# kdexd/probnmn-clevr

Hardware: AMD Instinct MI355X
Metric: CLEVR questions/sec (joint_training step) (higher is better)
Workload: dtype f32; 1 GPU; joint_training_ours.yml (NMN + seq2seq + REINFORCE), global batch 1024 = 1024 questions per GPU x 1 (BASELINE configs[3]), 14x14x1024 features, half of the batch with program supervision, fwd+bwd+[all-reduce]+clamp+Adam; global_batch=1024, per_gpu_batch=1024, parallelism=dp1

## Files before the change

include/probnmn_hip.h:

```cpp
#ifndef PROBNMN_HIP_H
#define PROBNMN_HIP_H

#include <stdint.h>

#ifdef __cplusplus
extern "C" {
#endif

#define PNMN_EINVAL (-1)
#define PNMN_ESHAPE (-2)

#define PNMN_CHANNELS 128

typedef struct pnmn_conv_item {
    const float* in;
    const float* in2;
    const float* mask;
    const float* gate;
    const float* weight;
    const float* bias;
    float*       out;
    int32_t      dilation;
    int32_t      flags;
    const float* mb_feats;
    const float* mb_attn;
    float*       mb_dfeats;
    float*       mb_dattn;
} pnmn_conv_item;
#define PNMN_CONV_ACCUMULATE 1
#define PNMN_CONV_ATOMIC     2
#define PNMN_CONV_MASKBWD    4
#define PNMN_CONV_DATTN     16
#define PNMN_CONV_MB_SOLE     8

int pnmn_conv_nhwc(const pnmn_conv_item* items, int n_items, int H, int W, int cin_chunks,
                   int ntaps , int in_stride, int out_stride,
                   int cout_blocks , int relu, void* stream);
int pnmn_conv_nhwc_cus(const pnmn_conv_item* items, int n_items, int H, int W, int cin_chunks, int ntaps, int in_stride,
                       int out_stride, int cout_blocks, int relu, int cus, void* stream);
int pnmn_conv_nhwc_launches(int n_items, int H, int W, int cin_chunks, int ntaps, int cout_blocks);
int pnmn_conv_force_split(int split);

typedef struct pnmn_wgrad_item {
    const float* x;
    const float* x2;
    const float* xmask;
    const float* dy;
    const float* gate;
    int32_t      dilation;
    int32_t      reserved;
} pnmn_wgrad_item;

typedef struct pnmn_wgrad_job {
    float*  dw;
    float*  dbias;
    int32_t item_begin;
    int32_t item_end;
} pnmn_wgrad_job;

int pnmn_conv_wgrad(const pnmn_wgrad_item* items, const pnmn_wgrad_job* jobs, int n_jobs, int H,
                    int W, int ntaps, int cin_blocks, int cout_blocks, int x_stride,
                    int dy_stride, void* stream);
int pnmn_conv_wgrad_cus(const pnmn_wgrad_item* items, const pnmn_wgrad_job* jobs, int n_jobs, int H, int W, int ntaps,
                        int cin_blocks, int cout_blocks, int x_stride, int dy_stride, int cus, void* stream);

typedef struct pnmn_wtrans_item {
    const float* src;
    float*       dst;
    int32_t      cout, cin, ntaps, reserved;
} pnmn_wtrans_item;
int pnmn_transpose_weights(const pnmn_wtrans_item* items, int n_items, void* stream);

typedef struct pnmn_dot1_item {
    const float* in;
    const float* w;
    const float* b;
    float*       out;
    const float* dout;
    float*       din;
    float*       dw;
    float*       db;
} pnmn_dot1_item;
int pnmn_dot1_sigmoid_fwd(const pnmn_dot1_item* items, int n_items, int HW, void* stream);
int pnmn_dot1_sigmoid_bwd(const pnmn_dot1_item* items, int n_items, int HW, void* stream);

typedef struct pnmn_same_item {
    const float* feats;
    const float* attn;
    const float* w;
    const float* b;
    float*       out;
    const float* dout;
    float*       dfeats;
    float*       dattn;
    float*       dw;
    float*       db;
} pnmn_same_item;
int pnmn_same_fwd(const pnmn_same_item* items, int n_items, int HW, void* stream);
int pnmn_same_bwd(const pnmn_same_item* items, int n_items, int HW, void* stream);

typedef struct pnmn_minmax_item {
    const float* a;
    const float* b;
    float*       out;
    const float* dout;
    float*       da;
    float*       db;
    int32_t      a_channels, b_channels;
    int32_t      is_max, reserved;
} pnmn_minmax_item;
int pnmn_minmax_fwd(const pnmn_minmax_item* items, int n_items, int HW, int C, void* stream);
int pnmn_minmax_bwd(const pnmn_minmax_item* items, int n_items, int HW, int C, void* stream);

typedef struct pnmn_maskbwd_item {
    const float* dx;
    const float* feats;
    const float* attn;
    float*       dfeats;
    float*       dattn;
} pnmn_maskbwd_item;
int pnmn_mask_bwd(const pnmn_maskbwd_item* items, int n_items, int HW, void* stream);
int pnmn_feat_grad_gather(const pnmn_maskbwd_item* items, float* gfeat, int n_items, int n_examples, int HW, void* stream);

typedef struct pnmn_axpy_item {
    const float* src;
    float*       dst;
    int64_t      n;
} pnmn_axpy_item;
int pnmn_accumulate(const pnmn_axpy_item* items, int n_items, void* stream);
int pnmn_set_rows(const pnmn_axpy_item* items, int n_items, void* stream);

int pnmn_nchw_to_nhwc(const float* src, float* dst, int n, int C, int HW, void* stream);
int pnmn_nchw_to_nhwc_rows(const float* src, float* dst, const int64_t* rows, int n, int C, int HW, void* stream);
int pnmn_nhwc_to_nchw(const float* src, float* dst, int n, int C, int HW, void* stream);

int pnmn_gather_features(const float* store, const int64_t* indices, float* dst, int n, int64_t n_store,
                         int C, int HW, void* stream);
int pnmn_copy_rows_h2d(const void* store, const int64_t* indices, void* dst, int n, int64_t n_store,
                       int64_t row_bytes, void* stream);

int pnmn_maxpool2_flatten_fwd(const float* in, float* out, int n, int H, int W, int C, void* stream);
int pnmn_maxpool2_flatten_bwd(const float* in, const float* dout, float* din, int n, int H, int W,
                              int C, void* stream);

int pnmn_answer_loss(const float* logits, const int64_t* answers, const int32_t* valid,
                     int64_t* predictions, float* loss, float* dlogits, int n, int num_answers,
                     int unknown_index, float scale, void* stream);

typedef struct {
    const float* src;
    const float* src2;
    float* dst;
    int32_t n, k, ld, kind;
} pnmn_derive_job;

int pnmn_token_prep(const int64_t* tokens, int64_t token_row_stride, int B, int T, int pad, int bos, int eos,
                    int drop_first, int64_t* out, float* fmask, int* last, void* stream);
int pnmn_length_order(const int32_t* last, int B, int T, int32_t* order, int32_t* tile_steps, void* stream);
int pnmn_trim_predictions(const int64_t* raw, int B, int T, int end, int64_t* out, void* stream);
int pnmn_mask_last_fwd(const float* hs, const float* fmask, const int* last, int B, int T, int H, float* enc,
                       float* hlast, void* stream);
int pnmn_mask_last_bwd(const float* denc, const float* dhlast, const float* fmask, const int* last, int B, int T,
                       int H, float* dhs, void* stream);
int64_t pnmn_embedding_grad_workspace_bytes(int B, int T, int V);
int pnmn_embedding_grad(const float* dy, const int64_t* tokens, int64_t token_row_stride, int B, int T, int C,
                        int V, int shift, int start, int skip, int accumulate, float* dw, void* workspace, void* stream);
int pnmn_derive_params(const pnmn_derive_job* jobs, int n_jobs, int max_quads, void* stream);

int pnmn_token_table_fwd(const float* emb, const float* weight, int64_t weight_row_stride,
                         const float* bias, int V, int K, int N, float* table, void* stream);
int pnmn_token_table_bwd(const float* dtable, const float* emb, const float* weight,
                         int64_t weight_row_stride, int V, int K, int N, int padding_idx, float* demb,
                         float* dweight, int64_t dweight_row_stride , float* dbias,
                         float* dbias2 , void* stream);

#define PNMN_TOKEN_SEGS 4
typedef struct pnmn_token_seg {
    const int64_t* src;
    const int64_t* index;
    int64_t        row_stride;
    int32_t        rows;
    int32_t        width;
} pnmn_token_seg;
int pnmn_token_rows(const pnmn_token_seg* segs , int n_segs, int64_t* dst, int W, int64_t pad, void* stream);

int pnmn_seq_nll_fwd(const float* logits, int64_t logits_bstride, const int64_t* tokens, int64_t tok_bstride,
                     const int64_t* mask_tokens, int64_t mask_bstride, int pad, float* loss, float* lse,
                     int B, int T, int V, float eps, void* stream);
int pnmn_seq_nll_bwd(const float* logits, int64_t logits_bstride, const int64_t* tokens, int64_t tok_bstride,
                     const int64_t* mask_tokens, int64_t mask_bstride, int pad, const float* lse,
                     const float* dloss, float* dlogits, int64_t dlogits_bstride, int B, int T, int V,
                     float eps, void* stream);

int pnmn_elbo_rows(const float* pg_loss, const float* qr_loss, const float* prior_loss, const float* nmn_loss,
                   const float* baseline, float beta, float gamma, int n, float* sums, float* dpg, void* stream);

int pnmn_joint_objective(const float* pg, const float* qr, const float* prior, const float* nmn, const float* pg_sup,
                         float* baseline, const float* w_unsup, const float* w_sup, float alpha, float beta, float gamma,
                         float decay, int update_baseline, int n, int m, float* stats, float* objective, float* d_pg,
                         float* d_qr, float* d_nmn, float* d_pg_sup, void* stream);

typedef struct pnmn_adam_item {
    float*       param;
    const float* grad;
    float*       exp_avg;
    float*       exp_avg_sq;
    int64_t      n;
    float        bc1;
    float        bc2_sqrt;
} pnmn_adam_item;
int pnmn_clamp_adam(const pnmn_adam_item* items, int n_items, double lr, double beta1, double beta2,
                    double eps, double weight_decay, double clamp, void* stream);
int pnmn_clamp_adam_blocks(const pnmn_adam_item* items, int n_items, double lr, double beta1, double beta2, double eps,
                           double weight_decay, double clamp, int blocks_per_item, void* stream);

int pnmn_lstm_cell_fwd(const float* gates, const float* c_prev, float* h, float* c, float* act,
                       int B, int hidden, void* stream);
int pnmn_lstm_cell_bwd(const float* act, const float* c_prev, const float* c, const float* dh,
                       const float* dc_in, float* dgates, float* dc_prev, int B, int hidden,
                       void* stream);

int pnmn_lstm_seq_fwd(const float* xp, const int64_t* tokens, int64_t token_stride, const float* w_hh,
                      float* hs, float* cs, float* act, int B, int T, int hidden, void* workspace,
                      void* stream);
int pnmn_lstm_seq_bwd(const float* dhs, const float* act, const float* cs, const float* w_hh_t,
                      float* dgates, int B, int T, int hidden, void* workspace, void* stream);
int64_t pnmn_lstm_seq_workspace_bytes(int B, int backward);
int pnmn_lstm_seq_fwd_ordered(const float* xp, const int64_t* tokens, int64_t token_stride, const float* w_hh,
                              float* hs, float* cs, float* act, int B, int T, int hidden, const int32_t* order,
                              const int32_t* tile_steps, void* workspace, void* stream);
int pnmn_lstm_seq_bwd_ordered(const float* dhs, const float* act, const float* cs, const float* w_hh_t,
                              float* dgates, int B, int T, int hidden, const int32_t* order,
                              const int32_t* tile_steps, void* workspace, void* stream);
int pnmn_cluster_reserve_cus(int cus);

int pnmn_attn_lstm_fwd(const float* xe, const float* etable, const float* enc, const float* mask,
                       const float* h0, const float* w_c, const float* w_hh, const float* w_p,
                       const float* b_p, float* hs, float* cs, float* act, float* ctx, float* probs,
                       int64_t* tokens, int B, int T, int S, int V, int hidden, int sample,
                       int pad_index, int unk_index, int start_index, uint64_t seed,
                       uint64_t row_offset, const int64_t* in_tokens, int64_t in_token_stride,
                       void* stream);
int pnmn_attn_lstm_bwd(const float* dhs, const float* act, const float* cs, const float* hs,
                       const float* ctx, const float* probs, const float* enc, const float* mask,
                       const float* h0, const float* w_c_t, const float* w_hh_t, float* dgates,
                       float* denc, float* dh0, int B, int T, int S, int hidden, void* stream);

int pnmn_attn_lstm_beam(const float* etable, const float* enc, const float* mask, const float* h0,
                        const float* w_c, const float* w_hh, const float* w_p, const float* b_p,
                        int64_t* tokens, float* scores, int32_t* trace_tokens, int32_t* trace_backptr,
                        float* trace_scores, int B, int T, int S, int V, int hidden, int beam,
                        int pad_index, int unk_index, int start_index, int end_index, void* stream);

#define PNMN_BEAM_MAX_STATES 32
#define PNMN_BEAM_MAX_CLASSES 16
int pnmn_attn_lstm_beam_constrained(const float* etable, const float* enc, const float* mask, const float* h0,
                                    const float* w_c, const float* w_hh, const float* w_p, const float* b_p,
                                    int64_t* tokens, float* scores, int32_t* trace_tokens, int32_t* trace_backptr,
                                    float* trace_scores, int B, int T, int S, int V, int hidden, int beam,
                                    int pad_index, int unk_index, int start_index, int end_index,
                                    const uint8_t* token_class, const uint8_t* next_state, const uint8_t* min_left,
                                    int n_states, int n_classes, void* stream);

typedef struct pnmn_decoder_fwd_job {
    const float *xe, *etable, *enc, *mask, *h0, *w_c, *w_hh, *w_p, *b_p;
    float *hs, *cs, *act, *ctx, *probs;
    int64_t* tokens;
    const int64_t* in_tokens;
    int64_t in_token_stride;
    uint64_t seed, row_offset;
    int32_t B, T, S, V, sample, pad_index, unk_index, start_index;
} pnmn_decoder_fwd_job;
typedef struct pnmn_decoder_bwd_job {
    const float *dhs, *act, *cs, *hs, *probs, *enc, *mask, *h0, *w_c_t, *w_hh_t;
    float *dgates, *dctx, *dscore, *weights, *dh0;
    int32_t B, T, S, reserved;
} pnmn_decoder_bwd_job;
int64_t pnmn_attn_lstm_group_workspace_bytes(const int32_t* rows, int n, int backward);
int pnmn_attn_lstm_fwd_group(const pnmn_decoder_fwd_job* jobs, int n, int hidden, void* workspace, void* stream);
int pnmn_attn_lstm_bwd_group(const pnmn_decoder_bwd_job* jobs, int n, int hidden, void* workspace, void* stream);
int pnmn_attn_denc(const float* weights, const float* dscore, const float* dctx, const float* hs, const float* h0,
                   float* denc, int B, int T, int S, int hidden, void* stream);

int pnmn_sample_tokens(const float* logits, int64_t* tokens, float* logprobs, int B, int V,
                       int greedy, uint64_t seed, uint64_t row_offset, uint32_t step, int pad_index,
                       int unk_index, int start_index, void* stream);

struct pnmn_sampling_filter {
    float temperature;
    int32_t top_k;
    float top_p;
    int32_t reserved;
};
int pnmn_sample_tokens_filtered(const float* logits, int64_t* tokens, float* logprobs, int B, int V,
                                int greedy, uint64_t seed, uint64_t row_offset, uint32_t step, int pad_index,
                                int unk_index, int start_index, const struct pnmn_sampling_filter* filter ,
                                void* stream);
int pnmn_attn_lstm_fwd_filtered(const float* xe, const float* etable, const float* enc, const float* mask,
                                const float* h0, const float* w_c, const float* w_hh, const float* w_p,
                                const float* b_p, float* hs, float* cs, float* act, float* ctx, float* probs,
                                int64_t* tokens, int B, int T, int S, int V, int hidden, int sample,
                                int pad_index, int unk_index, int start_index, uint64_t seed,
                                uint64_t row_offset, const int64_t* in_tokens, int64_t in_token_stride,
                                const struct pnmn_sampling_filter* filter , void* stream);
int pnmn_attn_lstm_fwd_group_filtered(const pnmn_decoder_fwd_job* jobs, const struct pnmn_sampling_filter* filters ,
                                      int n, int hidden, void* workspace, void* stream);

int pnmn_attn_lstm_fwd_constrained(const float* xe, const float* etable, const float* enc, const float* mask,
                                   const float* h0, const float* w_c, const float* w_hh, const float* w_p,
                                   const float* b_p, float* hs, float* cs, float* act, float* ctx, float* probs,
                                   int64_t* tokens, int B, int T, int S, int V, int hidden, int sample,
                                   int pad_index, int unk_index, int start_index, uint64_t seed,
                                   uint64_t row_offset, const int64_t* in_tokens, int64_t in_token_stride,
                                   const struct pnmn_sampling_filter* filter , int end_index,
                                   const uint8_t* token_class , const uint8_t* next_state ,
                                   const uint8_t* min_left , int n_states, int n_classes, void* stream);
int pnmn_attn_lstm_fwd_group_constrained(const pnmn_decoder_fwd_job* jobs, const struct pnmn_sampling_filter* filters ,
                                         int end_index, const uint8_t* token_class , const uint8_t* next_state ,
                                         const uint8_t* min_left , int n_states, int n_classes,
                                         int n, int hidden, void* workspace, void* stream);

#define PNMN_OP_CONV              0
#define PNMN_OP_WGRAD             1
#define PNMN_OP_TRANSPOSE_WEIGHTS 2
#define PNMN_OP_DOT_FWD           3
#define PNMN_OP_DOT_BWD           4
#define PNMN_OP_SAME_FWD          5
#define PNMN_OP_SAME_BWD          6
#define PNMN_OP_MINMAX_FWD        7
#define PNMN_OP_MINMAX_BWD        8
#define PNMN_OP_MASK_BWD          9
#define PNMN_OP_MAXPOOL_FWD       10
#define PNMN_OP_MAXPOOL_BWD       11
#define PNMN_OP_NCHW_TO_NHWC      12
#define PNMN_OP_SET_ROWS          13
#define PNMN_OP_ACCUMULATE        14
#define PNMN_OP_ZERO              15
#define PNMN_OP_FEAT_GATHER       16
typedef struct pnmn_launch {
    const void* a;
    const void* b;
    const void* c;
    int32_t     op;
    int32_t     n;
    int32_t     p[8];
} pnmn_launch;
int pnmn_run_launches(const pnmn_launch* list, int n, void* stream);

typedef struct pnmn_launch_timing {
    int32_t op, n;
    int32_t p[8];
    int32_t n_items;
    float   ms;
    double  flops, bytes;
} pnmn_launch_timing;
int pnmn_launch_trace_begin(void);
int pnmn_launch_trace_end(pnmn_launch_timing* out, int capacity, int* n_out);

#define PNMN_EAGAIN (-3)
typedef struct pnmn_trunk_config {
    const int32_t* kinds;
    const int64_t* w3;
    const int64_t* b3;
    const int64_t* wt3;
    const int64_t* dotw;
    const int64_t* dotb;
    int32_t n_kinds, channels, H, W, wgrad_chunk, wgrad_groups, fuse_mask_bwd, sole_writer, sort_by_weight, reserved;
} pnmn_trunk_config;
typedef struct pnmn_trunk_io {
    const int64_t*     programs;
    uint64_t           params, grads, wt, act, gact, feat, gfeat, final_, gfinal, ones;
    int64_t            act_capacity;
    const pnmn_launch* fwd_tail;
    const pnmn_launch* bwd_head;
    const pnmn_launch* bwd_tail;
    pnmn_launch*       bwd;
    uint8_t*           valid;
    int64_t            arena_floats;
    int32_t            n_programs, length, n_fwd_tail, n_bwd_head, n_bwd_tail, bwd_capacity, need_backward, launch;
    int32_t            n_bwd, bwd_piece_cut, n_prims, n_fwd, depth, n_invalid, n_feat_result;
    int32_t            conv_cus;
    int32_t            wgrad_cus;
    int32_t            n_conv, n_proj;
    int32_t            reserved;
    uint64_t           touched_tokens[4];
} pnmn_trunk_io;
int pnmn_trunk_planner_create(const pnmn_trunk_config* config, void** planner);
int pnmn_trunk_planner_destroy(void* planner);
int pnmn_trunk_plan_and_launch(void* planner, pnmn_trunk_io* io, void* stream);
int pnmn_trunk_last_forward(void* planner, pnmn_launch* out, int capacity);
int64_t pnmn_trunk_last_records_bytes(void* planner, uint64_t* out, int64_t capacity_words);

typedef struct {
    const int64_t* tables;
    const int64_t* nprims;
    const int64_t* tids;
    const int64_t* examples;
    const int64_t* base;
    const int64_t* tokens;
    const int64_t* w3;
    const int64_t* b3;
    const int64_t* wt3;
    const int64_t* dotw;
    const int64_t* dotb;
    uint64_t params, grads, wt, act, gact, feat, gfeat, final_, gfinal, ones;
    int32_t n_templates, pmax, nv, cmax;
    int32_t hw, channels, wgrad_chunk, wgrad_groups;
    int32_t fuse_mask_bwd, sole_writer, sort_by_weight, reserved;
} pnmn_plan_in;
int pnmn_plan_batch(const pnmn_plan_in* in, uint64_t* out_words, int64_t out_capacity, int64_t* meta, int32_t* cuts,
                    int32_t cuts_capacity);
int pnmn_compile_programs(const int64_t* tokens, int n_programs, int length, const int32_t* kinds,
                          int n_kinds, int channels, uint8_t* valid, int32_t* n_calls,
                          int32_t* calls, int32_t* result);

typedef struct pnmn_conv2d_desc {
    const float* x;
    const float* w;
    const float* scale;
    const float* shift;
    const float* residual;
    float*       y;
    int32_t      N, H, W, Cin, Ho, Wo, Cout, kh, kw, stride, pad, relu;
} pnmn_conv2d_desc;
int pnmn_conv2d_nhwc(const pnmn_conv2d_desc* desc, void* stream);
int pnmn_conv2d_weight_floats(int Cout, int Cin, int kh, int kw);
int pnmn_maxpool3x3s2_nhwc(const float* x, float* y, int N, int H, int W, int C, void* stream);

#define PNMN_IMAGE_PREP_MAX_TAPS  33
#define PNMN_IMAGE_PREP_MAX_WIDTH 448
#define PNMN_IMAGE_PREP_MAX_SIZE  16384
int pnmn_image_prep(const uint8_t* images, int64_t image_stride, int N, int Hin, int Win, const int32_t* kx,
                    const int32_t* xbounds, int ksx, const int32_t* ky, const int32_t* ybounds, int ksy,
// ... 70 lines not shown
```

probnmn-clevr_amd/csrc/decoder_multi.hip:

```cpp
#include <hip/hip_runtime.h>
#include <math.h>
#include <limits.h>
#include <stdint.h>

#include "../../include/probnmn_hip.h"
#include "cluster.h"
#include "lds_optin.h"
#include "sampling.h"

typedef float f32x4 __attribute__((ext_vector_type(4)));

namespace {

using pnmn::sigm;
using pnmn::wmax;
using pnmn::wsum;

constexpr int H = 256;
constexpr int G4 = 4 * H;
constexpr int ROWS = 16;
constexpr int MEMBERS = 8;
constexpr int RW = ROWS / MEMBERS;
constexpr int UW = H / MEMBERS;
constexpr int GLD = UW + 4;
constexpr int MAXS = 64;
constexpr int MAXV = 128;

__device__ __forceinline__ float dot4(const f32x4 a, const f32x4 b) { return a.x * b.x + a.y * b.y + a.z * b.z + a.w * b.w; }

struct MFwdArgs {
    const float* xe;
    const float* etable;
    const float* enc;
    const float* mask;
    const float* h0;
    const float* w_c;
    const float* w_hh;
    const float* w_p;
    const float* b_p;
    float* hs;
    float* cs;
    float* act;
    float* ctx;
    float* probs;
    int64_t* tokens;
    const int64_t* in_tokens;
    long in_stride;
    int* sync;
    int B, T, S, V, tiles;
    int sample;
    int pad, unk, start;
    uint64_t seed, row_offset;
};

constexpr size_t FWD_FIXED_LDS = sizeof(float) * (4 * ROWS * GLD + RW * 4 * H + ROWS * MAXV + RW * MAXS) + sizeof(int) * ROWS;
constexpr size_t FWD_OVERLAP_LDS = sizeof(float) * (ROWS * H + 64);

template <bool OVERLAP, bool SAMPLE, bool FILT = false, bool CONSTR = false>
__device__ __forceinline__ void attn_lstm_fwd_multi_body(const MFwdArgs& a, const int tile, const int part,
                                                         const pnmn::SamplingFilter& f = pnmn::SamplingFilter{1.f, 0, 1.f},
                                                         const pnmn::TokenAutomaton* aut = nullptr) {
    static_assert(SAMPLE || !CONSTR, "the automaton constrains the free-running modes only");
    extern __shared__ __attribute__((aligned(16))) char raw[];
    const int T = a.T, S = a.S;
    float* encl = reinterpret_cast<float*>(raw);
    float (*gl)[ROWS][GLD] = reinterpret_cast<float (*)[ROWS][GLD]>(encl + RW * S * H);
    float (*scl)[MAXS] = reinterpret_cast<float (*)[MAXS]>(&gl[4][0][0]);
    int* tokl = reinterpret_cast<int*>(&scl[RW][0]);
    float (*cpart)[4][H] = reinterpret_cast<float (*)[4][H]>(tokl + ROWS);
    float (*logl)[MAXV] = reinterpret_cast<float (*)[MAXV]>(&cpart[RW][0][0]);
    float* hst = &logl[ROWS][0];
    float* sink = hst + ROWS * H;

    const int tid = threadIdx.x, wave = tid >> 6, lane = tid & 63, li = lane & 15, g = lane >> 4;
    const int row0 = tile * ROWS, myrow0 = row0 + RW * part, u0 = UW * part;
    pnmn::Cluster cl;
    cl.start(a.sync + tile * pnmn::CLUSTER_COUNTER_STRIDE, MEMBERS);

    for (int i = tid; i < RW * S * (H / 4); i += 512) {
        const int rl = i / (S * (H / 4)), rem = i - rl * S * (H / 4);
        f32x4 v = f32x4{0.f, 0.f, 0.f, 0.f};
        if (myrow0 + rl < a.B) v = *reinterpret_cast<const f32x4*>(a.enc + (size_t)(myrow0 + rl) * S * H + 4 * rem);
        *reinterpret_cast<f32x4*>(encl + (size_t)rl * S * H + 4 * rem) = v;
    }
    const int gate = wave >> 1, ub = wave & 1;
    f32x4 wc[H / 16], wh[H / 16];
    {
        const int ntile = gate * (H / 16) + u0 / 16 + ub;
#pragma unroll
        for (int kb = 0; kb < H / 16; ++kb) {
            const size_t fo = ((size_t)(ntile * (H / 16) + kb) * 64 + lane) * 4;
            wc[kb] = *reinterpret_cast<const f32x4*>(a.w_c + fo);
            wh[kb] = *reinterpret_cast<const f32x4*>(a.w_hh + fo);
        }
    }
    if (tid < ROWS) tokl[tid] = a.start;
    const float row_mask = lane < S ? a.mask[(size_t)min(myrow0 + (wave >> 2), a.B - 1) * S + lane] : 0.f;
    float creg = 0.f;
    const int arow = min(row0 + li, a.B - 1);
    const int64_t* tf_row = (a.in_tokens && tid < ROWS) ? a.in_tokens + (size_t)min(row0 + tid, a.B - 1) * a.in_stride : nullptr;
    if (tf_row) tokl[tid] = (int)tf_row[0];

    constexpr int PARTF = ROWS * 64;
    const int s_row = tid >> 5, s_q = tid & 31;
    const int s_rowc = min(row0 + s_row, a.B - 1);
    const int s_off = (s_q >> 4) * PARTF + s_row * 64 + 4 * ((s_q & 15) ^ s_row);
    auto frags = [&](const float* tile_lds, const int p, f32x4 (&f)[4]) {
#pragma unroll
        for (int j = 0; j < 4; ++j) f[j] = *reinterpret_cast<const f32x4*>(tile_lds + p * PARTF + li * 64 + 4 * ((4 * j + g) ^ li));
    };
    auto mfma16 = [&](const f32x4 (&f)[4], const f32x4 (&w)[H / 16], const int p, f32x4& even, f32x4& odd) {
#pragma unroll
        for (int j = 0; j < 4; j += 2) {
            const int kb = p * 4 + j;
            even = __builtin_amdgcn_mfma_f32_16x16x4f32(f[j].x, w[kb].x, even, 0, 0, 0);
            odd = __builtin_amdgcn_mfma_f32_16x16x4f32(f[j + 1].x, w[kb + 1].x, odd, 0, 0, 0);
            even = __builtin_amdgcn_mfma_f32_16x16x4f32(f[j].y, w[kb].y, even, 0, 0, 0);
            odd = __builtin_amdgcn_mfma_f32_16x16x4f32(f[j + 1].y, w[kb + 1].y, odd, 0, 0, 0);
            even = __builtin_amdgcn_mfma_f32_16x16x4f32(f[j].z, w[kb].z, even, 0, 0, 0);
            odd = __builtin_amdgcn_mfma_f32_16x16x4f32(f[j + 1].z, w[kb + 1].z, odd, 0, 0, 0);
            even = __builtin_amdgcn_mfma_f32_16x16x4f32(f[j].w, w[kb].w, even, 0, 0, 0);
            odd = __builtin_amdgcn_mfma_f32_16x16x4f32(f[j + 1].w, w[kb + 1].w, odd, 0, 0, 0);
        }
    };

    auto stage_h = [&](const float* rows, const size_t row_stride) {
        const float* hsrc = rows + (size_t)s_rowc * row_stride + 4 * s_q;
        const f32x4 h_lo = *reinterpret_cast<const f32x4*>(hsrc), h_hi = *reinterpret_cast<const f32x4*>(hsrc + 128);
        *reinterpret_cast<f32x4*>(hst + s_off) = h_lo;
        *reinterpret_cast<f32x4*>(hst + s_off + 2 * PARTF) = h_hi;
    };
    if constexpr (OVERLAP) stage_h(a.h0, H);
    pnmn::AutomatonLds au{};
    int row_state[2] = {0, 0};
    if constexpr (CONSTR) au = pnmn::stage_automaton(reinterpret_cast<unsigned char*>(OVERLAP ? sink + 64 : hst), *aut);
    __syncthreads();

    for (int t = 0; t < T; ++t) {
        int zt = 0;
        asm volatile("" : "+v"(zt));
        f32x4 acc;
        f32x4 ph0 = f32x4{0.f, 0.f, 0.f, 0.f}, ph1 = ph0;
        auto load_inputs = [&] {
#pragma unroll
            for (int r = 0; r < 4; ++r) {
                const int rl = 4 * g + r, row = row0 + rl + zt;
                const int n = gate * H + u0 + 16 * ub + li;
                float v = 0.f;
                if (row < a.B) v = a.xe ? a.xe[((size_t)row * T + t) * G4 + n] : a.etable[(size_t)tokl[rl] * G4 + n];
                acc[r] = v;
            }
        };
        {
            const int rl = wave >> 2, q = wave & 3;
            const int row = myrow0 + rl + zt, rowc = min(row, a.B - 1);
            f32x4 hv;
            if constexpr (OVERLAP) {
                const int r = RW * part + rl;
                hv = *reinterpret_cast<const f32x4*>(hst + (lane >> 4) * PARTF + r * 64 + 4 * ((lane & 15) ^ r));
            } else {
                const float* hp = t > 0 ? a.hs + ((size_t)rowc * T + (t - 1)) * H : a.h0 + (size_t)rowc * H;
                hv = *reinterpret_cast<const f32x4*>(hp + 4 * lane);
            }
            const float* er = encl + (size_t)rl * S * H + 4 * lane;
            constexpr int NP = 4;
            int k_first = 0;
            if constexpr (OVERLAP) {
#pragma unroll
                for (int b = 0; b < 2; ++b) {
                    f32x4 ev[NP], hf[4];
                    float pk[NP];
#pragma unroll
                    for (int k = 0; k < NP; ++k) {
                        const int s = q + 4 * (NP * b + k);
                        ev[k] = *reinterpret_cast<const f32x4*>(er + (size_t)(s < S ? s : S - 1) * H);
                    }
                    frags(hst, b, hf);
                    mfma16(hf, wh, b, ph0, ph1);
#pragma unroll
                    for (int k = 0; k < NP; ++k) pk[k] = dot4(ev[k], hv);
#pragma unroll
                    for (int k = 0; k < NP; ++k) pk[k] = wsum(pk[k]);
#pragma unroll
                    for (int k = 0; k < NP; ++k) {
                        const int s = q + 4 * (NP * b + k);
                        float* dst = (lane == 0 && s < S) ? &scl[rl][s] : sink + lane;
                        *dst = pk[k];
                    }
                }
                k_first = 2 * NP;
            }
            {
                for (int k0 = k_first; q + 4 * k0 < S; k0 += NP) {
                    float part[NP];
#pragma unroll
                    for (int k = 0; k < NP; ++k) {
                        const int s = q + 4 * (k0 + k);
                        part[k] = s < S ? dot4(*reinterpret_cast<const f32x4*>(er + (size_t)s * H), hv) : 0.f;
                    }
#pragma unroll
                    for (int k = 0; k < NP; ++k) part[k] = wsum(part[k]);
#pragma unroll
                    for (int k = 0; k < NP; ++k)
                        if (lane == 0 && q + 4 * (k0 + k) < S) scl[rl][q + 4 * (k0 + k)] = part[k];
                }
            }
            __syncthreads();
            auto softmax = [&] {
                const float m = row_mask;
                const float v = (lane < S ? scl[rl][lane] : 0.f) * m;
                const float mx = wmax(lane < S ? v : -INFINITY);
                const float ex = lane < S ? expf(v - mx) : 0.f;
                const float p = ex / wsum(ex);
                const float qv = p * m;
                const float wgt = qv / (wsum(qv) + 1e-13f);
                if (lane < S) {
                    scl[rl][lane] = wgt;
                    if (row < a.B) a.probs[((size_t)row * T + t) * S + lane] = p;
                }
            };
            if constexpr (OVERLAP) {
                f32x4 hf[4];
                frags(hst, 2, hf);
                if (q == 0) {
                    mfma16(hf, wh, 2, ph0, ph1);
                    softmax();
                } else {
                    mfma16(hf, wh, 2, ph0, ph1);
                }
            } else {
                if (q == 0) softmax();
            }
            __syncthreads();
            f32x4 c4 = f32x4{0.f, 0.f, 0.f, 0.f};
            int s_first = q;
            if constexpr (OVERLAP) {
                constexpr int NC = 4;
                f32x4 ev[NC], hf[4];
                float wv[NC];
#pragma unroll
                for (int k = 0; k < NC; ++k) {
                    const int s = q + 4 * k, sc = s < S ? s : S - 1;
                    ev[k] = *reinterpret_cast<const f32x4*>(er + (size_t)sc * H);
                    const float w = scl[rl][sc];
                    wv[k] = s < S ? w : 0.f;
                }
                frags(hst, 3, hf);
                mfma16(hf, wh, 3, ph0, ph1);
#pragma unroll
                for (int k = 0; k < NC; ++k) c4 += ev[k] * wv[k];
                s_first = q + 4 * NC;
            }
            for (int s = s_first; s < S; s += 4) c4 += *reinterpret_cast<const f32x4*>(er + (size_t)s * H) * scl[rl][s];
            *reinterpret_cast<f32x4*>(&cpart[rl][q][4 * lane]) = c4;
            __syncthreads();
            const int rl2 = tid >> 8, k = tid & 255;
            const float cv = (cpart[rl2][0][k] + cpart[rl2][1][k]) + (cpart[rl2][2][k] + cpart[rl2][3][k]);
            if (myrow0 + rl2 < a.B) a.ctx[((size_t)(myrow0 + rl2 + zt) * T + t) * H + k] = cv;
        }
        cl.signal();
        cl.wait();

        const int tf_next = tf_row ? (int)tf_row[min(t + 1, T - 1)] : 0;
        if constexpr (OVERLAP) {
            float* cst = &cpart[0][0][0];
            const float* csrc = a.ctx + ((size_t)(s_rowc + zt) * T + t) * H + 4 * s_q;
            const f32x4 c_lo = *reinterpret_cast<const f32x4*>(csrc), c_hi = *reinterpret_cast<const f32x4*>(csrc + 128);
            load_inputs();
            *reinterpret_cast<f32x4*>(cst + s_off) = c_lo;
            *reinterpret_cast<f32x4*>(cst + s_off + 2 * PARTF) = c_hi;
            __syncthreads();
            f32x4 pc0 = f32x4{0.f, 0.f, 0.f, 0.f}, pc1 = pc0;
#pragma unroll
            for (int p = 0; p < 4; ++p) {
                f32x4 cf[4];
                frags(cst, p, cf);
                mfma16(cf, wc, p, pc0, pc1);
            }
            acc += (pc0 + pc1) + (ph0 + ph1);
        } else {
            load_inputs();
            constexpr int NB = 4, NPARTS = (H / 16) / NB, PART = 2 * ROWS * 64;
            float* stage = &cpart[0][0][0];
            const int s_tensor = tid >> 8, o_row = (tid >> 4) & 15, o_slot = tid & 15;
            const int o_rowc = min(row0 + o_row, a.B - 1);
            const float* s_src = (s_tensor == 0 ? a.ctx + ((size_t)o_rowc * T + t) * H
                                                : (t > 0 ? a.hs + ((size_t)o_rowc * T + (t - 1)) * H : a.h0 + (size_t)o_rowc * H)) + 4 * o_slot;
            float* s_dst = stage + (s_tensor * ROWS + o_row) * 64 + 4 * (o_slot ^ o_row);
            f32x4 sv = *reinterpret_cast<const f32x4*>(s_src);
            *reinterpret_cast<f32x4*>(s_dst) = sv;
            __syncthreads();
            f32x4 pc0 = f32x4{0.f, 0.f, 0.f, 0.f}, pc1 = pc0;
#pragma unroll
            for (int p = 0; p < NPARTS; ++p) {
                if (p + 1 < NPARTS) sv = *reinterpret_cast<const f32x4*>(s_src + (p + 1) * 64);
                const float* buf = stage + (p & 1) * PART;
                f32x4 ac[NB], ah[NB];
#pragma unroll
                for (int j = 0; j < NB; ++j) {
                    const int slot = (4 * j + g) ^ li;
                    ac[j] = *reinterpret_cast<const f32x4*>(buf + li * 64 + 4 * slot);
                    ah[j] = *reinterpret_cast<const f32x4*>(buf + (ROWS + li) * 64 + 4 * slot);
                }
                mfma16(ac, wc, p, pc0, pc1);
                mfma16(ah, wh, p, ph0, ph1);
                if (p + 1 < NPARTS) {
                    *reinterpret_cast<f32x4*>(s_dst + ((p + 1) & 1) * PART) = sv;
                    __syncthreads();
                }
            }
            acc += (pc0 + pc1) + (ph0 + ph1);
        }
#pragma unroll
        for (int r = 0; r < 4; ++r) gl[gate][4 * g + r][16 * ub + li] = acc[r];
        __syncthreads();
        {
            const int rl = tid >> 5, ul = tid & 31;
            const int row = row0 + rl + zt, u = u0 + ul;
            const float ig = sigm(gl[0][rl][ul]), fg = sigm(gl[1][rl][ul]);
            const float gg = tanhf(gl[2][rl][ul]), og = sigm(gl[3][rl][ul]);
            const float c = fg * creg + ig * gg;
            const float h = og * tanhf(c);
            creg = c;
            if (row < a.B) {
                const size_t o = ((size_t)row * T + t) * H + u;
                a.hs[o] = h;
                a.cs[o] = c;
                float* ar = a.act + ((size_t)row * T + t) * G4;
                ar[u] = ig;
                ar[H + u] = fg;
                ar[2 * H + u] = gg;
                ar[3 * H + u] = og;
            }
        }
        if (tf_row) tokl[tid] = tf_next;
        if (t + 1 == T && !SAMPLE) break;
        cl.signal();
        cl.wait();
        if constexpr (OVERLAP) {
            stage_h(a.hs + ((size_t)zt * T + t) * H, (size_t)T * H);
            __syncthreads();
        }

        if constexpr (SAMPLE) {
            const int V = a.V;
            if (16 * wave < V) {
                f32x4 lacc = f32x4{0.f, 0.f, 0.f, 0.f}, lodd = lacc;
                const int vn = 16 * wave + li;
                const bool vok = vn < V;
                const float* hp = a.hs + ((size_t)arow * T + t) * H + 4 * g;
                constexpr int NB = 4;
#pragma unroll
                for (int part = 0; part < (H / 16) / NB; ++part) {
                    f32x4 ah[NB], bp[NB];
                    if constexpr (OVERLAP) frags(hst, part, ah);
#pragma unroll
                    for (int j = 0; j < NB; ++j) {
                        const int kb = part * NB + j;
                        if constexpr (!OVERLAP) ah[j] = *reinterpret_cast<const f32x4*>(hp + kb * 16);
                        bp[j] = vok ? *reinterpret_cast<const f32x4*>(a.w_p + (size_t)vn * H + kb * 16 + 4 * g)
                                    : f32x4{0.f, 0.f, 0.f, 0.f};
                    }
#pragma unroll
                    for (int j = 0; j < NB; j += 2) {
                        lacc = __builtin_amdgcn_mfma_f32_16x16x4f32(ah[j].x, bp[j].x, lacc, 0, 0, 0);
                        lodd = __builtin_amdgcn_mfma_f32_16x16x4f32(ah[j + 1].x, bp[j + 1].x, lodd, 0, 0, 0);
                        lacc = __builtin_amdgcn_mfma_f32_16x16x4f32(ah[j].y, bp[j].y, lacc, 0, 0, 0);
                        lodd = __builtin_amdgcn_mfma_f32_16x16x4f32(ah[j + 1].y, bp[j + 1].y, lodd, 0, 0, 0);
                        lacc = __builtin_amdgcn_mfma_f32_16x16x4f32(ah[j].z, bp[j].z, lacc, 0, 0, 0);
                        lodd = __builtin_amdgcn_mfma_f32_16x16x4f32(ah[j + 1].z, bp[j + 1].z, lodd, 0, 0, 0);
                        lacc = __builtin_amdgcn_mfma_f32_16x16x4f32(ah[j].w, bp[j].w, lacc, 0, 0, 0);
                        lodd = __builtin_amdgcn_mfma_f32_16x16x4f32(ah[j + 1].w, bp[j + 1].w, lodd, 0, 0, 0);
                    }
                }
                lacc += lodd;
                const float bias = vok ? a.b_p[vn] : 0.f;
#pragma unroll
                for (int r = 0; r < 4; ++r) logl[4 * g + r][vn < MAXV ? vn : 0] = vok ? lacc[r] + bias : -INFINITY;
            }
            __syncthreads();
#pragma unroll
            for (int rr = 0; rr < 2; ++rr) {
                const int rl = 2 * wave + rr;
                const int row = row0 + rl;
                if (row >= a.B) continue;
                int choice;
                if constexpr (CONSTR) {
                    const auto set = pnmn::allowed_lanes(au, row_state[rr], T - 1 - t, V, a.pad, a.unk, a.start);
                    choice = pnmn::choose_row_token<FILT>(logl[rl], V, a.sample, a.pad, a.unk, a.start, a.seed,
                                                          a.row_offset + (uint64_t)row, (uint32_t)t, logl[rl], f, set);
                    row_state[rr] = pnmn::advance_row_state(au, row_state[rr], choice);
                } else {
                    choice = pnmn::choose_row_token<FILT>(logl[rl], V, a.sample, a.pad, a.unk, a.start, a.seed,
                                                          a.row_offset + (uint64_t)row, (uint32_t)t, logl[rl], f);
                }
                if (lane == 0) {
                    tokl[rl] = choice;
                    if (part == 0) a.tokens[(size_t)row * T + t] = choice;
                }
            }
            __syncthreads();
        }
    }
    cl.finish();
}

template <bool OVERLAP, bool SAMPLE>
__global__ __launch_bounds__(512) __attribute__((amdgpu_waves_per_eu(2, 2))) void attn_lstm_fwd_multi_kernel(const MFwdArgs a) {
    int tile, part;
    pnmn::cluster_coords<MEMBERS>(tile, part);
    if (tile >= a.tiles) return;
    attn_lstm_fwd_multi_body<OVERLAP, SAMPLE>(a, tile, part);
}

template <bool OVERLAP, bool SAMPLE0, bool SAMPLE1>
__global__ __launch_bounds__(512) __attribute__((amdgpu_waves_per_eu(2, 2))) void attn_lstm_fwd_pair_kernel(const MFwdArgs a0,
                                                                                                           const MFwdArgs a1,
                                                                                                           const int tiles0) {
    int tile, part;
    pnmn::cluster_coords<MEMBERS>(tile, part);
    if (tile < tiles0) {
        if (tile >= a0.tiles) return;
        attn_lstm_fwd_multi_body<OVERLAP, SAMPLE0>(a0, tile, part);
    } else {
        tile -= tiles0;
        if (tile >= a1.tiles) return;
        attn_lstm_fwd_multi_body<OVERLAP, SAMPLE1>(a1, tile, part);
    }
}

template <bool OVERLAP>
__global__ __launch_bounds__(512) __attribute__((amdgpu_waves_per_eu(2, 2))) void attn_lstm_fwd_multi_filtered_kernel(
    const MFwdArgs a, const pnmn::SamplingFilter f) {
    int tile, part;
    pnmn::cluster_coords<MEMBERS>(tile, part);
    if (tile >= a.tiles) return;
    attn_lstm_fwd_multi_body<OVERLAP, true, true>(a, tile, part, f);
}

template <bool OVERLAP, int M0, int M1>
__global__ __launch_bounds__(512) __attribute__((amdgpu_waves_per_eu(2, 2))) void attn_lstm_fwd_pair_filtered_kernel(
    const MFwdArgs a0, const MFwdArgs a1, const int tiles0, const pnmn::SamplingFilter f0, const pnmn::SamplingFilter f1) {
    int tile, part;
    pnmn::cluster_coords<MEMBERS>(tile, part);
    if (tile < tiles0) {
        if (tile >= a0.tiles) return;
        attn_lstm_fwd_multi_body<OVERLAP, M0 != 0, M0 == 2>(a0, tile, part, f0);
    } else {
        tile -= tiles0;
        if (tile >= a1.tiles) return;
        attn_lstm_fwd_multi_body<OVERLAP, M1 != 0, M1 == 2>(a1, tile, part, f1);
    }
}

template <bool OVERLAP, bool FILT>
__global__ __launch_bounds__(512) __attribute__((amdgpu_waves_per_eu(2, 2))) void attn_lstm_fwd_multi_constrained_kernel(
    const MFwdArgs a, const pnmn::SamplingFilter f, const pnmn::TokenAutomaton au) {
    int tile, part;
    pnmn::cluster_coords<MEMBERS>(tile, part);
    if (tile >= a.tiles) return;
    attn_lstm_fwd_multi_body<OVERLAP, true, FILT, true>(a, tile, part, f, &au);
}

template <bool OVERLAP, int M0, int M1>
__global__ __launch_bounds__(512) __attribute__((amdgpu_waves_per_eu(2, 2))) void attn_lstm_fwd_pair_constrained_kernel(
    const MFwdArgs a0, const MFwdArgs a1, const int tiles0, const pnmn::SamplingFilter f0, const pnmn::SamplingFilter f1,
    const pnmn::TokenAutomaton au) {
    int tile, part;
    pnmn::cluster_coords<MEMBERS>(tile, part);
    if (tile < tiles0) {
        if (tile >= a0.tiles) return;
        attn_lstm_fwd_multi_body<OVERLAP, M0 != 0, M0 == 2, M0 != 0>(a0, tile, part, f0, &au);
    } else {
        tile -= tiles0;
        if (tile >= a1.tiles) return;
        attn_lstm_fwd_multi_body<OVERLAP, M1 != 0, M1 == 2, M1 != 0>(a1, tile, part, f1, &au);
    }
}

struct MBwdArgs {
    const float* dhs;
    const float* act;
    const float* cs;
    const float* hs;
    const float* probs;
    const float* enc;
    const float* mask;
    const float* h0;
    const float* w_c_t;
    const float* w_hh_t;
    float* dgates;
    float* dctx;
    float* dscore;
    float* weights;
    float* dh0;
    float* x1;
    float* x2;
    int* sync;
    int B, T, S, tiles;
};

constexpr int DLD = 4 * UW + 4;
constexpr size_t BWD_FIXED_LDS = sizeof(float) * (ROWS * DLD + 2 * RW * H + 2 * RW * MAXS + RW * 4 * H + 64);

__device__ __forceinline__ void attn_lstm_bwd_multi_body(const MBwdArgs& a, const int tile, const int part) {
    extern __shared__ __attribute__((aligned(16))) char raw[];
    const int T = a.T, S = a.S;
    float* encl = reinterpret_cast<float*>(raw);
    float (*dgl)[DLD] = reinterpret_cast<float (*)[DLD]>(encl + RW * S * H);
    float (*dctxl)[H] = reinterpret_cast<float (*)[H]>(&dgl[ROWS][0]);
    float (*dhl)[H] = dctxl + RW;
    float (*dwl)[MAXS] = reinterpret_cast<float (*)[MAXS]>(&dhl[RW][0]);
    float (*dhpart)[4][H] = reinterpret_cast<float (*)[4][H]>(&dwl[2 * RW][0]);
    float* sink = &dhpart[RW][0][0];

    const int tid = threadIdx.x, wave = tid >> 6, lane = tid & 63, li = lane & 15, g = lane >> 4;
    const int row0 = tile * ROWS, myrow0 = row0 + RW * part, u0 = UW * part;
    pnmn::Cluster cl;
    cl.start(a.sync + tile * pnmn::CLUSTER_COUNTER_STRIDE, MEMBERS);
    float* x1t = a.x1 + (size_t)tile * 2 * MEMBERS * 2 * ROWS * H;
    float* x2t = a.x2 + (size_t)tile * 2 * ROWS * H;

    for (int i = tid; i < RW * S * (H / 4); i += 512) {
        const int rl = i / (S * (H / 4)), rem = i - rl * S * (H / 4);
        f32x4 v = f32x4{0.f, 0.f, 0.f, 0.f};
        if (myrow0 + rl < a.B) v = *reinterpret_cast<const f32x4*>(a.enc + (size_t)(myrow0 + rl) * S * H + 4 * rem);
        *reinterpret_cast<f32x4*>(encl + (size_t)rl * S * H + 4 * rem) = v;
    }
    constexpr int KB = 4 * UW / 16;
    f32x4 wc[2][KB], wh[2][KB];
#pragma unroll
    for (int nt = 0; nt < 2; ++nt)
#pragma unroll
        for (int kl = 0; kl < KB; ++kl) {
            const int q = kl / (UW / 16), jj = kl % (UW / 16);
            const int kb = (q * H + u0) / 16 + jj;
            const size_t fo = ((size_t)((2 * wave + nt) * (G4 / 16) + kb) * 64 + lane) * 4;
            wc[nt][kl] = *reinterpret_cast<const f32x4*>(a.w_c_t + fo);
            wh[nt][kl] = *reinterpret_cast<const f32x4*>(a.w_hh_t + fo);
        }
    float dc_rec = 0.f;
    const float row_mask = lane < S ? a.mask[(size_t)min(myrow0 + (wave >> 2), a.B - 1) * S + lane] : 0.f;
    __syncthreads();

    struct Saved {
        float ig, fg, gg, og, c, cp, dhs, p;
    };
    const int c_rl = tid >> 5, c_ul = tid & 31;
    const int c_row = row0 + c_rl, c_u = u0 + c_ul;
    const int p_row = min(myrow0 + (wave >> 2), a.B - 1);
    auto load_saved = [&](int t) {
        Saved v{0.f, 0.f, 0.f, 0.f, 0.f, 0.f, 0.f, 0.f};
        if (c_row < a.B) {
            const size_t o = ((size_t)c_row * T + t) * H + c_u;
            const float* ar = a.act + ((size_t)c_row * T + t) * G4;
            v.ig = ar[c_u], v.fg = ar[H + c_u], v.gg = ar[2 * H + c_u], v.og = ar[3 * H + c_u];
            v.c = a.cs[o];
            v.cp = t > 0 ? a.cs[o - H] : 0.f;
            v.dhs = a.dhs[o];
        }
        if ((wave & 3) == 0 && lane < S) v.p = a.probs[((size_t)p_row * T + t) * S + lane];
        return v;
    };
    Saved sv = load_saved(T - 1);

    auto dg_frag = [&](const int kl) { return *reinterpret_cast<const f32x4*>(&dgl[li][kl * 16 + 4 * g]); };
    auto mfma16 = [&](const f32x4 (&w)[2][KB], const int kl0, f32x4 (&acc)[2]) {
#pragma unroll
        for (int kl = kl0; kl < kl0 + 2; ++kl) {
            const f32x4 av = dg_frag(kl);
#pragma unroll
            for (int nt = 0; nt < 2; ++nt) {
                acc[nt] = __builtin_amdgcn_mfma_f32_16x16x4f32(w[nt][kl].x, av.x, acc[nt], 0, 0, 0);
                acc[nt] = __builtin_amdgcn_mfma_f32_16x16x4f32(w[nt][kl].y, av.y, acc[nt], 0, 0, 0);
                acc[nt] = __builtin_amdgcn_mfma_f32_16x16x4f32(w[nt][kl].z, av.z, acc[nt], 0, 0, 0);
                acc[nt] = __builtin_amdgcn_mfma_f32_16x16x4f32(w[nt][kl].w, av.w, acc[nt], 0, 0, 0);
            }
        }
    };

    for (int t = T - 1; t >= 0; --t) {
        const Saved cur = sv;
        int zt = 0;
        asm volatile("" : "+v"(zt));
        {
            const int rl = c_rl, ul = c_ul;
            const int row = c_row + zt, u = c_u;
            float di = 0.f, df = 0.f, dg = 0.f, dout = 0.f, dcp = 0.f;
            if (row < a.B) {
                const float ig = cur.ig, fg = cur.fg, gg = cur.gg, og = cur.og;
                const float c = cur.c;
                const float cp = cur.cp;
                const float tc = tanhf(c);
                float dhp = 0.f;
                if (t < T - 1) {
                    const float* ph = x1t + (((size_t)((t + 1) & 1) * MEMBERS) * 2 + 1) * ROWS * H + (size_t)(rl + zt) * H + u;
                    float pv[MEMBERS];
#pragma unroll
                    for (int m = 0; m < MEMBERS; ++m) pv[m] = ph[(size_t)(2 * m) * ROWS * H];
                    const float att = x2t[((size_t)((t + 1) & 1) * ROWS + rl) * H + u];
                    float sh = 0.f;
#pragma unroll
                    for (int m = 0; m < MEMBERS; ++m) sh += pv[m];
                    dhp = sh + att;
                }
                const float dh = cur.dhs + dhp;
                const float dc = dc_rec + dh * og * (1.f - tc * tc);
                di = dc * gg * ig * (1.f - ig);
                df = dc * cp * fg * (1.f - fg);
                dg = dc * ig * (1.f - gg * gg);
                dout = dh * tc * og * (1.f - og);
                dcp = dc * fg;
                float* dr = a.dgates + ((size_t)row * T + t) * G4;
                dr[u] = di;
                dr[H + u] = df;
                dr[2 * H + u] = dg;
                dr[3 * H + u] = dout;
            }
            dc_rec = dcp;
            dgl[rl][ul] = di;
            dgl[rl][UW + ul] = df;
            dgl[rl][2 * UW + ul] = dg;
            dgl[rl][3 * UW + ul] = dout;
        }
        __syncthreads();
        float* const pc = x1t + (((size_t)(t & 1) * MEMBERS + part) * 2 + 0) * ROWS * H;
        float* const ph = pc + ROWS * H;
        {
            f32x4 accc[2] = {f32x4{0.f, 0.f, 0.f, 0.f}, f32x4{0.f, 0.f, 0.f, 0.f}};
#pragma unroll
            for (int kl = 0; kl < KB; kl += 2) mfma16(wc, kl, accc);
#pragma unroll
            for (int nt = 0; nt < 2; ++nt) {
                const size_t o = (size_t)(li + zt) * H + 16 * (2 * wave + nt) + 4 * g;
                *reinterpret_cast<f32x4*>(pc + o) = accc[nt];
            }
        }
        cl.signal();
        cl.wait();

        f32x4 acch[2] = {f32x4{0.f, 0.f, 0.f, 0.f}, f32x4{0.f, 0.f, 0.f, 0.f}};
        {
            const int rl2 = tid >> 8, k = tid & 255;
            const float* src = x1t + (size_t)(t & 1) * MEMBERS * 2 * ROWS * H + (size_t)(RW * part + rl2 + zt) * H + k;
            float pv[MEMBERS];
#pragma unroll
            for (int s = 0; s < MEMBERS; ++s) pv[s] = src[(size_t)(2 * s) * ROWS * H];
            float sc = 0.f;
#pragma unroll
            for (int s = 0; s < MEMBERS; ++s) sc += pv[s];
            dctxl[rl2][k] = sc;
            if (myrow0 + rl2 < a.B) a.dctx[((size_t)(myrow0 + rl2 + zt) * T + t) * H + k] = sc;
        }
        __syncthreads();
        {
            const int rl = wave >> 2, q = wave & 3;
            const int row = myrow0 + rl + zt;
            const float* er = encl + (size_t)rl * S * H + 4 * lane;
            const f32x4 dc4 = *reinterpret_cast<const f32x4*>(&dctxl[rl][4 * lane]);
            constexpr int NP = 4;
#pragma unroll
            for (int b = 0; b < 2; ++b) {
                f32x4 ev[NP];
                float pk[NP];
#pragma unroll
                for (int k = 0; k < NP; ++k) {
                    const int s = q + 4 * (NP * b + k);
                    ev[k] = *reinterpret_cast<const f32x4*>(er + (size_t)(s < S ? s : S - 1) * H);
                }
                mfma16(wh, 2 * b, acch);
#pragma unroll
                for (int k = 0; k < NP; ++k) pk[k] = dot4(ev[k], dc4);
#pragma unroll
                for (int k = 0; k < NP; ++k) pk[k] = wsum(pk[k]);
#pragma unroll
                for (int k = 0; k < NP; ++k) {
                    const int s = q + 4 * (NP * b + k);
                    float* dst = (lane == 0 && s < S) ? &dwl[rl][s] : sink + lane;
                    *dst = pk[k];
                }
            }
            for (int k0 = 2 * NP; q + 4 * k0 < S; k0 += NP) {
                float part[NP];
#pragma unroll
                for (int k = 0; k < NP; ++k) {
                    const int s = q + 4 * (k0 + k);
                    part[k] = s < S ? dot4(*reinterpret_cast<const f32x4*>(er + (size_t)s * H), dc4) : 0.f;
                }
#pragma unroll
                for (int k = 0; k < NP; ++k) part[k] = wsum(part[k]);
#pragma unroll
                for (int k = 0; k < NP; ++k)
                    if (lane == 0 && q + 4 * (k0 + k) < S) dwl[rl][q + 4 * (k0 + k)] = part[k];
            }
            __syncthreads();
            auto softmax_bwd = [&] {
                const float m = row_mask;
                const float p = lane < S ? cur.p : 0.f;
                const float qv = p * m;
                const float Z = wsum(qv) + 1e-13f;
                const float dw = lane < S ? dwl[rl][lane] : 0.f;
                const float dq = dw / Z - wsum(dw * qv) / (Z * Z);
                const float dp = dq * m;
                const float dv = p * (dp - wsum(dp * p));
                const float dscore = dv * m;
                if (lane < S) {
                    dwl[rl][lane] = dscore;
                    if (row < a.B) {
                        a.dscore[((size_t)row * T + t) * S + lane] = dscore;
                        a.weights[((size_t)row * T + t) * S + lane] = qv / Z;
                    }
                }
            };
            if (q == 0) {
                mfma16(wh, 4, acch);
                softmax_bwd();
            } else {
                mfma16(wh, 4, acch);
            }
            __syncthreads();
            f32x4 dh4 = f32x4{0.f, 0.f, 0.f, 0.f};
            {
                constexpr int NC = 4;
                f32x4 ev[NC];
                float wv[NC];
#pragma unroll
                for (int k = 0; k < NC; ++k) {
                    const int s = q + 4 * k, sc = s < S ? s : S - 1;
                    ev[k] = *reinterpret_cast<const f32x4*>(er + (size_t)sc * H);
                    const float w = dwl[rl][sc];
                    wv[k] = s < S ? w : 0.f;
                }
                mfma16(wh, 6, acch);
#pragma unroll
                for (int k = 0; k < NC; ++k) dh4 += ev[k] * wv[k];
            }
            for (int s = q + 16; s < S; s += 4) dh4 += *reinterpret_cast<const f32x4*>(er + (size_t)s * H) * dwl[rl][s];
            *reinterpret_cast<f32x4*>(&dhpart[rl][q][4 * lane]) = dh4;
        }
#pragma unroll
        for (int nt = 0; nt < 2; ++nt) {
            const size_t o = (size_t)(li + zt) * H + 16 * (2 * wave + nt) + 4 * g;
            *reinterpret_cast<f32x4*>(ph + o) = acch[nt];
        }
        __syncthreads();
        {
            const int rl2 = tid >> 8, k = tid & 255;
            const float v = (dhpart[rl2][0][k] + dhpart[rl2][1][k]) + (dhpart[rl2][2][k] + dhpart[rl2][3][k]);
            x2t[((size_t)(t & 1) * ROWS + RW * part + rl2 + zt) * H + k] = v;
        }
        if (t > 0) sv = load_saved(t - 1);
        cl.signal();
        cl.wait();
    }
    {
        const int rl2 = tid >> 8, k = tid & 255;
        const float* ph0 = x1t + (size_t)1 * ROWS * H + (size_t)(RW * part + rl2) * H + k;
        float pv[MEMBERS];
#pragma unroll
        for (int m = 0; m < MEMBERS; ++m) pv[m] = ph0[(size_t)(2 * m) * ROWS * H];
        const float att = x2t[((size_t)0 * ROWS + RW * part + rl2) * H + k];
        float sh = 0.f;
#pragma unroll
        for (int m = 0; m < MEMBERS; ++m) sh += pv[m];
        if (myrow0 + rl2 < a.B) a.dh0[(size_t)(myrow0 + rl2) * H + k] = sh + att;
    }
    cl.finish();
}

__global__ __launch_bounds__(512) __attribute__((amdgpu_waves_per_eu(2, 2))) void attn_lstm_bwd_multi_kernel(const MBwdArgs a) {
    int tile, part;
    pnmn::cluster_coords<MEMBERS>(tile, part);
    if (tile >= a.tiles) return;
    attn_lstm_bwd_multi_body(a, tile, part);
}

__global__ __launch_bounds__(512) __attribute__((amdgpu_waves_per_eu(2, 2))) void attn_lstm_bwd_pair_kernel(const MBwdArgs a0,
                                                                                                           const MBwdArgs a1,
                                                                                                           const int tiles0) {
    int tile, part;
    pnmn::cluster_coords<MEMBERS>(tile, part);
    if (tile < tiles0) {
        if (tile >= a0.tiles) return;
        attn_lstm_bwd_multi_body(a0, tile, part);
    } else {
        tile -= tiles0;
        if (tile >= a1.tiles) return;
        attn_lstm_bwd_multi_body(a1, tile, part);
    }
}

__global__ __launch_bounds__(512) __attribute__((amdgpu_waves_per_eu(2, 2))) void attn_lstm_bwd_group3_kernel(const MBwdArgs a0,
                                                                                                             const MBwdArgs a1,
                                                                                                             const MBwdArgs a2,
                                                                                                             const int tiles0,
                                                                                                             const int tiles01) {
    int tile, part;
    pnmn::cluster_coords<MEMBERS>(tile, part);
    if (tile < tiles0) {
        if (tile >= a0.tiles) return;
        attn_lstm_bwd_multi_body(a0, tile, part);
    } else if (tile < tiles01) {
        tile -= tiles0;
        if (tile >= a1.tiles) return;
        attn_lstm_bwd_multi_body(a1, tile, part);
    } else {
        tile -= tiles01;
        if (tile >= a2.tiles) return;
        attn_lstm_bwd_multi_body(a2, tile, part);
    }
}

const void* fwd_multi_variant(bool overlap, bool sample) {
    if (overlap) return sample ? reinterpret_cast<const void*>(attn_lstm_fwd_multi_kernel<true, true>)
                               : reinterpret_cast<const void*>(attn_lstm_fwd_multi_kernel<true, false>);
    return sample ? reinterpret_cast<const void*>(attn_lstm_fwd_multi_kernel<false, true>)
                  : reinterpret_cast<const void*>(attn_lstm_fwd_multi_kernel<false, false>);
}
template <bool OVERLAP>
const void* fwd_pair_variant_of(bool s0, bool s1) {
    if (s0) return s1 ? reinterpret_cast<const void*>(attn_lstm_fwd_pair_kernel<OVERLAP, true, true>)
                      : reinterpret_cast<const void*>(attn_lstm_fwd_pair_kernel<OVERLAP, true, false>);
    return s1 ? reinterpret_cast<const void*>(attn_lstm_fwd_pair_kernel<OVERLAP, false, true>)
              : reinterpret_cast<const void*>(attn_lstm_fwd_pair_kernel<OVERLAP, false, false>);
}
const void* fwd_pair_variant(bool overlap, bool s0, bool s1) {
    return overlap ? fwd_pair_variant_of<true>(s0, s1) : fwd_pair_variant_of<false>(s0, s1);
}

const void* fwd_multi_filtered_variant(bool overlap) {
    return overlap ? reinterpret_cast<const void*>(attn_lstm_fwd_multi_filtered_kernel<true>)
                   : reinterpret_cast<const void*>(attn_lstm_fwd_multi_filtered_kernel<false>);
}
template <bool OVERLAP>
const void* fwd_pair_filtered_variant_of(int m0, int m1) {
    if (m0 == 2) return m1 == 2 ? reinterpret_cast<const void*>(attn_lstm_fwd_pair_filtered_kernel<OVERLAP, 2, 2>)
                       : m1 == 1 ? reinterpret_cast<const void*>(attn_lstm_fwd_pair_filtered_kernel<OVERLAP, 2, 1>)
                                 : reinterpret_cast<const void*>(attn_lstm_fwd_pair_filtered_kernel<OVERLAP, 2, 0>);
    return m0 == 1 ? reinterpret_cast<const void*>(attn_lstm_fwd_pair_filtered_kernel<OVERLAP, 1, 2>)
                   : reinterpret_cast<const void*>(attn_lstm_fwd_pair_filtered_kernel<OVERLAP, 0, 2>);
}
const void* fwd_pair_filtered_variant(bool overlap, int m0, int m1) {
    return overlap ? fwd_pair_filtered_variant_of<true>(m0, m1) : fwd_pair_filtered_variant_of<false>(m0, m1);
}

const void* fwd_multi_constrained_variant(bool overlap, int m) {
    if (overlap) return m == 2 ? reinterpret_cast<const void*>(attn_lstm_fwd_multi_constrained_kernel<true, true>)
                               : reinterpret_cast<const void*>(attn_lstm_fwd_multi_constrained_kernel<true, false>);
    return m == 2 ? reinterpret_cast<const void*>(attn_lstm_fwd_multi_constrained_kernel<false, true>)
                  : reinterpret_cast<const void*>(attn_lstm_fwd_multi_constrained_kernel<false, false>);
}
template <bool OVERLAP>
const void* fwd_pair_constrained_variant_of(int m0, int m1) {
    if (m0 == 0) return m1 == 2 ? reinterpret_cast<const void*>(attn_lstm_fwd_pair_constrained_kernel<OVERLAP, 0, 2>)
                                : reinterpret_cast<const void*>(attn_lstm_fwd_pair_constrained_kernel<OVERLAP, 0, 1>);
    if (m0 == 1) return m1 == 2 ? reinterpret_cast<const void*>(attn_lstm_fwd_pair_constrained_kernel<OVERLAP, 1, 2>)
                                : reinterpret_cast<const void*>(attn_lstm_fwd_pair_constrained_kernel<OVERLAP, 1, 1>);
    return reinterpret_cast<const void*>(attn_lstm_fwd_pair_constrained_kernel<OVERLAP, 2, 2>);
}
const void* fwd_pair_constrained_variant(bool overlap, int m0, int m1) {
    return overlap ? fwd_pair_constrained_variant_of<true>(m0, m1) : fwd_pair_constrained_variant_of<false>(m0, m1);
}

int rows_per_launch() {
    const int cus = pnmn::device_cus();
    return cus >= 8 * MEMBERS ? (cus / (8 * MEMBERS)) * 8 * ROWS : 0;
}


constexpr size_t LDS_LIMIT = 160 * 1024;
constexpr int MAX_JOBS = 3;

inline int padded_tiles(int B) { return 8 * ((((B + ROWS - 1) / ROWS) + 7) / 8); }

bool fits(const int* rows, int n) {
    const int chunk = rows_per_launch();
    int tiles = 0;
    for (int i = 0; i < n; ++i) {
        if (rows[i] <= 0) return false;
        tiles += padded_tiles(rows[i]);
    }
    return chunk > 0 && tiles * ROWS <= chunk && tiles <= 128;
}
template <class Job>
bool jobs_fit(const Job* j, int n) {
    int rows[MAX_JOBS];
    for (int i = 0; i < n; ++i) {
        if (j[i].T <= 0) return false;
        rows[i] = j[i].B;
    }
    return fits(rows, n);
}

int exchange_tiles(const int* rows, int n, int chunk) {
    if (n == 1) return ((rows[0] < chunk ? rows[0] : chunk) + ROWS - 1) / ROWS;
    int tiles = 0;
    for (int i = 0; i < n; ++i) tiles += padded_tiles(rows[i]);
    return tiles;
}

int64_t workspace_bytes(const int* rows, int n, bool backward) {
    if (n > 1 && !fits(rows, n)) {
        const int64_t a = workspace_bytes(rows, n - 1, backward), b = workspace_bytes(rows + n - 1, 1, backward);
        return a > b ? a : b;
    }
    const int chunk = rows_per_launch();
    if (chunk <= 0 || rows[0] <= 0) return 0;
    int64_t bytes = (int64_t)pnmn::CLUSTER_SYNC_BYTES;
    if (backward) bytes += (int64_t)exchange_tiles(rows, n, chunk) * (2 * MEMBERS * 2 + 2) * ROWS * H * sizeof(float);
    return bytes;
}

int check_job(const pnmn_decoder_fwd_job& j, int hidden) {
    if (!j.enc || !j.mask || !j.h0 || !j.w_c || !j.w_hh || !j.hs || !j.cs || !j.act || !j.ctx || !j.probs) return PNMN_EINVAL;
    if (j.sample ? (!j.etable || !j.w_p || !j.b_p || !j.tokens) : (!j.xe && !(j.etable && j.in_tokens))) return PNMN_EINVAL;
    if (hidden != H || j.S < 1 || j.S > MAXS || (j.sample && (j.V < 1 || j.V > MAXV))) return PNMN_ESHAPE;
    return 0;
}
int check_job(const pnmn_decoder_bwd_job& j, int hidden) {
    if (!j.dhs || !j.act || !j.cs || !j.hs || !j.probs || !j.enc || !j.mask || !j.h0 || !j.w_c_t || !j.w_hh_t || !j.dgates ||
        !j.dctx || !j.dscore || !j.weights || !j.dh0)
        return PNMN_EINVAL;
    if (hidden != H || j.S < 1 || j.S > MAXS) return PNMN_ESHAPE;
    return 0;
}

MFwdArgs kernel_args(const pnmn_decoder_fwd_job& j, size_t r, int rows, int* sync, int tile0) {
    const int T = j.T, S = j.S;
    return MFwdArgs{j.xe ? j.xe + r * T * G4 : nullptr, j.etable, j.enc + r * S * H, j.mask + r * S, j.h0 + r * H, j.w_c, j.w_hh,
                    j.w_p, j.b_p, j.hs + r * T * H, j.cs + r * T * H, j.act + r * T * G4, j.ctx + r * T * H, j.probs + r * T * S,
                    j.tokens ? j.tokens + r * T : nullptr, (!j.sample && !j.xe) ? j.in_tokens + r * j.in_token_stride : nullptr,
                    (long)j.in_token_stride, sync + tile0 * pnmn::CLUSTER_COUNTER_STRIDE, rows, T, S, j.V, (rows + ROWS - 1) / ROWS,
                    j.sample, j.pad_index, j.unk_index, j.start_index, j.seed, j.row_offset + r};
}
MBwdArgs kernel_args(const pnmn_decoder_bwd_job& j, size_t r, int rows, int* sync, int tile0, float* x1, float* x2) {
    const int T = j.T, S = j.S;
    return MBwdArgs{j.dhs + r * T * H, j.act + r * T * G4, j.cs + r * T * H, j.hs + r * T * H, j.probs + r * T * S,
                    j.enc + r * S * H, j.mask + r * S, j.h0 + r * H, j.w_c_t, j.w_hh_t, j.dgates + r * T * G4, j.dctx + r * T * H,
                    j.dscore + r * T * S, j.weights + r * T * S, j.dh0 + r * H, x1 + (size_t)tile0 * 2 * MEMBERS * 2 * ROWS * H,
                    x2 + (size_t)tile0 * 2 * ROWS * H, sync + tile0 * pnmn::CLUSTER_COUNTER_STRIDE, rows, T, S,
                    (rows + ROWS - 1) / ROWS};
}

template <class Job>
int plan_group(const Job* j, int n, int hidden, int& smax, int& chunk, int* rows, int* tile0) {
    smax = 0;
    tile0[0] = 0;
    for (int i = 0; i < n; ++i) {
        if (const int e = check_job(j[i], hidden)) return e;
        smax = j[i].S > smax ? j[i].S : smax;
        rows[i] = j[i].B;
        tile0[i + 1] = tile0[i] + padded_tiles(rows[i]);
    }
    chunk = rows_per_launch();
    return chunk > 0 ? 0 : PNMN_ESHAPE;
}

int launch_fwd_constrained(const pnmn_decoder_fwd_job* j, const pnmn_sampling_filter* f, const pnmn::TokenAutomaton& au, int n,
                           int hidden, void* workspace, hipStream_t st);
int launch_fwd(const pnmn_decoder_fwd_job* j, const pnmn_sampling_filter* f, int n, int hidden, void* workspace, hipStream_t st,
               const pnmn::TokenAutomaton* au = nullptr) {
    if (n > 1 && !jobs_fit(j, n)) {
        const int rc = launch_fwd(j, f, n - 1, hidden, workspace, st, au);
        return rc != 0 ? rc : launch_fwd(j + n - 1, f ? f + n - 1 : nullptr, 1, hidden, workspace, st, au);
    }
    if (au && (j[0].sample != 0 || (n > 1 && j[1].sample != 0))) return launch_fwd_constrained(j, f, *au, n, hidden, workspace, st);
    if (j[0].B <= 0 || j[0].T <= 0) return 0;
    int smax, chunk, rows[MAX_JOBS], tile0[MAX_JOBS + 1];
    if (const int e = plan_group(j, n, hidden, smax, chunk, rows, tile0)) return e;
    const bool overlap = FWD_FIXED_LDS + sizeof(float) * RW * smax * H + FWD_OVERLAP_LDS <= LDS_LIMIT;
    const size_t lds = FWD_FIXED_LDS + sizeof(float) * RW * smax * H + (overlap ? FWD_OVERLAP_LDS : 0);
    const bool s0 = j[0].sample != 0, s1 = n > 1 && j[1].sample != 0;
    int m[2] = {0, 0};
    pnmn::SamplingFilter ff[2] = {{1.f, 0, 1.f}, {1.f, 0, 1.f}};
    for (int i = 0; i < n; ++i) {
        m[i] = j[i].sample == 0 ? 0 : (f && j[i].sample == 1 && !pnmn::filter_is_identity(f[i])) ? 2 : 1;
        if (m[i] == 2) ff[i] = pnmn::SamplingFilter{f[i].temperature, f[i].top_k, f[i].top_p};
    }
    const bool filtered = m[0] == 2 || m[1] == 2;
    const void* kernel = filtered ? (n == 1 ? fwd_multi_filtered_variant(overlap) : fwd_pair_filtered_variant(overlap, m[0], m[1]))
                                  : (n == 1 ? fwd_multi_variant(overlap, s0) : fwd_pair_variant(overlap, s0, s1));
    {
        static std::atomic<uint64_t> cfg[2][8], cfg_filtered[2][2][9];
        std::atomic<uint64_t>& c = filtered ? cfg_filtered[n - 1][overlap][3 * m[0] + m[1]] : cfg[n - 1][4 * overlap + 2 * s0 + s1];
        if (const int e = pnmn::opt_in_lds(kernel, LDS_LIMIT, c)) return e;
    }
    int* sync = nullptr;
    if (n > 1) {
        hipError_t e = pnmn::cluster_sync_block(workspace, st, &sync);
        if (e != hipSuccess) return (int)e;
        const MFwdArgs a0 = kernel_args(j[0], 0, rows[0], sync, 0), a1 = kernel_args(j[1], 0, rows[1], sync, tile0[1]);
        if (filtered) {
            const auto pair = reinterpret_cast<void (*)(const MFwdArgs, const MFwdArgs, const int, const pnmn::SamplingFilter,
                                                        const pnmn::SamplingFilter)>(const_cast<void*>(kernel));
            hipLaunchKernelGGL(pair, dim3(MEMBERS * tile0[2]), dim3(512), lds, st, a0, a1, tile0[1], ff[0], ff[1]);
        } else {
            const auto pair = reinterpret_cast<void (*)(const MFwdArgs, const MFwdArgs, const int)>(const_cast<void*>(kernel));
            hipLaunchKernelGGL(pair, dim3(MEMBERS * tile0[2]), dim3(512), lds, st, a0, a1, tile0[1]);
        }
        return (int)hipGetLastError();
    }
    for (int r0 = 0; r0 < rows[0]; r0 += chunk) {
        const int part = rows[0] - r0 < chunk ? rows[0] - r0 : chunk;
        hipError_t e = pnmn::cluster_sync_block(workspace, st, &sync);
        if (e != hipSuccess) return (int)e;
        const MFwdArgs a = kernel_args(j[0], (size_t)r0, part, sync, 0);
        if (filtered) {
            const auto multi = reinterpret_cast<void (*)(const MFwdArgs, const pnmn::SamplingFilter)>(const_cast<void*>(kernel));
            hipLaunchKernelGGL(multi, dim3(MEMBERS * padded_tiles(part)), dim3(512), lds, st, a, ff[0]);
        } else {
            const auto multi = reinterpret_cast<void (*)(const MFwdArgs)>(const_cast<void*>(kernel));
            hipLaunchKernelGGL(multi, dim3(MEMBERS * padded_tiles(part)), dim3(512), lds, st, a);
        }
        e = hipGetLastError();
        if (e != hipSuccess) return (int)e;
    }
    return 0;
}

int launch_fwd_constrained(const pnmn_decoder_fwd_job* j, const pnmn_sampling_filter* f, const pnmn::TokenAutomaton& au, int n,
                           int hidden, void* workspace, hipStream_t st) {
    if (j[0].B <= 0 || j[0].T <= 0) return 0;
    int smax, chunk, rows[MAX_JOBS], tile0[MAX_JOBS + 1];
    if (const int e = plan_group(j, n, hidden, smax, chunk, rows, tile0)) return e;
    constexpr size_t TABLES = pnmn::AUTOMATON_LDS_BYTES;
    const bool overlap = FWD_FIXED_LDS + sizeof(float) * RW * smax * H + FWD_OVERLAP_LDS + TABLES <= LDS_LIMIT;
    const size_t lds = FWD_FIXED_LDS + sizeof(float) * RW * smax * H + (overlap ? FWD_OVERLAP_LDS : 0) + TABLES;
    int m[2] = {0, 0};
    pnmn::SamplingFilter ff[2] = {{1.f, 0, 1.f}, {1.f, 0, 1.f}};
    for (int i = 0; i < n; ++i) {
        m[i] = j[i].sample == 0 ? 0 : (j[i].sample == 1 && !pnmn::filter_is_identity(f[i])) ? 2 : 1;
        if (m[i] == 2) ff[i] = pnmn::SamplingFilter{f[i].temperature, f[i].top_k, f[i].top_p};
    }
    int* sync = nullptr;
    static std::atomic<uint64_t> cfg[2][2][9];
    if (n > 1) {
        const int lo = m[0] <= m[1] ? 0 : 1, hi = 1 - lo;
        const void* kernel = fwd_pair_constrained_variant(overlap, m[lo], m[hi]);
        if (const int e = pnmn::opt_in_lds(kernel, LDS_LIMIT, cfg[1][overlap][3 * m[lo] + m[hi]])) return e;
        hipError_t e = pnmn::cluster_sync_block(workspace, st, &sync);
        if (e != hipSuccess) return (int)e;
        const int tiles_lo = padded_tiles(rows[lo]);
        const MFwdArgs a0 = kernel_args(j[lo], 0, rows[lo], sync, 0), a1 = kernel_args(j[hi], 0, rows[hi], sync, tiles_lo);
        const auto pair = reinterpret_cast<void (*)(const MFwdArgs, const MFwdArgs, const int, const pnmn::SamplingFilter,
                                                    const pnmn::SamplingFilter, const pnmn::TokenAutomaton)>(const_cast<void*>(kernel));
        hipLaunchKernelGGL(pair, dim3(MEMBERS * tile0[2]), dim3(512), lds, st, a0, a1, tiles_lo, ff[lo], ff[hi], au);
        return (int)hipGetLastError();
    }
    const void* kernel = fwd_multi_constrained_variant(overlap, m[0]);
    if (const int e = pnmn::opt_in_lds(kernel, LDS_LIMIT, cfg[0][overlap][m[0]])) return e;
    const auto multi = reinterpret_cast<void (*)(const MFwdArgs, const pnmn::SamplingFilter, const pnmn::TokenAutomaton)>(
        const_cast<void*>(kernel));
    for (int r0 = 0; r0 < rows[0]; r0 += chunk) {
        const int part = rows[0] - r0 < chunk ? rows[0] - r0 : chunk;
        hipError_t e = pnmn::cluster_sync_block(workspace, st, &sync);
        if (e != hipSuccess) return (int)e;
        const MFwdArgs a = kernel_args(j[0], (size_t)r0, part, sync, 0);
        hipLaunchKernelGGL(multi, dim3(MEMBERS * padded_tiles(part)), dim3(512), lds, st, a, ff[0], au);
        e = hipGetLastError();
        if (e != hipSuccess) return (int)e;
    }
    return 0;
}

int launch_bwd(const pnmn_decoder_bwd_job* j, int n, int hidden, void* workspace, hipStream_t st) {
    if (n > 1 && !jobs_fit(j, n)) {
        const int rc = launch_bwd(j, n - 1, hidden, workspace, st);
        return rc != 0 ? rc : launch_bwd(j + n - 1, 1, hidden, workspace, st);
    }
    if (j[0].B <= 0 || j[0].T <= 0) return 0;
    int smax, chunk, rows[MAX_JOBS], tile0[MAX_JOBS + 1];
    if (const int e = plan_group(j, n, hidden, smax, chunk, rows, tile0)) return e;
    const size_t lds = BWD_FIXED_LDS + sizeof(float) * RW * smax * H;
    {
        const void* const kernels[MAX_JOBS] = {reinterpret_cast<const void*>(attn_lstm_bwd_multi_kernel),
                                               reinterpret_cast<const void*>(attn_lstm_bwd_pair_kernel),
                                               reinterpret_cast<const void*>(attn_lstm_bwd_group3_kernel)};
        static std::atomic<uint64_t> cfg[MAX_JOBS];
        if (const int e = pnmn::opt_in_lds(kernels[n - 1], LDS_LIMIT, cfg[n - 1])) return e;
    }
    float* x1 = reinterpret_cast<float*>(static_cast<char*>(workspace) + pnmn::CLUSTER_SYNC_BYTES);
    float* x2 = x1 + (size_t)exchange_tiles(rows, n, chunk) * 2 * MEMBERS * 2 * ROWS * H;
    int* sync = nullptr;
    if (n > 1) {
        hipError_t e = pnmn::cluster_sync_block(workspace, st, &sync);
        if (e != hipSuccess) return (int)e;
        MBwdArgs a[MAX_JOBS];
        for (int i = 0; i < n; ++i) a[i] = kernel_args(j[i], 0, rows[i], sync, tile0[i], x1, x2);
        const dim3 grid(MEMBERS * tile0[n]);
        if (n == 2) hipLaunchKernelGGL(attn_lstm_bwd_pair_kernel, grid, dim3(512), lds, st, a[0], a[1], tile0[1]);
        else hipLaunchKernelGGL(attn_lstm_bwd_group3_kernel, grid, dim3(512), lds, st, a[0], a[1], a[2], tile0[1], tile0[2]);
        return (int)hipGetLastError();
    }
    for (int r0 = 0; r0 < rows[0]; r0 += chunk) {
        const int part = rows[0] - r0 < chunk ? rows[0] - r0 : chunk;
        hipError_t e = pnmn::cluster_sync_block(workspace, st, &sync);
        if (e != hipSuccess) return (int)e;
        const MBwdArgs a = kernel_args(j[0], (size_t)r0, part, sync, 0, x1, x2);
        hipLaunchKernelGGL(attn_lstm_bwd_multi_kernel, dim3(MEMBERS * padded_tiles(part)), dim3(512), lds, st, a);
        e = hipGetLastError();
        if (e != hipSuccess) return (int)e;
    }
    return 0;
}

}

extern "C" {

int64_t pnmn_attn_lstm_group_workspace_bytes(const int32_t* rows, int n, int backward) {
    if (!rows || n < 1 || n > MAX_JOBS) return 0;
    return workspace_bytes(rows, n, backward != 0);
}

int pnmn_attn_lstm_fwd_group(const pnmn_decoder_fwd_job* jobs, int n, int hidden, void* workspace, void* stream) {
    if (!jobs || !workspace || n < 1 || n > 2) return PNMN_EINVAL;
    return launch_fwd(jobs, nullptr, n, hidden, workspace, static_cast<hipStream_t>(stream));
}

int pnmn_attn_lstm_fwd_group_filtered(const pnmn_decoder_fwd_job* jobs, const pnmn_sampling_filter* filters, int n, int hidden,
                                      void* workspace, void* stream) {
    if (!jobs || !filters || !workspace || n < 1 || n > 2) return PNMN_EINVAL;
    for (int i = 0; i < n; ++i)
        if (!pnmn::filter_valid(filters + i)) return PNMN_EINVAL;
    return launch_fwd(jobs, filters, n, hidden, workspace, static_cast<hipStream_t>(stream));
}

int pnmn_attn_lstm_fwd_group_constrained(const pnmn_decoder_fwd_job* jobs, const pnmn_sampling_filter* filters, int end_index,
                                         const uint8_t* token_class, const uint8_t* next_state, const uint8_t* min_left,
                                         int n_states, int n_classes, int n, int hidden, void* workspace, void* stream) {
    if (!jobs || !filters || !workspace || n < 1 || n > 2) return PNMN_EINVAL;
    int V = 0, T = INT_MAX;
    for (int i = 0; i < n; ++i) {
        if (!pnmn::filter_valid(filters + i)) return PNMN_EINVAL;
        if (jobs[i].sample == 0) continue;
        if (V != 0 && jobs[i].V != V) return PNMN_EINVAL;
        V = jobs[i].V;
        T = jobs[i].T < T ? jobs[i].T : T;
    }
    pnmn::TokenAutomaton au;
    if (const int e = pnmn::fill_automaton(au, token_class, next_state, min_left, n_states, n_classes, V, T, end_index)) return e;
    return launch_fwd(jobs, filters, n, hidden, workspace, static_cast<hipStream_t>(stream), &au);
}

int pnmn_attn_lstm_bwd_group(const pnmn_decoder_bwd_job* jobs, int n, int hidden, void* workspace, void* stream) {
    if (!jobs || !workspace || n < 1 || n > MAX_JOBS) return PNMN_EINVAL;
    return launch_bwd(jobs, n, hidden, workspace, static_cast<hipStream_t>(stream));
}

}
```

probnmn-clevr_amd/csrc/seqglue.hip:

```cpp
#include <hip/hip_runtime.h>
#include <stdint.h>
#include <stdlib.h>

#include "../../include/probnmn_hip.h"

namespace {

__global__ __launch_bounds__(256) void token_prep_kernel(const int64_t* __restrict__ tokens, int64_t tstride, int B, int T,
                                                         int pad, int bos, int eos, int drop_first,
                                                         int64_t* __restrict__ out, float* __restrict__ fmask,
                                                         int* __restrict__ last) {
    const int b = blockIdx.x * 4 + (threadIdx.x >> 6);
    const int lane = threadIdx.x & 63;
    if (b >= B) return;
    const int64_t* row = tokens + (size_t)b * tstride;
    int n = 0;
    for (int t = lane; t < T; t += 64) n += row[t] != pad;
#pragma unroll
    for (int o = 32; o > 0; o >>= 1) n += __shfl_xor(n, o);
    const int W = T + 2 - drop_first;
    int valid = 0;
    for (int j = lane; j < W; j += 64) {
        const int f = j + drop_first;
        int64_t v = (f == 0) ? bos : (f <= T ? row[f - 1] : 0);
        if (f == n + 1) v = eos;
        out[(size_t)b * W + j] = v;
        const bool m = v != pad;
        if (fmask) fmask[(size_t)b * W + j] = m ? 1.f : 0.f;
        valid += m;
    }
    if (last) {
#pragma unroll
        for (int o = 32; o > 0; o >>= 1) valid += __shfl_xor(valid, o);
        if (lane == 0) last[b] = valid - 1;
    }
}

struct TokenSegs {
    pnmn_token_seg s[PNMN_TOKEN_SEGS];
    int n;
};
__global__ __launch_bounds__(256) void token_rows_kernel(const TokenSegs segs, int64_t* __restrict__ dst, int W, int64_t pad,
                                                         int total) {
    const int r = blockIdx.x * 4 + (threadIdx.x >> 6), lane = threadIdx.x & 63;
    if (r >= total) return;
    int k = 0, first = 0;
    while (k + 1 < segs.n && r >= first + segs.s[k].rows) first += segs.s[k].rows, ++k;
    const pnmn_token_seg sg = segs.s[k];
    const int64_t i = sg.index ? sg.index[r - first] : (int64_t)(r - first);
    const int64_t* row = sg.src + i * sg.row_stride;
    for (int w = lane; w < W; w += 64) dst[(size_t)r * W + w] = w < sg.width ? row[w] : pad;
}

__global__ __launch_bounds__(256) void trim_predictions_kernel(const int64_t* __restrict__ raw, int B, int T, int end,
                                                               int64_t* __restrict__ out) {
    const int b = blockIdx.x * 4 + (threadIdx.x >> 6);
    const int lane = threadIdx.x & 63;
    if (b >= B) return;
    const int64_t* row = raw + (size_t)b * T;
    int first = T;
    for (int t = lane; t < T; t += 64)
        if (row[t] == end && t < first) first = t;
#pragma unroll
    for (int o = 32; o > 0; o >>= 1) first = min(first, __shfl_xor(first, o));
    for (int t = lane; t < T; t += 64) {
        const bool keep = (first == T) || (first > 0 && t <= first);
        out[(size_t)b * T + t] = keep ? row[t] : 0;
    }
}

__global__ __launch_bounds__(256) void mask_last_fwd_kernel(const float* __restrict__ hs, const float* __restrict__ fmask,
                                                            const int* __restrict__ last, int T, int H,
                                                            float* __restrict__ enc, float* __restrict__ hlast) {
    const int b = blockIdx.x;
    int l = last[b];
    if (l < 0) l += T;
    const int h4 = H >> 2;
    const float4* src = reinterpret_cast<const float4*>(hs + (size_t)b * T * H);
    float4* dst = reinterpret_cast<float4*>(enc + (size_t)b * T * H);
    for (int i = blockIdx.y * 256 + threadIdx.x; i < T * h4; i += gridDim.y * 256) {
        const int t = i / h4;
        const float m = fmask[(size_t)b * T + t];
        float4 v = src[i];
        v.x *= m, v.y *= m, v.z *= m, v.w *= m;
        dst[i] = v;
        if (t == l) reinterpret_cast<float4*>(hlast + (size_t)b * H)[i - t * h4] = v;
    }
}

constexpr int LO_MAX_T = 4096;
__global__ __launch_bounds__(64) void length_order_kernel(const int32_t* __restrict__ last, int B, int T,
                                                          int32_t* __restrict__ order, int32_t* __restrict__ tile_steps) {
    extern __shared__ int first[];
    const int lane = threadIdx.x;
    for (int s = lane; s <= T; s += 64) first[s] = 0;
    __syncthreads();
    for (int b = lane; b < B; b += 64) atomicAdd(&first[min(max(last[b] + 1, 1), T)], 1);
    __syncthreads();
    int carry = 0;
    for (int top = T; top >= 1; top -= 64) {
        const int s = top - lane;
        const int n = s >= 1 ? first[s] : 0;
        int incl = n;
#pragma unroll
        for (int o = 1; o < 64; o <<= 1) {
            const int v = __shfl_up(incl, o);
            if (lane >= o) incl += v;
        }
        if (s >= 1) first[s] = carry + incl - n;
        carry += __shfl(incl, 63);
    }
    __syncthreads();
    for (int b0 = 0; b0 < B; b0 += 64) {
        const int b = b0 + lane;
        const int s = b < B ? min(max(last[b] + 1, 1), T) : 0;
        int before = 0, after = 0;
        for (int j = 0; j < 64; ++j) {
            const int sj = __shfl(s, j);
            before += (sj == s && j < lane);
            after += (sj == s && j > lane);
        }
        const int pos = s ? first[s] + before : 0;
        __syncthreads();
        if (s) {
            order[pos] = b;
            if ((pos & 15) == 0) tile_steps[pos >> 4] = s;
            if (after == 0) first[s] = pos + 1;
        }
        __syncthreads();
    }
}

__global__ __launch_bounds__(256) void mask_last_bwd_kernel(const float* __restrict__ denc, const float* __restrict__ dhlast,
                                                            const float* __restrict__ fmask, const int* __restrict__ last,
                                                            int T, int H, float* __restrict__ dhs) {
    const int b = blockIdx.x;
    int l = last[b];
    if (l < 0) l += T;
    const int h4 = H >> 2;
    const float4* src = denc ? reinterpret_cast<const float4*>(denc + (size_t)b * T * H) : nullptr;
    float4* dst = reinterpret_cast<float4*>(dhs + (size_t)b * T * H);
    for (int i = blockIdx.y * 256 + threadIdx.x; i < T * h4; i += gridDim.y * 256) {
        const int t = i / h4;
        const float m = fmask[(size_t)b * T + t];
        float4 v = src ? src[i] : float4{0.f, 0.f, 0.f, 0.f};
        if (dhlast && t == l) {
            const float4 d = reinterpret_cast<const float4*>(dhlast + (size_t)b * H)[i - t * h4];
            v.x += d.x, v.y += d.y, v.z += d.z, v.w += d.w;
        }
        v.x *= m, v.y *= m, v.z *= m, v.w *= m;
        dst[i] = v;
    }
}

constexpr int EG_CHUNK = 64;

__device__ __forceinline__ int eg_token(const int64_t* __restrict__ tokens, int64_t tok_bstride, int T, unsigned magic, int shift,
                                        int start, int skip, int V, int r) {
    int b = magic ? (int)__umulhi((unsigned)r, magic) : r;
    b -= (b * T > r);
    const int t = r - b * T;
    const int64_t raw = tokens[(size_t)b * tok_bstride + (shift ? max(t - 1, 0) : t)];
    const int64_t v = (shift && t == 0) ? (int64_t)start : raw;
    return (v == skip || v < 0 || v >= V) ? -1 : (int)v;
}

__global__ __launch_bounds__(1024) void embedding_rows_kernel(const int64_t* __restrict__ tokens, int64_t tok_bstride, int B,
                                                              int T, unsigned magic, int V, int shift, int start, int skip, int C,
                                                              int* __restrict__ order, int* __restrict__ chunks, int max_per,
                                                              int* __restrict__ count, float* __restrict__ dw, int keep) {
    __shared__ int whist[16][128], hist[128], rowbase[128], chbase[128];
    const int tid = threadIdx.x, wave = tid >> 6;
    const int per = (B * T + gridDim.x - 1) / gridDim.x;
    const int lo = blockIdx.x * per, R = min(B * T, lo + per);
    chunks += 3 * (size_t)blockIdx.x * max_per;
    count += blockIdx.x;
    for (int i = tid; i < 16 * 128; i += 1024) (&whist[0][0])[i] = 0;
    __syncthreads();
    constexpr int UN = 8;
    for (int r0 = lo + tid; r0 < R; r0 += 1024 * UN) {
        int v[UN];
#pragma unroll
        for (int u = 0; u < UN; ++u) v[u] = eg_token(tokens, tok_bstride, T, magic, shift, start, skip, V, min(r0 + 1024 * u, R - 1));
#pragma unroll
        for (int u = 0; u < UN; ++u)
            if (r0 + 1024 * u < R && v[u] >= 0) atomicAdd(&whist[wave][v[u]], 1);
    }
    if (!keep)
        for (size_t i = blockIdx.x * 1024 + tid; i < (size_t)V * C / 4; i += 1024 * gridDim.x)
            reinterpret_cast<float4*>(dw)[i] = float4{0.f, 0.f, 0.f, 0.f};
    __syncthreads();
    if (tid < 128) {
        int run = 0;
        for (int w = 0; w < 16; ++w) {
            const int n = whist[w][tid];
            whist[w][tid] = run;
            run += n;
        }
        hist[tid] = run;
    }
    __syncthreads();
    if (tid == 0) {
        int rows = lo, ch = 0;
        for (int v = 0; v < V; ++v) {
            rowbase[v] = rows, chbase[v] = ch;
            rows += hist[v];
            ch += (hist[v] + EG_CHUNK - 1) / EG_CHUNK;
        }
        *count = ch;
    }
    __syncthreads();
    for (int r0 = lo + tid; r0 < R; r0 += 1024 * UN) {
        int v[UN];
#pragma unroll
        for (int u = 0; u < UN; ++u) v[u] = eg_token(tokens, tok_bstride, T, magic, shift, start, skip, V, min(r0 + 1024 * u, R - 1));
#pragma unroll
        for (int u = 0; u < UN; ++u)
            if (r0 + 1024 * u < R && v[u] >= 0) order[rowbase[v[u]] + atomicAdd(&whist[wave][v[u]], 1)] = r0 + 1024 * u;
    }
    for (int v = tid; v < V; v += 1024) {
        const int n = hist[v];
        for (int j = 0; j * EG_CHUNK < n; ++j) {
            int* c = chunks + 3 * (chbase[v] + j);
            c[0] = v, c[1] = rowbase[v] + j * EG_CHUNK, c[2] = rowbase[v] + min(n, (j + 1) * EG_CHUNK);
        }
    }
}

__global__ __launch_bounds__(256) void embedding_sum_kernel(const float* __restrict__ dy, const int* __restrict__ order,
                                                            const int* __restrict__ chunks, int max_per,
                                                            const int* __restrict__ count, int C, float* __restrict__ dw) {
    const int slice = blockIdx.x / max_per, j = blockIdx.x % max_per;
    if (j >= count[slice]) return;
    const int c = (blockIdx.y * 256 + threadIdx.x) * 4;
    if (c >= C) return;
    const int* ch = chunks + 3 * ((size_t)slice * max_per + j);
    const int v = ch[0], b = ch[1], e = ch[2];
    constexpr int UN = 8;
    float4 acc = float4{0.f, 0.f, 0.f, 0.f};
    for (int i = b; i < e; i += UN) {
        float4 q[UN];
#pragma unroll
        for (int u = 0; u < UN; ++u) q[u] = *reinterpret_cast<const float4*>(dy + (size_t)order[min(i + u, e - 1)] * C + c);
#pragma unroll
        for (int u = 0; u < UN; ++u)
            if (i + u < e) acc.x += q[u].x, acc.y += q[u].y, acc.z += q[u].z, acc.w += q[u].w;
    }
    float* dst = dw + (size_t)v * C + c;
    unsafeAtomicAdd(dst, acc.x);
    unsafeAtomicAdd(dst + 1, acc.y);
    unsafeAtomicAdd(dst + 2, acc.z);
    unsafeAtomicAdd(dst + 3, acc.w);
}

__global__ __launch_bounds__(256) void derive_params_kernel(const pnmn_derive_job* __restrict__ jobs) {
    const pnmn_derive_job jb = jobs[blockIdx.y];
    const int q = blockIdx.x * 256 + threadIdx.x;
    if (jb.kind == 2) {
        if (q * 4 < jb.n) {
            const float4 a = reinterpret_cast<const float4*>(jb.src)[q], b = reinterpret_cast<const float4*>(jb.src2)[q];
            reinterpret_cast<float4*>(jb.dst)[q] = float4{a.x + b.x, a.y + b.y, a.z + b.z, a.w + b.w};
        }
        return;
    }
    if ((size_t)q * 4 >= (size_t)jb.n * jb.k) return;
    const int r = q & 15, a = (q >> 4) & 3, kb = jb.k >> 4;
    const int j = (q >> 6) % kb, i = (q >> 6) / kb;
    const int x = 16 * i + r, y = 16 * j + 4 * a;
    float4 v;
    if (jb.kind == 0) {
        v = *reinterpret_cast<const float4*>(jb.src + (size_t)x * jb.ld + y);
    } else {
        v.x = jb.src[(size_t)(y + 0) * jb.ld + x];
        v.y = jb.src[(size_t)(y + 1) * jb.ld + x];
        v.z = jb.src[(size_t)(y + 2) * jb.ld + x];
        v.w = jb.src[(size_t)(y + 3) * jb.ld + x];
    }
    reinterpret_cast<float4*>(jb.dst)[q] = v;
}


typedef float f32x4 __attribute__((ext_vector_type(4)));

__device__ __forceinline__ f32x4 mfma4(const f32x4 a, const f32x4 b, f32x4 acc) {
    acc = __builtin_amdgcn_mfma_f32_16x16x4f32(a.x, b.x, acc, 0, 0, 0);
    acc = __builtin_amdgcn_mfma_f32_16x16x4f32(a.y, b.y, acc, 0, 0, 0);
    acc = __builtin_amdgcn_mfma_f32_16x16x4f32(a.z, b.z, acc, 0, 0, 0);
    acc = __builtin_amdgcn_mfma_f32_16x16x4f32(a.w, b.w, acc, 0, 0, 0);
    return acc;
}

__global__ __launch_bounds__(256) void token_table_fwd_kernel(const float* __restrict__ emb, const float* __restrict__ w, long ldw,
                                                              const float* __restrict__ bias, int V, int K, int N,
                                                              float* __restrict__ table) {
    const int wave = threadIdx.x >> 6, lane = threadIdx.x & 63, li = lane & 15, g = lane >> 4;
    const int n0 = 16 * blockIdx.x;
    const float* wrow = w + (size_t)(n0 + li) * ldw + 4 * g;
    const float b = bias ? bias[n0 + li] : 0.f;
    for (int mt = wave; 16 * mt < V; mt += 4) {
        const float* arow = emb + (size_t)min(16 * mt + li, V - 1) * K + 4 * g;
        f32x4 acc = f32x4{0.f, 0.f, 0.f, 0.f};
        for (int kb = 0; kb < K / 16; ++kb)
            acc = mfma4(*reinterpret_cast<const f32x4*>(arow + 16 * kb), *reinterpret_cast<const f32x4*>(wrow + 16 * kb), acc);
#pragma unroll
        for (int r = 0; r < 4; ++r) {
            const int v = 16 * mt + 4 * g + r;
            if (v < V) table[(size_t)v * N + n0 + li] = acc[r] + b;
        }
    }
}

__global__ __launch_bounds__(256) void token_table_bwd_kernel(const float* __restrict__ dtable, const float* __restrict__ emb,
                                                              const float* __restrict__ w, long ldw, int V, int K, int N,
                                                              int padding_idx, float* __restrict__ demb,
                                                              float* __restrict__ dw, long lddw, float* __restrict__ dbias,
                                                              float* __restrict__ dbias2) {
    __shared__ float lds[128 * 17];
    const int tid = threadIdx.x, wave = tid >> 6, lane = tid & 63, li = lane & 15, g = lane >> 4;
    const int V16 = (V + 15) & ~15;
    if ((int)blockIdx.x < N / 16) {
        const int n0 = 16 * blockIdx.x;
        for (int i = tid; i < V16 * 16; i += 256) {
            const int v = i >> 4, c = i & 15;
            lds[v * 17 + c] = v < V ? dtable[(size_t)v * N + n0 + c] : 0.f;
        }
        __syncthreads();
        if (dbias && tid < 16) {
            float sum = 0.f;
            for (int v = 0; v < V; ++v) sum += lds[v * 17 + tid];
            dbias[n0 + tid] = sum;
            if (dbias2) dbias2[n0 + tid] = sum;
        }
        if (!dw) return;
        for (int kt = wave; kt < K / 16; kt += 4) {
            f32x4 acc = f32x4{0.f, 0.f, 0.f, 0.f};
            for (int vb = 0; vb < V16 / 16; ++vb) {
                f32x4 a, b;
#pragma unroll
                for (int j = 0; j < 4; ++j) {
                    const int v = 16 * vb + 4 * g + j;
                    a[j] = lds[v * 17 + li];
                    b[j] = v < V ? emb[(size_t)v * K + 16 * kt + li] : 0.f;
                }
                acc = mfma4(a, b, acc);
            }
#pragma unroll
            for (int r = 0; r < 4; ++r) dw[(size_t)(n0 + 4 * g + r) * lddw + 16 * kt + li] = acc[r];
        }
        return;
    }
    if (!demb) return;
    const int tile = blockIdx.x - N / 16, mt = tile / (K / 16), kt = tile % (K / 16);
    const float* arow = dtable + (size_t)min(16 * mt + li, V - 1) * N + 4 * g;
    f32x4 acc = f32x4{0.f, 0.f, 0.f, 0.f};
    const int per = N / 4;
    for (int n = wave * per; n < (wave + 1) * per; n += 16) {
        f32x4 b;
#pragma unroll
        for (int j = 0; j < 4; ++j) b[j] = w[(size_t)(n + 4 * g + j) * ldw + 16 * kt + li];
        acc = mfma4(*reinterpret_cast<const f32x4*>(arow + n), b, acc);
    }
#pragma unroll
    for (int r = 0; r < 4; ++r) lds[(wave * 16 + 4 * g + r) * 17 + li] = acc[r];
    __syncthreads();
    {
        const int r = tid >> 4, c = tid & 15, v = 16 * mt + r;
        if (v < V) {
            const float sum = (lds[r * 17 + c] + lds[(16 + r) * 17 + c]) + (lds[(32 + r) * 17 + c] + lds[(48 + r) * 17 + c]);
            demb[(size_t)v * K + 16 * kt + c] = v == padding_idx ? 0.f : sum;
        }
    }
}

}

extern "C" int pnmn_token_prep(const int64_t* tokens, int64_t token_row_stride, int B, int T, int pad, int bos, int eos,
                               int drop_first, int64_t* out, float* fmask, int* last, void* stream) {
    if (B <= 0) return 0;
    if (!tokens || !out || T < 0) return PNMN_EINVAL;
    hipLaunchKernelGGL(token_prep_kernel, dim3((B + 3) / 4), dim3(256), 0, static_cast<hipStream_t>(stream), tokens,
                       token_row_stride, B, T, pad, bos, eos, drop_first, out, fmask, last);
    return (int)hipGetLastError();
}

extern "C" int pnmn_length_order(const int32_t* last, int B, int T, int32_t* order, int32_t* tile_steps, void* stream) {
    if (B <= 0) return 0;
    if (!last || !order || !tile_steps || T <= 0) return PNMN_EINVAL;
    if (T > LO_MAX_T) return PNMN_ESHAPE;
    hipLaunchKernelGGL(length_order_kernel, dim3(1), dim3(64), (size_t)(T + 1) * sizeof(int), static_cast<hipStream_t>(stream),
                       last, B, T, order, tile_steps);
    return (int)hipGetLastError();
}

extern "C" int pnmn_token_rows(const pnmn_token_seg* segs, int n_segs, int64_t* dst, int W, int64_t pad, void* stream) {
    if (n_segs <= 0 || W <= 0) return 0;
    if (!segs || !dst || n_segs > PNMN_TOKEN_SEGS) return PNMN_EINVAL;
    TokenSegs t;
    int total = 0;
    for (int k = 0; k < n_segs; ++k) {
        if (segs[k].rows < 0 || (segs[k].rows > 0 && !segs[k].src) || segs[k].width < 0) return PNMN_EINVAL;
        t.s[k] = segs[k];
        total += segs[k].rows;
    }
    t.n = n_segs;
    if (total == 0) return 0;
    hipLaunchKernelGGL(token_rows_kernel, dim3((total + 3) / 4), dim3(256), 0, static_cast<hipStream_t>(stream), t, dst, W, pad,
                       total);
    return (int)hipGetLastError();
}

extern "C" int pnmn_trim_predictions(const int64_t* raw, int B, int T, int end, int64_t* out, void* stream) {
    if (B <= 0 || T <= 0) return 0;
    if (!raw || !out) return PNMN_EINVAL;
    hipLaunchKernelGGL(trim_predictions_kernel, dim3((B + 3) / 4), dim3(256), 0, static_cast<hipStream_t>(stream), raw, B, T,
                       end, out);
    return (int)hipGetLastError();
}

extern "C" int pnmn_mask_last_fwd(const float* hs, const float* fmask, const int* last, int B, int T, int H, float* enc,
                                  float* hlast, void* stream) {
    if (B <= 0 || T <= 0) return 0;
    if (!hs || !fmask || !last || !enc || !hlast || (H & 3)) return PNMN_EINVAL;
    const int per_row = (T * (H >> 2) + 255) / 256;
    hipLaunchKernelGGL(mask_last_fwd_kernel, dim3(B, per_row < 8 ? per_row : 8), dim3(256), 0,
                       static_cast<hipStream_t>(stream), hs, fmask, last, T, H, enc, hlast);
    return (int)hipGetLastError();
}

extern "C" int pnmn_mask_last_bwd(const float* denc, const float* dhlast, const float* fmask, const int* last, int B, int T,
                                  int H, float* dhs, void* stream) {
    if (B <= 0 || T <= 0) return 0;
    if (!fmask || !last || !dhs || (H & 3)) return PNMN_EINVAL;
    const int per_row = (T * (H >> 2) + 255) / 256;
    hipLaunchKernelGGL(mask_last_bwd_kernel, dim3(B, per_row < 8 ? per_row : 8), dim3(256), 0,
                       static_cast<hipStream_t>(stream), denc, dhlast, fmask, last, T, H, dhs);
    return (int)hipGetLastError();
}

namespace {
constexpr int EG_SLICES = 8;
inline int eg_max_per(long rows, int V) { return (int)(((rows + EG_SLICES - 1) / EG_SLICES) / EG_CHUNK) + V; }
}

extern "C" int64_t pnmn_embedding_grad_workspace_bytes(int B, int T, int V) {
    if (B <= 0 || T <= 0 || V <= 0) return 0;
    const long rows = (long)B * T;
    return (int64_t)sizeof(int) * (rows + (long)EG_SLICES * (3 * eg_max_per(rows, V) + 1));
}

extern "C" int pnmn_embedding_grad(const float* dy, const int64_t* tokens, int64_t token_row_stride, int B, int T, int C,
                                   int V, int shift, int start, int skip, int accumulate, float* dw, void* workspace,
                                   void* stream) {
    if (V <= 0 || C <= 0) return 0;
    if (!dw || (C & 3) || V > 128) return PNMN_EINVAL;
    hipStream_t s = static_cast<hipStream_t>(stream);
    if (B <= 0 || T <= 0) return accumulate ? 0 : (int)hipMemsetAsync(dw, 0, sizeof(float) * (size_t)V * C, s);
    if (!dy || !tokens || !workspace) return PNMN_EINVAL;
    const long rows = (long)B * T;
    if (rows * T >= (1L << 32)) return PNMN_ESHAPE;
    const unsigned magic = T == 1 ? 0u : (unsigned)(((1ULL << 32) + T - 1) / T);
    const int max_per = eg_max_per(rows, V);
    int* order = static_cast<int*>(workspace);
    int* chunks = order + rows;
    int* count = chunks + 3 * (size_t)EG_SLICES * max_per;
    hipLaunchKernelGGL(embedding_rows_kernel, dim3(EG_SLICES), dim3(1024), 0, s, tokens, token_row_stride, B, T, magic, V, shift,
                       start, skip, C, order, chunks, max_per, count, dw, accumulate);
    hipLaunchKernelGGL(embedding_sum_kernel, dim3(EG_SLICES * max_per, (C + 1023) / 1024), dim3(256), 0, s, dy, order, chunks,
                       max_per, count, C, dw);
    return (int)hipGetLastError();
}

extern "C" int pnmn_derive_params(const pnmn_derive_job* jobs, int n_jobs, int max_quads, void* stream) {
    if (n_jobs <= 0) return 0;
    if (!jobs || max_quads <= 0) return PNMN_EINVAL;
    hipLaunchKernelGGL(derive_params_kernel, dim3((max_quads + 255) / 256, n_jobs), dim3(256), 0,
                       static_cast<hipStream_t>(stream), jobs);
    return (int)hipGetLastError();
}

extern "C" int pnmn_token_table_fwd(const float* emb, const float* weight, int64_t weight_row_stride, const float* bias, int V,
                                    int K, int N, float* table, void* stream) {
    if (V <= 0) return 0;
    if (!emb || !weight || !table) return PNMN_EINVAL;
    if (V > 128 || K < 16 || K % 16 || N < 64 || N % 64 || weight_row_stride % 4) return PNMN_ESHAPE;
    hipLaunchKernelGGL(token_table_fwd_kernel, dim3(N / 16), dim3(256), 0, static_cast<hipStream_t>(stream), emb, weight,
                       (long)weight_row_stride, bias, V, K, N, table);
    return (int)hipGetLastError();
}

extern "C" int pnmn_token_table_bwd(const float* dtable, const float* emb, const float* weight, int64_t weight_row_stride, int V,
                                    int K, int N, int padding_idx, float* demb, float* dweight, int64_t dweight_row_stride,
                                    float* dbias, float* dbias2, void* stream) {
    if (V <= 0) return 0;
    if (!dtable || !emb || !weight) return PNMN_EINVAL;
    if (V > 128 || K < 16 || K % 16 || N < 64 || N % 64) return PNMN_ESHAPE;
    const int blocks = N / 16 + (demb ? ((V + 15) / 16) * (K / 16) : 0);
    hipLaunchKernelGGL(token_table_bwd_kernel, dim3(blocks), dim3(256), 0, static_cast<hipStream_t>(stream), dtable, emb, weight,
                       (long)weight_row_stride, V, K, N, padding_idx, demb, dweight,
                       (long)(dweight_row_stride > 0 ? dweight_row_stride : K), dbias, dbias2);
    return (int)hipGetLastError();
}

namespace {
constexpr int DENC_H = 256, DENC_SB = 16, DENC_MAXT = 64;
__global__ __launch_bounds__(256) void attn_denc_kernel(const float* __restrict__ weights, const float* __restrict__ dscore,
                                                        const float* __restrict__ dctx, const float* __restrict__ hs,
                                                        const float* __restrict__ h0, float* __restrict__ denc, int T, int S) {
    __shared__ float wl[DENC_MAXT][DENC_SB], dl[DENC_MAXT][DENC_SB];
    const int b = blockIdx.x, s0 = blockIdx.y * DENC_SB, c = threadIdx.x;
    const int ns = (S - s0) < DENC_SB ? (S - s0) : DENC_SB;
    for (int i = threadIdx.x; i < T * DENC_SB; i += 256) {
        const int t = i / DENC_SB, s = i % DENC_SB;
        const bool ok = s < ns;
        wl[t][s] = ok ? weights[((size_t)b * T + t) * S + s0 + s] : 0.f;
        dl[t][s] = ok ? dscore[((size_t)b * T + t) * S + s0 + s] : 0.f;
    }
    __syncthreads();
    float acc[DENC_SB];
#pragma unroll
    for (int s = 0; s < DENC_SB; ++s) acc[s] = 0.f;
    const float* dc = dctx + (size_t)b * T * DENC_H + c;
    const float* hp = hs + (size_t)b * T * DENC_H + c;
    float hprev = h0[(size_t)b * DENC_H + c];
    for (int t = 0; t < T; ++t) {
        const float d = dc[(size_t)t * DENC_H];
        const float hnext = (t + 1 < T) ? hp[(size_t)t * DENC_H] : 0.f;
#pragma unroll
        for (int s = 0; s < DENC_SB; ++s) acc[s] += wl[t][s] * d + dl[t][s] * hprev;
        hprev = hnext;
    }
    for (int s = 0; s < ns; ++s) denc[((size_t)b * S + s0 + s) * DENC_H + c] = acc[s];
}
}

extern "C" int pnmn_attn_denc(const float* weights, const float* dscore, const float* dctx, const float* hs, const float* h0,
                              float* denc, int B, int T, int S, int hidden, void* stream) {
    if (B <= 0 || S <= 0) return 0;
    if (!weights || !dscore || !dctx || !hs || !h0 || !denc) return PNMN_EINVAL;
    if (hidden != DENC_H || T < 1 || T > DENC_MAXT) return PNMN_ESHAPE;
    hipLaunchKernelGGL(attn_denc_kernel, dim3(B, (S + DENC_SB - 1) / DENC_SB), dim3(256), 0, static_cast<hipStream_t>(stream),
                       weights, dscore, dctx, hs, h0, denc, T, S);
    return (int)hipGetLastError();
}
```

probnmn-clevr_amd/probnmn/_hip.py:

```python
import ctypes
import os
import re
import time
from typing import Dict, Optional

import numpy as np
import torch

_HERE = os.path.dirname(os.path.abspath(__file__))
LIB_PATH = os.environ.get("PNMN_LIB") or os.path.join(os.path.dirname(_HERE), "lib", "libprobnmn_hip.so")
HEADER_PATH = os.path.join(os.path.dirname(os.path.dirname(_HERE)), "include", "probnmn_hip.h")


class HipLibraryError(RuntimeError):
    pass


_lib: Optional[ctypes.CDLL] = None

_C_SCALARS = {
    "int": (ctypes.c_int, np.int32),
    "int32_t": (ctypes.c_int32, np.int32),
    "uint32_t": (ctypes.c_uint32, np.uint32),
    "int64_t": (ctypes.c_int64, np.int64),
# ... 29 lines not shown
        constants[m[1]] = int(m[2] or m[3])

    def record(body: str, name: str) -> np.dtype:
        fields = []
        for decl in filter(None, (d.strip() for d in body.split(";"))):
            words = re.sub(r"\bconst\b", " ", decl).replace("*", " * ").split(None, 1)
            declarators = [re.fullmatch(r"\s*(\*?)\s*(\w+)\s*(?:\[\s*(\w+)\s*\])?\s*", d) for d in words[-1].split(",")]
            if len(words) != 2 or None in declarators:
                raise HipLibraryError("probnmn_hip.h: cannot read the field `%s` of %s" % (decl, name))
            for star, field, length in (d.groups() for d in declarators):
                kind = np.uint64 if star else scalar(words[0], "%s; /* %s */" % (decl, name), 1)
                if length is None:
                    fields.append((field, kind))
                elif length.isdigit() or length in constants:
                    fields.append((field, kind, (int(length) if length.isdigit() else constants[length],)))
                else:
                    raise HipLibraryError("probnmn_hip.h: array length `%s` of `%s` in %s is neither a number nor a "
                                          "#define above it" % (length, decl, name))
        return np.dtype(fields, align=True)

    records: Dict[str, np.dtype] = {}
    for m in re.finditer(r"\btypedef\b(?:\s+struct\s*\w*\s*\{([^{}]*)\}\s*(pnmn_\w+)\s*;)?", text):
        if m[2] is None:
            raise HipLibraryError("probnmn_hip.h: cannot read the record at `%s`: a record is `typedef struct [tag] { ... } "
                                  "pnmn_x;`" % " ".join(text[m.start():m.start() + 60].split()))
        records[m[2]] = record(m[1], m[2])
    HOST_BLOCKS.update({m[1]: record(m[2], m[1]) for m in re.finditer(r"^[ \t]*struct\s+(pnmn_\w+)\s*\{([^{}]*)\}\s*;", text, flags=re.M)})

    signatures: Dict[str, tuple] = {}
    restypes = {}
    for m in re.finditer(r"^(int|int64_t)\s+(pnmn_\w+)\s*\(([^()]*)\)\s*;", text, flags=re.M):
        params = [p.strip() for p in m[3].split(",")]
        argtypes = []
        for p in [] if params in (["void"], [""]) else params:
            words = re.sub(r"\b(const|struct)\b", " ", p).split()
            if "*" in p:
                argtypes.append(ctypes.c_void_p)
            elif len(words) == 2:
                argtypes.append(scalar(words[0], "%s /* %s */" % (p, m[2]), 0))
            else:
                raise HipLibraryError("probnmn_hip.h: cannot read the parameter `%s` of %s" % (p, m[2]))
        signatures[m[2]] = tuple(argtypes)
        restypes[m[2]] = _C_SCALARS[m[1]][0]
    for m in re.finditer(r"\b(pnmn_\w+)\s*\(", text):
        if m[1] not in signatures:
            raise HipLibraryError("probnmn_hip.h: cannot read the declaration of %s: a prototype is `int` or `int64_t` at "
                                  "the start of a line, the name, the parameters, `);`" % m[1])
    return signatures, restypes, records, constants


SIGNATURES, RESTYPES, RECORDS, CONSTANTS = read_header()
globals().update({name[len("pnmn_"):].upper(): dtype for name, dtype in RECORDS.items()})
globals().update({name[len("pnmn_"):].upper(): dtype for name, dtype in HOST_BLOCKS.items()})
globals().update({name[len("PNMN_"):]: value for name, value in CONSTANTS.items()})
GEMM_A_T, GEMM_B_T, GEMM_ACC = (CONSTANTS["PNMN_GEMM_" + n] for n in ("A_TRANSPOSED", "B_TRANSPOSED", "ACCUMULATE"))
ABI_VERSION = CONSTANTS["PNMN_ABI_VERSION"]
ITEM_SIZES = {name: (dtype, dtype.itemsize) for name, dtype in RECORDS.items()}


def lib() -> ctypes.CDLL:
    global _lib
    if _lib is None:
        if not os.path.exists(LIB_PATH):
            raise HipLibraryError(
                "libprobnmn_hip.so not found at %s -- build it with `python -c 'import "
                "__graft_entry__ as g; g.build()'` (hipcc --offload-arch=gfx950); there is no "
                "fallback path" % LIB_PATH
            )
        handle = ctypes.CDLL(LIB_PATH)
        for name, argtypes in SIGNATURES.items():
            fn = getattr(handle, name)
            fn.restype = RESTYPES[name]
            fn.argtypes = list(argtypes)
        if handle.pnmn_abi_version() != ABI_VERSION:
            raise HipLibraryError("%s has ABI version %d, this package binds version %d -- rebuild the library"
                                  % (LIB_PATH, handle.pnmn_abi_version(), ABI_VERSION))
        _lib = handle
    return _lib


_TRACE = None


def check(code: int, what: str) -> None:
    if code != 0:
        kind = "argument/shape error" if code < 0 else "hipError_t"
        raise HipLibraryError("%s failed: %s %d" % (what, kind, code))
    if _TRACE is not None:
        stream = torch.cuda.current_stream()
        ev = torch.cuda.Event()
        ev.record(stream)
        _TRACE.append((what, stream.cuda_stream, ev))
        del _TRACE[:-4000]


def mark(what: str) -> None:
    if _TRACE is not None:
        check(0, "mark: " + what)


def _start_trace(seconds: float) -> None:
    import sys
    import threading

    global _TRACE
    _TRACE = []

    def watch():
        time.sleep(seconds)
        per_stream = {}
        for what, stream, ev in list(_TRACE):
            st = per_stream.setdefault(stream, {"done": None, "stuck": None, "pending": 0})
            if ev.query():
                if st["stuck"] is None:
                    st["done"] = what
            else:
                st["pending"] += 1
                if st["stuck"] is None:
                    st["stuck"] = what
        for stream, st in per_stream.items():
            print("[pnmn trace] stream %#x: last completed launch = %s; first incomplete = %s (%d launches pending)"
                  % (stream, st["done"], st["stuck"], st["pending"]), file=sys.stderr, flush=True)

    threading.Thread(target=watch, daemon=True).start()


if os.environ.get("PNMN_TRACE_LAUNCHES"):
    _start_trace(float(os.environ["PNMN_TRACE_LAUNCHES"]))


class LaunchList:

    def __init__(self):
        self._rows = []

    def add(self, op: int, n: int, a: int, b: int = 0, c: int = 0, p=()) -> None:
        q = tuple(p) + (0,) * (8 - len(p))
        self._rows.append((a, b, c, op | (n << 32), q[0] | (q[1] << 32), q[2] | (q[3] << 32), q[4] | (q[5] << 32),
                           q[6] | (q[7] << 32)))

    def __len__(self) -> int:
        return len(self._rows)

    def run(self, stream: int, what: str) -> None:
        if self._rows:
            rec = np.array(self._rows, dtype=np.uint64)
            check(lib().pnmn_run_launches(rec.ctypes.data, len(self._rows), stream), what)
            self._rows = []


def decoder_workspace_bytes(rows, backward: bool) -> int:
    r = np.asarray(rows, np.int32)
    return int(lib().pnmn_attn_lstm_group_workspace_bytes(r.ctypes.data, len(r), 1 if backward else 0))


def stream_ptr(device: torch.device) -> int:
    idx = device.index
    if idx is None:
        idx = torch.cuda.current_device()
    return torch._C._cuda_getCurrentRawStream(idx)


class _PinnedRing:

    SMALL, SMALL_SLOTS = 16 << 10, 64

    def __init__(self, slots: int = 6):
        self._bufs = [None] * slots
        self._events = [None] * slots
        self._next = 0
        self._small = None
        self._big = 16 << 20
        self._small_events = [None] * self.SMALL_SLOTS
        self._small_next = 0
        self.wait_seconds = 0.0

    def _wait(self, ev) -> None:
        if ev is not None and not ev.query():
            t0 = time.perf_counter()
            ev.synchronize()
            self.wait_seconds += time.perf_counter() - t0

    def stage(self, raw, device: torch.device, total: int = -1) -> torch.Tensor:
        pieces = None
        if total >= 0:
            pieces, n = raw, total
        else:
            n = raw.size
        if n <= self.SMALL:
            if self._small is None:
                self._small = torch.empty(self.SMALL * self.SMALL_SLOTS, dtype=torch.uint8).pin_memory()
            i = self._small_next
            self._small_next = (i + 1) % self.SMALL_SLOTS
            events, buf = self._small_events, self._small[i * self.SMALL:(i + 1) * self.SMALL]
        else:
            i = self._next
            self._next = (i + 1) % len(self._bufs)
            events, buf = self._events, self._bufs[i]
        self._wait(events[i])
        if buf is None or buf.numel() < n:
            while self._big < n:
                self._big *= 2
            buf = torch.empty(self._big, dtype=torch.uint8).pin_memory()
            self._bufs[i] = buf
        if pieces is None:
            buf.numpy()[:n] = raw
        else:
            view = buf.numpy()
            for off, piece in pieces:
                view[off:off + piece.size] = piece
        out = buf[:n].to(device, non_blocking=True)
        if events[i] is None:
            events[i] = torch.cuda.Event()
        events[i].record(torch.cuda.current_stream(device))
        return out


_rings: Dict[int, _PinnedRing] = {}


def _ring(device: torch.device) -> _PinnedRing:
    idx = device.index if device.index is not None else torch.cuda.current_device()
    r = _rings.get(idx)
    if r is None:
        r = _rings[idx] = _PinnedRing()
    return r


def ring_wait_seconds() -> float:
    return sum(r.wait_seconds for r in _rings.values())


def to_device(records: np.ndarray, device: torch.device) -> torch.Tensor:
    if device.type != "cuda":
        raise HipLibraryError("probnmn HIP kernels need a cuda (ROCm) device, got %s" % device)
    raw = np.ascontiguousarray(records).view(np.uint8).reshape(-1)
    return _ring(device).stage(raw, device)


def pieces_to_device(pieces, total: int, device: torch.device) -> torch.Tensor:
    if device.type != "cuda":
        raise HipLibraryError("probnmn HIP kernels need a cuda (ROCm) device, got %s" % device)
    return _ring(device).stage(pieces, device, total)


def small_to_device(values, dtype: torch.dtype, device: torch.device) -> torch.Tensor:
    host = torch.tensor(values, dtype=dtype)
    if host.numel() == 0:
        return torch.empty(0, dtype=dtype, device=device)
    raw = host.view(torch.uint8).numpy() if dtype != torch.bool else host.numpy().view(np.uint8)
    return to_device(raw, device).view(dtype)
```

probnmn-clevr_amd/probnmn/runtime/seq_plan.py:

```python
import os
from dataclasses import dataclass
from typing import Dict, List, NamedTuple, Optional

import numpy as np
import torch

from probnmn import _hip


SPLIT_SLOTS = int(os.environ.get("PNMN_PLAN_SPLIT_SLOTS", "512"))
SPLIT_MIN_KTILES = int(os.environ.get("PNMN_PLAN_SPLIT_MIN", "8"))
USE_STACK = True
STACK_FWD_ENCODERS = int(os.environ.get("PNMN_PLAN_FWD_ENC", "2"))
STACK_PG_ENCODER = int(os.environ.get("PNMN_PLAN_PG_ENC", "1"))
STACK_BWD_ENCODERS = int(os.environ.get("PNMN_PLAN_BWD_ENC", "0"))
LENGTH_ORDER_ABOVE_ROWS = 256
DECODER_BUFFERS = (("hs", 256), ("cs", 256), ("cx", 256), ("act", 1024), ("dhs", 256), ("dg", 1024), ("dctx", 256))


class PlanUnsupported(Exception):
    """The models / shapes are outside what the plan is built for: the trainer keeps the eager passes."""


class _Calls(list):
    def add(self, name: str, *args) -> None:
        self.append((getattr(_hip.lib(), name), args, name))

    def add_fn(self, name: str, fn) -> None:
        self.append((fn, (), name))

    def run(self) -> None:
        for fn, args, name in self:
            rc = fn(*args)
            if rc:
                _hip.check(rc, name)


def _supported(model) -> bool:
    lstm, cell = model._encoder._module, model._decoder_cell
    return (lstm.hidden_size == 256 and lstm.num_layers == 2 and lstm.input_size == 256 and cell.hidden_size == 256
            and cell.input_size == 512 and model._output_projection_layer.weight.size(0) <= 128
            and model._source_embedder.embedding.weight.size(0) <= 128)


def _dropout_p(lstm) -> float:
    return float(lstm.dropout) if lstm.num_layers > 1 else 0.0


class _Model:

    def __init__(self, model, dev):
        self.model = model
        lstm, cell, proj = model._encoder._module, model._decoder_cell, model._output_projection_layer
        self.emb_src, self.emb_tgt = model._source_embedder.embedding.weight, model._target_embedder.weight
        self.lstm, self.cell, self.proj = lstm, cell, proj
        self.params = [self.emb_src] + [getattr(lstm, "%s_l%d" % (n, layer)) for layer in (0, 1)
                                        for n in ("weight_ih", "weight_hh", "bias_ih", "bias_hh")] \
            + [self.emb_tgt, cell.weight_ih, cell.weight_hh, cell.bias_ih, cell.bias_hh, proj.weight, proj.bias]
        for p in self.params:
            if not p.is_contiguous() or p.device != dev or p.dtype != torch.float32:
                raise PlanUnsupported("parameter layout")
        offs, total = [], 0
        for p in self.params:
            offs.append(total)
            total += (p.numel() + 63) // 64 * 64
        self.gflat = torch.zeros(total, dtype=torch.float32, device=dev)
        self.grads = [self.gflat[o:o + p.numel()].view(p.shape) for o, p in zip(offs, self.params)]
        self.g = {id(p): g for p, g in zip(self.params, self.grads)}
        self.signature = tuple(p.data_ptr() for p in self.params)
        self.derived = model._derived()

    def grad(self, p) -> torch.Tensor:
        return self.g[id(p)]

    def attach(self) -> None:
        for p, g in zip(self.params, self.grads):
            p.grad = g


class _TokenTable(NamedTuple):
    tag: str
    emb: torch.Tensor
    w_ih: torch.Tensor
    col0: int
    b_ih: torch.Tensor
    b_hh: torch.Tensor
    bias: torch.Tensor
    pad_idx: int
    table: torch.Tensor


class _Loss(NamedTuple):
    logits: torch.Tensor
    ld: int
    target: int
    target_stride: int
    mask: int
    mask_stride: int
    pad: int
    loss: torch.Tensor
    lse: torch.Tensor
    rows: int
    T: int
    V: int
    eps: float

    def _head(self):
        return (self.logits.data_ptr(), self.ld, self.target, self.target_stride, self.mask, self.mask_stride, self.pad)

    def forward(self, calls: _Calls, stream: int) -> None:
        calls.add("pnmn_seq_nll_fwd", *self._head(), self.loss.data_ptr(), self.lse.data_ptr(), self.rows, self.T, self.V,
                  self.eps, stream)

    def backward(self, calls: _Calls, dloss: torch.Tensor, dlogits: torch.Tensor, stream: int) -> None:
        calls.add("pnmn_seq_nll_bwd", *self._head(), self.lse.data_ptr(), dloss.data_ptr(), dlogits.data_ptr(), self.ld,
                  self.rows, self.T, self.V, self.eps, stream)


@dataclass
class _DecoderPass:
    tag: str
    rows: int
    T: int
    S: int
    row0: int
    enc_row0: int
    tokens: torch.Tensor
    shift: int
    trimmed: Optional[torch.Tensor]
    v: Dict[str, torch.Tensor]
    loss: _Loss


@dataclass
class _DecoderSet:
    tag: str
    mm: _Model
    enc: Dict
    table: _TokenTable
    flat: Dict[str, torch.Tensor]
    logits: torch.Tensor
    dlogits: torch.Tensor
    passes: List[_DecoderPass]


class _EncoderPass(NamedTuple):
    tag: str
    mm: Optional[_Model]
    embedding: torch.nn.Embedding
    tokens: torch.Tensor
    width: int
    rows: int
    drop_first: bool = True
    want_last: bool = True
    p: float = 0.0


class Seq2SeqPlan:

    def __init__(self, pg, qr, prior, dev: torch.device, n: int, m: int, tq: int, tp: int):
        if not (_supported(pg) and _supported(qr)) or n <= 0 or m <= 0:
            raise PlanUnsupported("model shapes")
        pl = prior._encoder._module
        if pl.hidden_size != 256 or pl.num_layers != 2 or pl.input_size != 256:
            raise PlanUnsupported("prior shapes")
        if pl.training and _dropout_p(pl) > 0:
            raise PlanUnsupported("prior in training mode with dropout")
        self.dev, self.n, self.m, self.tq, self.tp = dev, n, m, tq, tp
        self.stream = _hip.stream_ptr(dev)
        self.pg, self.qr, self.prior = _Model(pg, dev), _Model(qr, dev), prior
        self.drop_p = (_dropout_p(pg._encoder._module), _dropout_p(qr._encoder._module))
        self.B, self.D = n + m, pg._max_decoding_steps
        if _hip.decoder_workspace_bytes([n, m], False) <= 0 or _hip.decoder_workspace_bytes([self.B], False) <= 0 \
                or int(_hip.lib().pnmn_lstm_seq_workspace_bytes(self.B, 0)) <= 0:
            raise PlanUnsupported("batch does not fit the multi-CU recurrent kernels in one launch")
        self._bufs: Dict[str, torch.Tensor] = {}
        self._keep: List = []
        self.anchor = torch.zeros((), device=dev, requires_grad=True)
        self.fwd_pg_enc, self.fwd_pg, self.fwd_pg_finish, self.fwd_qr, self.fwd_prior = (_Calls() for _ in range(5))
        self.bwd_a, self.bwd_b = _Calls(), _Calls()
        self._build()

    def buf(self, name: str, *shape, dtype=torch.float32, zero: bool = False) -> torch.Tensor:
        if name in self._bufs:
            raise KeyError(name)
        t = (torch.zeros if zero else torch.empty)(*shape, dtype=dtype, device=self.dev)
        self._bufs[name] = t
        return t

    def bytes_buf(self, name: str, nbytes: int, zero: bool = False) -> torch.Tensor:
        return self.buf(name, max(int(nbytes), 16), dtype=torch.uint8, zero=zero)

    def __getitem__(self, name: str) -> torch.Tensor:
        return self._bufs[name]

    def _gemm(self, calls: _Calls, name: str, descs) -> None:
        lib = _hip.lib()
        for lo in range(0, len(descs), _hip.GEMM_MAX):
            part = descs[lo:lo + _hip.GEMM_MAX]
            rec = np.zeros(len(part), _hip.GEMM_DESC)
            tiles = [((d["M"] + 127) // 128) * ((d["N"] + 127) // 128) for d in part]
            ktiles = [(d["K"] + 31) // 32 for d in part]
            auto = [i for i, d in enumerate(part) if d.get("split") == "auto"]
            fixed_units = sum(t for i, t in enumerate(tiles) if i not in auto)
            chunk_len, best = SPLIT_MIN_KTILES, None
            for cand in range(SPLIT_MIN_KTILES, 129):
                splits = [max(1, min(-(-ktiles[i] // cand), 64)) for i in auto]
                units = fixed_units + sum(tiles[i] * sp for i, sp in zip(auto, splits))
                longest = max([-(-ktiles[i] // sp) for i, sp in zip(auto, splits)] + [ktiles[i] for i in range(len(part)) if i not in auto] + [1])
                rounds = units // SPLIT_SLOTS + (0.6 if units % SPLIT_SLOTS else 0.0)
                cost = rounds * longest + 4.0 * sum(tiles[i] * sp for i, sp in zip(auto, splits) if sp > 1) / SPLIT_SLOTS
                if best is None or cost < best:
                    chunk_len, best = cand, cost
            for i, d in enumerate(part):
                r = rec[i]
                r["a"], r["b"], r["c"] = d["a"], d["b"], d["c"]
                r["lda"], r["ldb"], r["ldc"] = d["lda"], d["ldb"], d["ldc"]
                r["M"], r["N"], r["K"] = d["M"], d["N"], d["K"]
                r["flags"] = (_hip.GEMM_A_T if d.get("ta") else 0) | (_hip.GEMM_B_T if d.get("tb") else 0) | (_hip.GEMM_ACC if d.get("acc") else 0)
                r["bias"] = d.get("bias", 0)
                split = d.get("split", 1)
                if split == "auto":
                    split = max(1, min(-(-ktiles[i] // chunk_len), 64))
                r["split_k"] = split
                if split > 1:
                    ws = self.bytes_buf("%s.ws%d" % (name, lo + i), lib.pnmn_gemm_workspace_bytes(d["M"], d["N"], split), zero=True)
                    r["workspace"] = ws.data_ptr()
                r["shift_t"], r["shift_h0"], r["ld_h0"] = d.get("shift_t", 0), d.get("h0", 0), d.get("ld_h0", 0)
                r["colsum"], r["colsum2"] = d.get("colsum", 0), d.get("colsum2", 0)
            self._keep.append(rec)
            calls.add("pnmn_gemm_cus", rec.ctypes.data, len(rec), 0, self.stream)

    def _table_forward(self, calls: _Calls, t: _TokenTable) -> None:
        calls.add("pnmn_token_table_fwd", t.emb.data_ptr(), t.w_ih.data_ptr() + 4 * t.col0, t.w_ih.stride(0), t.bias.data_ptr(),
                  t.emb.size(0), 256, 1024, t.table.data_ptr(), self.stream)

    def _table_backward(self, calls: _Calls, t: _TokenTable, mm: _Model, start: int, uses) -> None:
        V, g = t.emb.size(0), mm.grad
        dtable = self.buf(t.tag + ".dtable", V, 1024)
        for k, (ws_name, dg, tokens, shift) in enumerate(uses):
            rows, T = dg.shape[:2]
            ews = self.bytes_buf(ws_name, _hip.lib().pnmn_embedding_grad_workspace_bytes(rows, T, V))
            calls.add("pnmn_embedding_grad", dg.data_ptr(), tokens.data_ptr(), tokens.stride(0), rows, T, 1024, V, shift, start, -1,
                      1 if k else 0, dtable.data_ptr(), ews.data_ptr(), self.stream)
        ld = t.w_ih.stride(0)
        calls.add("pnmn_token_table_bwd", dtable.data_ptr(), t.emb.data_ptr(), t.w_ih.data_ptr() + 4 * t.col0, ld, V, 256, 1024, t.pad_idx,
                  g(t.emb).data_ptr(), g(t.w_ih).data_ptr() + 4 * t.col0, ld if ld != 256 else 0, g(t.b_ih).data_ptr(),
                  g(t.b_hh).data_ptr(), self.stream)

    def _encoder_prepare(self, calls: _Calls, ep: _EncoderPass) -> Dict:
        model, derived = (ep.mm.model, ep.mm.derived) if ep.mm is not None else (self.prior, self.prior._derived())
        tag, rows, lstm, emb, f = ep.tag, ep.rows, model._encoder._module, ep.embedding.weight, self.buf
        T, V = ep.width + 2 - int(ep.drop_first), emb.size(0)
        e = dict(tag=tag, mm=ep.mm, derived=derived, lstm=lstm, T=T, rows=rows, want_last=ep.want_last,
                 src=f(tag + ".src", rows, T, dtype=torch.long), fmask=f(tag + ".fmask", rows, T), last=f(tag + ".last", rows, dtype=torch.int32),
                 table=f(tag + ".table", V, 1024), hs1=f(tag + ".hs1", rows, T, 256), cs1=f(tag + ".cs1", rows, T, 256),
                 act1=f(tag + ".act1", rows, T, 1024), hs2=f(tag + ".hs2", rows, T, 256), cs2=f(tag + ".cs2", rows, T, 256),
                 act2=f(tag + ".act2", rows, T, 1024), p=ep.p, seed=0, row_offset=0, drop_recs=[])
        e["tab"] = _TokenTable(tag, emb, lstm.weight_ih_l0, 0, lstm.bias_ih_l0, lstm.bias_hh_l0, derived["l0.b"],
                               -1 if ep.embedding.padding_idx is None else ep.embedding.padding_idx, e["table"])
        if ep.p > 0:
            e["hsd"] = f(tag + ".hsd", rows, T, 256)
        calls.add("pnmn_token_prep", ep.tokens.data_ptr(), ep.tokens.stride(0), rows, ep.width, model._pad_index, model._start_index,
                  model._end_index, int(ep.drop_first), e["src"].data_ptr(), e["fmask"].data_ptr(), e["last"].data_ptr(), self.stream)
        if rows > LENGTH_ORDER_ABOVE_ROWS and os.environ.get("PNMN_LSTM_LENGTH_ORDER", "1") != "0":
            e["order"], e["tile_steps"] = f(tag + ".order", rows, dtype=torch.int32), f(tag + ".tile_steps", (rows + 15) // 16, dtype=torch.int32)
            calls.add("pnmn_length_order", e["last"].data_ptr(), rows, T, e["order"].data_ptr(), e["tile_steps"].data_ptr(), self.stream)
        self._table_forward(calls, e["tab"])
        if ep.want_last:
            e["enc"], e["h"] = f(tag + ".enc", rows, T, 256), f(tag + ".h", rows, 256)
        return e

    def _stack_jobs(self, encs: List[Dict], backward: bool) -> np.ndarray:
        jobs = np.zeros(2 * len(encs), _hip.LSTM_STACK_JOB)
        for k, e in enumerate(encs):
            d = e["derived"]
            a, b = jobs[2 * k], jobs[2 * k + 1]
            if not backward:
                a["xp"], a["tokens"], a["token_stride"], a["w_hh"] = e["table"].data_ptr(), e["src"].data_ptr(), e["src"].stride(0), d["l0.hh"].data_ptr()
                a["hs"], a["cs"], a["act"], a["dep"] = e["hs1"].data_ptr(), e["cs1"].data_ptr(), e["act1"].data_ptr(), -1
                b["w_hh"], b["w_ih"], b["bias"] = d["l1.hh"].data_ptr(), d["l1.ih"].data_ptr(), d["l1.b"].data_ptr()
                b["hs"], b["cs"], b["act"], b["dep"] = e["hs2"].data_ptr(), e["cs2"].data_ptr(), e["act2"].data_ptr(), 2 * k
            else:
                a["dhs"], a["act"], a["cs"], a["w_hh"], a["dgates"], a["dep"] = (e["dhs2"].data_ptr(), e["act2"].data_ptr(), e["cs2"].data_ptr(),
                                                                                 d["l1.hhT"].data_ptr(), e["dg2"].data_ptr(), -1)
                b["act"], b["cs"], b["w_hh"], b["w_ih"], b["dgates"], b["dep"] = (e["act1"].data_ptr(), e["cs1"].data_ptr(), d["l0.hhT"].data_ptr(),
                                                                                 d["l1.ihT"].data_ptr(), e["dg1"].data_ptr(), 2 * k)
            for j in (a, b):
                j["B"], j["T"] = e["rows"], e["T"]
        return jobs

    def _stack_launches(self, calls: _Calls, name: str, encs: List[Dict], backward: bool, most: Optional[int] = None) -> List[Dict]:
        lib, left, group = _hip.lib(), [], []
        if most is None:
            most = STACK_BWD_ENCODERS if backward else STACK_FWD_ENCODERS
        use = USE_STACK and most > 0 and all("l1.ih" in e["derived"] for e in encs)

        def flush():
            if not group:
                return
            jobs = self._stack_jobs(group, backward)
            ws = self.bytes_buf("%s.stack_ws%d" % (name, len(self._keep)), lib.pnmn_lstm_stack_workspace_bytes(jobs.ctypes.data, len(jobs), int(backward)))
            self._keep.append(jobs)
            if any(e["p"] > 0 for e in group):
                drops = np.zeros(len(jobs), _hip.LSTM_DROPOUT_DESC)
                for k, e in enumerate(group):
                    if e["p"] > 0:
                        i = 2 * k + int(backward)
                        drops[i]["p"] = e["p"]
                        if not backward:
                            drops[i]["hsd"] = e["hsd"].data_ptr()
                        e["drop_recs"].append((drops, i))
                self._keep.append(drops)
                calls.add("pnmn_lstm_stack_bwd_dropout" if backward else "pnmn_lstm_stack_fwd_dropout", jobs.ctypes.data, drops.ctypes.data,
                          len(jobs), ws.data_ptr(), self.stream)
            else:
                calls.add("pnmn_lstm_stack_bwd" if backward else "pnmn_lstm_stack_fwd", jobs.ctypes.data, len(jobs), ws.data_ptr(), self.stream)
            del group[:]

        for e in encs:
            if not use:
                left.append(e)
                continue
            trial = self._stack_jobs(group + [e], backward)
            if len(group) < most and 2 * (len(group) + 1) <= _hip.LSTM_STACK_JOBS and int(lib.pnmn_lstm_stack_workspace_bytes(trial.ctypes.data, len(trial), int(backward))) > 0:
                group.append(e)
                continue
            flush()
            alone = self._stack_jobs([e], backward)
            if int(lib.pnmn_lstm_stack_workspace_bytes(alone.ctypes.data, 2, int(backward))) > 0:
                group.append(e)
            else:
                left.append(e)
        flush()
        return left

    def _dropout_call(self, calls: _Calls, e: Dict, src: torch.Tensor, dst: torch.Tensor) -> None:
        fn, st = _hip.lib().pnmn_lstm_dropout, self.stream
        x, y, rows, T, p = src.data_ptr(), dst.data_ptr(), e["rows"], e["T"], e["p"]
        calls.add_fn("pnmn_lstm_dropout", lambda: fn(x, y, rows, T, 256, p, e["seed"], e["row_offset"], st))

    def _set_dropout(self, e: Dict, seed: int, row_offset: int) -> None:
        e["seed"], e["row_offset"] = seed, row_offset
        for rec, i in e["drop_recs"]:
            rec[i]["seed"], rec[i]["row_offset"] = seed, row_offset

    def _encoders_fwd(self, calls: _Calls, name: str, encs: List[Dict], most: Optional[int] = None) -> None:
        lib, st = _hip.lib(), self.stream
        for e in self._stack_launches(calls, name, encs, False, most):
            d, lstm, rows, T = e["derived"], e["lstm"], e["rows"], e["T"]
            xp2 = self.buf(e["tag"] + ".xp2", rows, T, 1024)
            ws = self.bytes_buf(e["tag"] + ".lstm_ws", lib.pnmn_lstm_seq_workspace_bytes(rows, 0))
            fwd, ordered = ("pnmn_lstm_seq_fwd_ordered", (e["order"].data_ptr(), e["tile_steps"].data_ptr())) if "order" in e else ("pnmn_lstm_seq_fwd", ())
            calls.add(fwd, e["table"].data_ptr(), e["src"].data_ptr(), e["src"].stride(0), d["l0.hh"].data_ptr(),
                      e["hs1"].data_ptr(), e["cs1"].data_ptr(), e["act1"].data_ptr(), rows, T, 256, *ordered, ws.data_ptr(), st)
            x2 = e["hs1"]
            if e["p"] > 0:
                self._dropout_call(calls, e, e["hs1"], e["hsd"])
                x2 = e["hsd"]
            self._gemm(calls, e["tag"] + ".xp2g", [dict(a=x2.data_ptr(), b=lstm.weight_ih_l1.data_ptr(), c=xp2.data_ptr(), M=rows * T,
                                                        N=1024, K=256, lda=256, ldb=256, ldc=1024, tb=1, bias=d["l1.b"].data_ptr())])
            calls.add(fwd, xp2.data_ptr(), None, 0, d["l1.hh"].data_ptr(), e["hs2"].data_ptr(), e["cs2"].data_ptr(),
                      e["act2"].data_ptr(), rows, T, 256, *ordered, ws.data_ptr(), st)
        for e in encs:
            if e["want_last"]:
                calls.add("pnmn_mask_last_fwd", e["hs2"].data_ptr(), e["fmask"].data_ptr(), e["last"].data_ptr(), e["rows"], e["T"], 256,
                          e["enc"].data_ptr(), e["h"].data_ptr(), st)

    def _encoders_bwd(self, calls: _Calls, name: str, encs: List[Dict]) -> None:
        lib, st = _hip.lib(), self.stream
        f = self.buf
        for e in encs:
            tag, rows, T = e["tag"], e["rows"], e["T"]
            e["dhs2"], e["dg2"], e["dg1"] = f(tag + ".dhs2", rows, T, 256), f(tag + ".dg2", rows, T, 1024), f(tag + ".dg1", rows, T, 1024)
            calls.add("pnmn_mask_last_bwd", e["denc"].data_ptr(), e["dh"].data_ptr(), e["fmask"].data_ptr(), e["last"].data_ptr(), rows, T, 256,
                      e["dhs2"].data_ptr(), st)
        for e in self._stack_launches(calls, name, encs, True):
            d, lstm, tag, rows, T = e["derived"], e["lstm"], e["tag"], e["rows"], e["T"]
            dhs1 = f(tag + ".dhs1", rows, T, 256)
            ws = self.bytes_buf(tag + ".lstm_bws", lib.pnmn_lstm_seq_workspace_bytes(rows, 1))
            bwd, ordered = ("pnmn_lstm_seq_bwd_ordered", (e["order"].data_ptr(), e["tile_steps"].data_ptr())) if "order" in e else ("pnmn_lstm_seq_bwd", ())
            calls.add(bwd, e["dhs2"].data_ptr(), e["act2"].data_ptr(), e["cs2"].data_ptr(), d["l1.hhT"].data_ptr(),
                      e["dg2"].data_ptr(), rows, T, 256, *ordered, ws.data_ptr(), st)
            self._gemm(calls, tag + ".dx", [dict(a=e["dg2"].data_ptr(), b=lstm.weight_ih_l1.data_ptr(), c=dhs1.data_ptr(), M=rows * T, N=256,
                                                 K=1024, lda=1024, ldb=256, ldc=256, split="auto")])
            if e["p"] > 0:
                self._dropout_call(calls, e, dhs1, dhs1)
            calls.add(bwd, dhs1.data_ptr(), e["act1"].data_ptr(), e["cs1"].data_ptr(), d["l0.hhT"].data_ptr(),
                      e["dg1"].data_ptr(), rows, T, 256, *ordered, ws.data_ptr(), st)

    def _encoders_param_grads(self, calls: _Calls, deferred: List, encs: List[Dict]) -> None:
        for e in encs:
            mm, lstm, rows, T = e["mm"], e["lstm"], e["rows"], e["T"]
            dg1, dg2, g = e["dg1"], e["dg2"], mm.grad
            self._table_backward(calls, e["tab"], mm, 0, [(e["tag"] + ".emb_ws", dg1, e["src"], 0)])
            K = rows * T
            deferred += [
                dict(a=dg2.data_ptr(), b=e["hs2"].data_ptr(), c=g(lstm.weight_hh_l1).data_ptr(), M=1024, N=256, K=K, lda=1024, ldb=256,
                     ldc=256, ta=1, split="auto", shift_t=T, colsum=g(lstm.bias_ih_l1).data_ptr(), colsum2=g(lstm.bias_hh_l1).data_ptr()),
                dict(a=dg2.data_ptr(), b=(e["hsd"] if e["p"] > 0 else e["hs1"]).data_ptr(), c=g(lstm.weight_ih_l1).data_ptr(), M=1024,
                     N=256, K=K, lda=1024, ldb=256, ldc=256, ta=1, split="auto"),
                dict(a=dg1.data_ptr(), b=e["hs1"].data_ptr(), c=g(lstm.weight_hh_l0).data_ptr(), M=1024, N=256, K=K, lda=1024, ldb=256,
                     ldc=256, ta=1, split="auto", shift_t=T),
            ]

    def _decoder_set(self, tag: str, mm: _Model, enc: Dict, passes) -> _DecoderSet:
        f, S, V = self.buf, enc["T"], mm.proj.weight.size(0)
        R = sum(rows * T for _, _, rows, T, _, _ in passes)
        table = _TokenTable(tag + ".d", mm.emb_tgt, mm.cell.weight_ih, 256, mm.cell.bias_ih, mm.cell.bias_hh, mm.derived["d.b"], -1,
                            f(tag + ".d.table", V, 1024))
        dec = _DecoderSet(tag, mm, enc, table, {k: f("%s.d.%s" % (tag, k), R, w) for k, w in DECODER_BUFFERS},
                          f(tag + ".logits", R, V), f(tag + ".dlogits", R, V), [])
        row0 = enc_row0 = 0
        for ptag, suffix, rows, T, tokens, trimmed in passes:
            v = {k: dec.flat[k][row0:row0 + rows * T].view(rows, T, w) for k, w in DECODER_BUFFERS}
            for k in ("probs", "dscore", "weights"):
                v[k] = f("%s.%s" % (ptag, k), rows, T, S)
            target = tokens.data_ptr() + (0 if trimmed is not None else 8)
            loss = _Loss(dec.logits[row0:], T * V, target, tokens.stride(0), target if trimmed is None else trimmed.data_ptr(),
                         tokens.stride(0), mm.model._pad_index, f("%s.loss%s" % (tag, suffix), rows), f("%s.lse%s" % (tag, suffix), rows, T),
                         rows, T, V, 1e-13 if trimmed is None else 1e-12)
            dec.passes.append(_DecoderPass(ptag, rows, T, S, row0, enc_row0, tokens, int(trimmed is not None), trimmed, v, loss))
            row0, enc_row0 = row0 + rows * T, enc_row0 + rows
        return dec

    def _decoder_fwd_job(self, j, dec: _DecoderSet, p: _DecoderPass) -> None:
        e, r0, mm = dec.enc, p.enc_row0, dec.mm
        j["etable"], j["enc"], j["mask"], j["h0"] = dec.table.table.data_ptr(), e["enc"][r0:].data_ptr(), e["fmask"][r0:].data_ptr(), e["h"][r0:].data_ptr()
        j["w_c"], j["w_hh"] = mm.derived["d.c"].data_ptr(), mm.derived["d.hh"].data_ptr()
        j["hs"], j["cs"], j["act"], j["ctx"], j["probs"] = (p.v[k].data_ptr() for k in ("hs", "cs", "act", "cx", "probs"))
        j["B"], j["T"], j["S"], j["start_index"] = p.rows, p.T, p.S, mm.model._start_index
        if p.trimmed is None:
            j["in_tokens"], j["in_token_stride"] = p.tokens.data_ptr(), p.tokens.stride(0)
        else:
            j["w_p"], j["b_p"], j["tokens"], j["V"], j["sample"] = mm.proj.weight.data_ptr(), mm.proj.bias.data_ptr(), p.tokens.data_ptr(), mm.proj.weight.size(0), 1
            j["pad_index"], j["unk_index"] = mm.model._pad_index, mm.model._unk_index

    def _decoder_forward(self, calls: _Calls, dec: _DecoderSet, source: torch.Tensor, tgt: torch.Tensor, ws_name: str) -> np.ndarray:
        model, rows = dec.mm.model, [p.rows for p in dec.passes]
        calls.add("pnmn_token_prep", source.data_ptr(), source.stride(0), source.size(0), source.size(1), model._pad_index, model._start_index,
                  model._end_index, 0, tgt.data_ptr(), None, None, self.stream)
        self._table_forward(calls, dec.table)
        jobs = np.zeros(len(dec.passes), _hip.DECODER_FWD_JOB)
        for j, p in zip(jobs, dec.passes):
            self._decoder_fwd_job(j, dec, p)
        ws = self.bytes_buf(ws_name, _hip.decoder_workspace_bytes(rows, False))
        calls.add("pnmn_attn_lstm_fwd_group", jobs.ctypes.data, len(jobs), 256, ws.data_ptr(), self.stream)
        return jobs

    def _decoder_losses(self, calls: _Calls, dec: _DecoderSet) -> None:
        proj, (R, V) = dec.mm.proj, dec.logits.shape
        self._gemm(calls, dec.tag + ".logits_g", [dict(a=dec.flat["hs"].data_ptr(), b=proj.weight.data_ptr(), c=dec.logits.data_ptr(), M=R, N=V,
                                                       K=256, lda=256, ldb=256, ldc=V, tb=1, bias=proj.bias.data_ptr())])
        for p in dec.passes:
            p.loss.forward(calls, self.stream)

    def _build(self) -> None:
        if self.pg.derived is None or self.qr.derived is None or self.prior._derived() is None:
            raise PlanUnsupported("derived parameters")
        self._generator_encoder()
        dec_pg = self._generator_decoders()
        self._decoder_losses(self.fwd_pg_finish, dec_pg)
        e_pr = self._reconstructor_encoder()
        dec_qr = self._reconstructor_decoder()
        self._prior_loss(e_pr)
        self._backward_chain([dec_pg, dec_qr])
        self._parameter_gradients([dec_pg, dec_qr])
        self.out.update(loss_s=dec_pg.passes[0].loss.loss, loss_t=dec_pg.passes[1].loss.loss, loss_q=dec_qr.passes[0].loss.loss)
        self._derived_sig = self._sig()

    def _generator_encoder(self) -> None:
        pg, f = self.pg, self.buf
        self.out = dict(ques=f("ques", self.B, self.tq, dtype=torch.long), prog_sup=f("prog_sup", self.m, self.tp, dtype=torch.long))
        self.e_pg = self._encoder_prepare(self.fwd_pg_enc, _EncoderPass(
            "pg.e", pg, pg.model._source_embedder.embedding, self.out["ques"], self.tq, self.B, p=self.drop_p[0]))
        self._encoders_fwd(self.fwd_pg_enc, "pg.e", [self.e_pg], most=STACK_PG_ENCODER)
        stacked = any(name.startswith("pnmn_lstm_stack_fwd") for _, _, name in self.fwd_pg_enc)
        self.pg_encoder_workgroups = 16 * (-(-self.B // 16)) if stacked else 0
        if self.e_pg["T"] > 64 or self.D > 64:
            raise PlanUnsupported("more than 64 source positions / decoding steps")

    def _generator_decoders(self) -> _DecoderSet:
        n, m, D, tp, f = self.n, self.m, self.D, self.tp, self.buf
        tgt, raw, z = f("pg.tgt", m, tp + 2, dtype=torch.long), f("pg.raw", n, D, dtype=torch.long), f("pg.z", n, D, dtype=torch.long)
        dec = self._decoder_set("pg", self.pg, self.e_pg, [("pg.s", "_s", n, D, raw, z), ("pg.t", "_t", m, tp + 1, tgt, None)])
        self.pair_jobs = self._decoder_forward(self.fwd_pg, dec, self.out["prog_sup"], tgt, "pg.pair_ws")
        self.fwd_pg.add("pnmn_trim_predictions", raw.data_ptr(), n, D, self.pg.model._end_index, z.data_ptr(), self.stream)
        self.out.update(z=z, raw=raw)
        return dec

    def _reconstructor_encoder(self) -> Dict:
        n, m, D, tp, qr, pr, c = self.n, self.m, self.D, self.tp, self.qr, self.prior, self.fwd_qr
        z, Wq = self.out["z"], max(D, tp)
        source = self.buf("qr.source", self.B, Wq, dtype=torch.long)
        segs = np.zeros(2, _hip.TOKEN_SEG)
        segs[0]["src"], segs[0]["row_stride"], segs[0]["rows"], segs[0]["width"] = z.data_ptr(), D, n, D
        segs[1]["src"], segs[1]["row_stride"], segs[1]["rows"], segs[1]["width"] = self.out["prog_sup"].data_ptr(), tp, m, tp
        self._keep.append(segs)
        c.add("pnmn_token_rows", segs.ctypes.data, 2, source.data_ptr(), Wq, 0, self.stream)
        self.e_qr = self._encoder_prepare(c, _EncoderPass(
            "qr.e", qr, qr.model._source_embedder.embedding, source, Wq, self.B, p=self.drop_p[1]))
        e_pr = self._encoder_prepare(c, _EncoderPass("pr.e", None, pr._embedder.embedding, z, D, n, drop_first=False, want_last=False))
        self._encoders_fwd(c, "qr.e", [self.e_qr, e_pr])
        if self.e_qr["T"] > 64 or self.tq + 1 > 64:
            raise PlanUnsupported("more than 64 positions in the reconstructor")
        return e_pr

    def _reconstructor_decoder(self) -> _DecoderSet:
        tgt = self.buf("qr.tgt", self.B, self.tq + 2, dtype=torch.long)
        dec = self._decoder_set("qr", self.qr, self.e_qr, [("qr.q", "", self.B, self.tq + 1, tgt, None)])
        self._keep.append(self._decoder_forward(self.fwd_qr, dec, self.out["ques"], tgt, "qr.dec_ws"))
        self._decoder_losses(self.fwd_qr, dec)
        return dec

    def _prior_loss(self, e_pr: Dict) -> None:
        n, pr, c, f = self.n, self.prior, self.fwd_prior, self.buf
        emb, src, Tz, Vz = pr._embedder.embedding.weight, e_pr["src"], e_pr["T"], pr._embedder.embedding.weight.size(0)
        proj, plog = f("pr.proj", n * Tz, 256), f("pr.logits", n * Tz, Vz)
        self._gemm(c, "pr.proj_g", [dict(a=e_pr["hs2"].data_ptr(), b=pr._projection_layer.weight.data_ptr(), c=proj.data_ptr(), M=n * Tz,
                                         N=256, K=256, lda=256, ldb=256, ldc=256, tb=1)])
        self._gemm(c, "pr.out_g", [dict(a=proj.data_ptr(), b=emb.data_ptr(), c=plog.data_ptr(), M=n * Tz, N=Vz, K=256, lda=256, ldb=256,
                                        ldc=Vz, tb=1)])
        loss = _Loss(plog, Tz * Vz, src.data_ptr() + 8, src.stride(0), src.data_ptr() + 8, src.stride(0), pr._pad_index,
                     f("pr.loss", n), f("pr.lse", n, Tz - 1), n, Tz - 1, Vz, 1e-13)
        loss.forward(c, self.stream)
        self.out["loss_p"] = loss.loss
        self.prior_sig = tuple(p.data_ptr() for p in pr.parameters())

    def _backward_chain(self, decs: List[_DecoderSet]) -> None:
        c, f, st = self.bwd_a, self.buf, self.stream
        passes = [(dec, p) for dec in decs for p in dec.passes]
        self.d_rows = {key: f("d.loss_" + key, p.rows) for key, (_, p) in zip("stq", passes)}
        for dloss, (dec, p) in zip(self.d_rows.values(), passes):
            p.loss.backward(c, dloss, dec.dlogits[p.row0:], st)
        self._gemm(c, "dhs_g", [dict(a=dec.dlogits.data_ptr(), b=dec.mm.proj.weight.data_ptr(), c=dec.flat["dhs"].data_ptr(), M=dec.logits.size(0),
                                     N=256, K=dec.logits.size(1), lda=dec.logits.size(1), ldb=256, ldc=256) for dec in decs])
        for dec in decs:
            dec.enc["denc"], dec.enc["dh"] = f(dec.tag + ".denc", *dec.enc["enc"].shape), f(dec.tag + ".dh", *dec.enc["h"].shape)
        bj = np.zeros(len(passes), _hip.DECODER_BWD_JOB)
        for j, (dec, p) in zip(bj, passes):
            e, r0 = dec.enc, p.enc_row0
            j["dhs"], j["act"], j["cs"], j["hs"], j["probs"] = (p.v[k].data_ptr() for k in ("dhs", "act", "cs", "hs", "probs"))
            j["enc"], j["mask"], j["h0"] = e["enc"][r0:].data_ptr(), e["fmask"][r0:].data_ptr(), e["h"][r0:].data_ptr()
            j["w_c_t"], j["w_hh_t"] = dec.mm.derived["d.cT"].data_ptr(), dec.mm.derived["d.hhT"].data_ptr()
            j["dgates"], j["dctx"], j["dscore"], j["weights"] = (p.v[k].data_ptr() for k in ("dg", "dctx", "dscore", "weights"))
            j["dh0"] = e["dh"][r0:].data_ptr()
            j["B"], j["T"], j["S"] = p.rows, p.T, p.S
        self._keep.append(bj)
        gws = self.bytes_buf("group_ws", _hip.decoder_workspace_bytes([p.rows for _, p in passes], True))
        c.add("pnmn_attn_lstm_bwd_group", bj.ctypes.data, len(bj), 256, gws.data_ptr(), st)
        for dec, p in passes:
            c.add("pnmn_attn_denc", p.v["weights"].data_ptr(), p.v["dscore"].data_ptr(), p.v["dctx"].data_ptr(), p.v["hs"].data_ptr(),
                  dec.enc["h"][p.enc_row0:].data_ptr(), dec.enc["denc"][p.enc_row0:].data_ptr(), p.rows, p.T, p.S, 256, st)
        self._encoders_bwd(self.bwd_b, "enc", [dec.enc for dec in decs])

    def _parameter_gradients(self, decs: List[_DecoderSet]) -> None:
        c, deferred = self.bwd_b, []
        for dec in decs:
            mm, flat, (R, V), g, cell = dec.mm, dec.flat, dec.logits.shape, dec.mm.grad, dec.mm.cell
            self._table_backward(c, dec.table, mm, mm.model._start_index,
                                 [("%s.d.emb_ws%d" % (dec.tag, k), p.v["dg"], p.tokens, p.shift) for k, p in enumerate(dec.passes)])
            deferred.append(dict(a=dec.dlogits.data_ptr(), b=flat["hs"].data_ptr(), c=g(mm.proj.weight).data_ptr(), M=V, N=256, K=R, lda=V,
                                 ldb=256, ldc=256, ta=1, split="auto", colsum=g(mm.proj.bias).data_ptr()))
            deferred.append(dict(a=flat["dg"].data_ptr(), b=flat["cx"].data_ptr(), c=g(cell.weight_ih).data_ptr(), M=1024, N=256, K=R, lda=1024,
                                 ldb=256, ldc=512, ta=1, split="auto"))
            for k, p in enumerate(dec.passes):
                deferred.append(dict(a=p.v["dg"].data_ptr(), b=p.v["hs"].data_ptr(), c=g(cell.weight_hh).data_ptr(), M=1024, N=256,
                                     K=p.rows * p.T, lda=1024, ldb=256, ldc=256, ta=1, split="auto", shift_t=p.T,
                                     h0=dec.enc["h"][p.enc_row0:].data_ptr(), ld_h0=256, acc=1 if k else 0))
        self._encoders_param_grads(c, deferred, [dec.enc for dec in decs])
        self._gemm(c, "wgrad", [d for d in deferred if not d.get("acc")])
        self._gemm(c, "wgrad2", [d for d in deferred if d.get("acc")])

    def _sig(self):
        return tuple(t.data_ptr() for model in (self.pg.model, self.qr.model, self.prior) for t in model._derived().values())

    def still_valid(self) -> bool:
        if _hip.stream_ptr(self.dev) != self.stream:
            return False
        for mm in (self.pg, self.qr):
            if tuple(p.data_ptr() for p in mm.params) != mm.signature:
                return False
        if tuple(p.data_ptr() for p in self.prior.parameters()) != self.prior_sig:
            return False
        if (_dropout_p(self.pg.lstm), _dropout_p(self.qr.lstm)) != self.drop_p:
            return False
        if self.prior.training and _dropout_p(self.prior._encoder._module) > 0:
            return False
        return self._sig() == self._derived_sig

    def run_encoder(self, question: torch.Tensor, program: torch.Tensor, nosup_d: torch.Tensor, sup_d: torch.Tensor) -> None:
        lib, st = _hip.lib(), self.stream
        if question.dtype != torch.long or program.dtype != torch.long or question.stride(1) != 1 or program.stride(1) != 1:
            raise _hip.HipLibraryError("token matrices must be int64 with contiguous rows")
        segs = np.zeros(2, _hip.TOKEN_SEG)
        segs[0]["src"], segs[0]["index"], segs[0]["row_stride"], segs[0]["rows"], segs[0]["width"] = \
            question.data_ptr(), nosup_d.data_ptr(), question.stride(0), self.n, self.tq
        segs[1]["src"], segs[1]["index"], segs[1]["row_stride"], segs[1]["rows"], segs[1]["width"] = \
            question.data_ptr(), sup_d.data_ptr(), question.stride(0), self.m, self.tq
        _hip.check(lib.pnmn_token_rows(segs.ctypes.data, 2, self.out["ques"].data_ptr(), self.tq, 0, st), "token_rows")
        segs[0]["src"], segs[0]["index"], segs[0]["row_stride"], segs[0]["rows"], segs[0]["width"] = \
            program.data_ptr(), sup_d.data_ptr(), program.stride(0), self.m, self.tp
        _hip.check(lib.pnmn_token_rows(segs.ctypes.data, 1, self.out["prog_sup"].data_ptr(), self.tp, 0, st), "token_rows")
        if self.drop_p[0] > 0:
            self._set_dropout(self.e_pg, int(torch.randint(0, 2 ** 62, (1,)).item()), self.pg.model.sample_row_offset)
        seed = int(torch.randint(0, 2 ** 62, (1,)).item())
        torch.randint(0, 2 ** 62, (1,))
        if self.drop_p[1] > 0:
            self._set_dropout(self.e_qr, int(torch.randint(0, 2 ** 62, (1,)).item()), self.qr.model.sample_row_offset)
        torch.randint(0, 2 ** 62, (1,))
        self.pair_jobs[0]["seed"] = seed
        self.pair_jobs[0]["row_offset"] = self.pg.model.sample_row_offset
        self.fwd_pg_enc.run()

    def run_decoders(self) -> torch.Tensor:
        self.fwd_pg.run()
        return self.out["z"]

    def run_generator_finish(self) -> None:
        self.fwd_pg_finish.run()

    def run_reconstructor(self) -> None:
        self.fwd_qr.run()

    def run_prior(self) -> torch.Tensor:
        self.fwd_prior.run()
        return self.out["loss_p"]

    def losses(self):
        return _PlanNode.apply(self.anchor, self)

    def backward(self, d_s, d_t, d_q) -> None:
        for key, d in (("s", d_s), ("t", d_t), ("q", d_q)):
            if d is None:
                self.d_rows[key].zero_()
            else:
                self.d_rows[key].copy_(d)
        self.bwd_a.run()
        self.bwd_b.run()
        self.pg.attach()
        self.qr.attach()


class _PlanNode(torch.autograd.Function):
    @staticmethod
    def forward(ctx, anchor, plan: Seq2SeqPlan):
        ctx.plan = plan
        o = plan.out
        return o["loss_s"].view_as(o["loss_s"]), o["loss_t"].view_as(o["loss_t"]), o["loss_q"].view_as(o["loss_q"])

    @staticmethod
    def backward(ctx, d_s, d_t, d_q):
        ctx.plan.backward(d_s, d_t, d_q)
        return None, None
```

Baseline: 37860 questions/s.

## Length-order decoder rows and stop each tile at its longest sequence

The attention-LSTM decoder forward and backward kernels gain an ordered variant. It sorts rows by sequence length and runs each 16-row tile only for that tile's maximum step count, zero-filling hs and ctx for the skipped steps. This removes recurrent steps spent on padding in teacher-forced and sampled-then-trained passes. Separately, the embedding gradient is restructured into column chunks with per-slice partial sums. The changes add token_last and length_order launches plus indirect row indexing, and they rely on tile_steps being correct for every row.

```diff
diff --git a/include/probnmn_hip.h b/include/probnmn_hip.h
--- a/include/probnmn_hip.h
+++ b/include/probnmn_hip.h
@@ -157,6 +157,8 @@
 int pnmn_token_prep(const int64_t* tokens, int64_t token_row_stride, int B, int T, int pad, int bos, int eos,
                     int drop_first, int64_t* out, float* fmask, int* last, void* stream);
 int pnmn_length_order(const int32_t* last, int B, int T, int32_t* order, int32_t* tile_steps, void* stream);
+int pnmn_token_last(const int64_t* tokens, int64_t token_row_stride, int B, int T, int pad, int extra, int32_t* last,
+                    void* stream);
 int pnmn_trim_predictions(const int64_t* raw, int B, int T, int end, int64_t* out, void* stream);
 int pnmn_mask_last_fwd(const float* hs, const float* fmask, const int* last, int B, int T, int H, float* enc,
                        float* hlast, void* stream);
@@ -279,6 +281,12 @@
 int64_t pnmn_attn_lstm_group_workspace_bytes(const int32_t* rows, int n, int backward);
 int pnmn_attn_lstm_fwd_group(const pnmn_decoder_fwd_job* jobs, int n, int hidden, void* workspace, void* stream);
 int pnmn_attn_lstm_bwd_group(const pnmn_decoder_bwd_job* jobs, int n, int hidden, void* workspace, void* stream);
+int pnmn_attn_lstm_fwd_group_ordered(const pnmn_decoder_fwd_job* jobs, const int32_t* const* order ,
+                                     const int32_t* const* tile_steps , int n, int hidden, void* workspace,
+                                     void* stream);
+int pnmn_attn_lstm_bwd_group_ordered(const pnmn_decoder_bwd_job* jobs, const int32_t* const* order ,
+                                     const int32_t* const* tile_steps , int n, int hidden, void* workspace,
+                                     void* stream);
 int pnmn_attn_denc(const float* weights, const float* dscore, const float* dctx, const float* hs, const float* h0,
                    float* denc, int B, int T, int S, int hidden, void* stream);
 
diff --git a/probnmn-clevr_amd/csrc/decoder_multi.hip b/probnmn-clevr_amd/csrc/decoder_multi.hip
--- a/probnmn-clevr_amd/csrc/decoder_multi.hip
+++ b/probnmn-clevr_amd/csrc/decoder_multi.hip
@@ -53,14 +53,29 @@
     uint64_t seed, row_offset;
 };
 
+struct RowOrder {
+    const int32_t* order;
+    const int32_t* tile_steps;
+};
+__device__ __forceinline__ int slot_row(const int32_t* __restrict__ order, int slot, int B) {
+    slot = min(slot, B - 1);
+    return order ? order[slot] : slot;
+}
+__device__ __forceinline__ int tile_step_count(const int32_t* __restrict__ tile_steps, int tile, int T) {
+    return tile_steps ? min(max(tile_steps[tile], 1), T) : T;
+}
+constexpr size_t ORDER_LDS = sizeof(int) * ROWS;
+
 constexpr size_t FWD_FIXED_LDS = sizeof(float) * (4 * ROWS * GLD + RW * 4 * H + ROWS * MAXV + RW * MAXS) + sizeof(int) * ROWS;
 constexpr size_t FWD_OVERLAP_LDS = sizeof(float) * (ROWS * H + 64);
 
-template <bool OVERLAP, bool SAMPLE, bool FILT = false, bool CONSTR = false>
+template <bool OVERLAP, bool SAMPLE, bool FILT = false, bool CONSTR = false, bool ORD = false>
 __device__ __forceinline__ void attn_lstm_fwd_multi_body(const MFwdArgs& a, const int tile, const int part,
                                                          const pnmn::SamplingFilter& f = pnmn::SamplingFilter{1.f, 0, 1.f},
-                                                         const pnmn::TokenAutomaton* aut = nullptr) {
+                                                         const pnmn::TokenAutomaton* aut = nullptr,
+                                                         const RowOrder ro = RowOrder{nullptr, nullptr}) {
     static_assert(SAMPLE || !CONSTR, "the automaton constrains the free-running modes only");
+    static_assert(!SAMPLE || !ORD, "a free-running pass takes no order: a row's step count is not known before it has run");
     extern __shared__ __attribute__((aligned(16))) char raw[];
     const int T = a.T, S = a.S;
     float* encl = reinterpret_cast<float*>(raw);
@@ -71,16 +86,25 @@
     float (*logl)[MAXV] = reinterpret_cast<float (*)[MAXV]>(&cpart[RW][0][0]);
     float* hst = &logl[ROWS][0];
     float* sink = hst + ROWS * H;
+    int* ordl = reinterpret_cast<int*>(OVERLAP ? sink + 64 : hst);
 
     const int tid = threadIdx.x, wave = tid >> 6, lane = tid & 63, li = lane & 15, g = lane >> 4;
     const int row0 = tile * ROWS, myrow0 = row0 + RW * part, u0 = UW * part;
+    const int steps = ORD ? tile_step_count(ro.tile_steps, tile, T) : T;
+    int erow[RW] = {0, 0}, my_brow = 0;
+    if constexpr (ORD) {
+#pragma unroll
+        for (int r = 0; r < RW; ++r) erow[r] = slot_row(ro.order, myrow0 + r, a.B);
+        my_brow = __builtin_amdgcn_readfirstlane((wave >> 2) ? erow[1] : erow[0]);
+    }
     pnmn::Cluster cl;
     cl.start(a.sync + tile * pnmn::CLUSTER_COUNTER_STRIDE, MEMBERS);
 
     for (int i = tid; i < RW * S * (H / 4); i += 512) {
         const int rl = i / (S * (H / 4)), rem = i - rl * S * (H / 4);
         f32x4 v = f32x4{0.f, 0.f, 0.f, 0.f};
-        if (myrow0 + rl < a.B) v = *reinterpret_cast<const f32x4*>(a.enc + (size_t)(myrow0 + rl) * S * H + 4 * rem);
+        if (myrow0 + rl < a.B)
+            v = *reinterpret_cast<const f32x4*>(a.enc + (size_t)(ORD ? (rl ? erow[1] : erow[0]) : myrow0 + rl) * S * H + 4 * rem);
         *reinterpret_cast<f32x4*>(encl + (size_t)rl * S * H + 4 * rem) = v;
     }
     const int gate = wave >> 1, ub = wave & 1;
@@ -95,15 +119,19 @@
         }
     }
     if (tid < ROWS) tokl[tid] = a.start;
-    const float row_mask = lane < S ? a.mask[(size_t)min(myrow0 + (wave >> 2), a.B - 1) * S + lane] : 0.f;
+    const float row_mask = lane < S ? a.mask[(size_t)(ORD ? my_brow : min(myrow0 + (wave >> 2), a.B - 1)) * S + lane] : 0.f;
     float creg = 0.f;
     const int arow = min(row0 + li, a.B - 1);
-    const int64_t* tf_row = (a.in_tokens && tid < ROWS) ? a.in_tokens + (size_t)min(row0 + tid, a.B - 1) * a.in_stride : nullptr;
+    const int64_t* tf_row = (a.in_tokens && tid < ROWS)
+                                ? a.in_tokens + (size_t)(ORD ? slot_row(ro.order, row0 + tid, a.B) : min(row0 + tid, a.B - 1)) * a.in_stride
+                                : nullptr;
     if (tf_row) tokl[tid] = (int)tf_row[0];
+    if constexpr (ORD)
+        if (tid < ROWS) ordl[tid] = slot_row(ro.order, row0 + tid, a.B);
 
     constexpr int PARTF = ROWS * 64;
     const int s_row = tid >> 5, s_q = tid & 31;
-    const int s_rowc = min(row0 + s_row, a.B - 1);
+    const int s_rowc = ORD ? slot_row(ro.order, row0 + s_row, a.B) : min(row0 + s_row, a.B - 1);
     const int s_off = (s_q >> 4) * PARTF + s_row * 64 + 4 * ((s_q & 15) ^ s_row);
     auto frags = [&](const float* tile_lds, const int p, f32x4 (&f)[4]) {
 #pragma unroll
@@ -136,7 +164,7 @@
     if constexpr (CONSTR) au = pnmn::stage_automaton(reinterpret_cast<unsigned char*>(OVERLAP ? sink + 64 : hst), *aut);
     __syncthreads();
 
-    for (int t = 0; t < T; ++t) {
+    for (int t = 0; t < steps; ++t) {
         int zt = 0;
         asm volatile("" : "+v"(zt));
         f32x4 acc;
@@ -147,13 +175,17 @@
                 const int rl = 4 * g + r, row = row0 + rl + zt;
                 const int n = gate * H + u0 + 16 * ub + li;
                 float v = 0.f;
-                if (row < a.B) v = a.xe ? a.xe[((size_t)row * T + t) * G4 + n] : a.etable[(size_t)tokl[rl] * G4 + n];
+                if constexpr (ORD) {
+                    if (row < a.B) v = a.xe ? a.xe[((size_t)ordl[rl] * T + t) * G4 + n] : a.etable[(size_t)tokl[rl] * G4 + n];
+                } else {
+                    if (row < a.B) v = a.xe ? a.xe[((size_t)row * T + t) * G4 + n] : a.etable[(size_t)tokl[rl] * G4 + n];
+                }
                 acc[r] = v;
             }
         };
         {
             const int rl = wave >> 2, q = wave & 3;
-            const int row = myrow0 + rl + zt, rowc = min(row, a.B - 1);
+            const int row = myrow0 + rl + zt, rowc = ORD ? my_brow : min(row, a.B - 1);
             f32x4 hv;
             if constexpr (OVERLAP) {
                 const int r = RW * part + rl;
@@ -216,7 +248,7 @@
                 const float wgt = qv / (wsum(qv) + 1e-13f);
                 if (lane < S) {
                     scl[rl][lane] = wgt;
-                    if (row < a.B) a.probs[((size_t)row * T + t) * S + lane] = p;
+                    if (row < a.B) a.probs[((size_t)(ORD ? my_brow : row) * T + t) * S + lane] = p;
                 }
             };
             if constexpr (OVERLAP) {
@@ -256,7 +288,7 @@
             __syncthreads();
             const int rl2 = tid >> 8, k = tid & 255;
             const float cv = (cpart[rl2][0][k] + cpart[rl2][1][k]) + (cpart[rl2][2][k] + cpart[rl2][3][k]);
-            if (myrow0 + rl2 < a.B) a.ctx[((size_t)(myrow0 + rl2 + zt) * T + t) * H + k] = cv;
+            if (myrow0 + rl2 < a.B) a.ctx[((size_t)(ORD ? my_brow : myrow0 + rl2 + zt) * T + t) * H + k] = cv;
         }
         cl.signal();
         cl.wait();
@@ -283,7 +315,7 @@
             constexpr int NB = 4, NPARTS = (H / 16) / NB, PART = 2 * ROWS * 64;
             float* stage = &cpart[0][0][0];
             const int s_tensor = tid >> 8, o_row = (tid >> 4) & 15, o_slot = tid & 15;
-            const int o_rowc = min(row0 + o_row, a.B - 1);
+            const int o_rowc = ORD ? ordl[o_row] : min(row0 + o_row, a.B - 1);
             const float* s_src = (s_tensor == 0 ? a.ctx + ((size_t)o_rowc * T + t) * H
                                                 : (t > 0 ? a.hs + ((size_t)o_rowc * T + (t - 1)) * H : a.h0 + (size_t)o_rowc * H)) + 4 * o_slot;
             float* s_dst = stage + (s_tensor * ROWS + o_row) * 64 + 4 * (o_slot ^ o_row);
@@ -323,10 +355,11 @@
             const float h = og * tanhf(c);
             creg = c;
             if (row < a.B) {
-                const size_t o = ((size_t)row * T + t) * H + u;
+                const int brow = ORD ? s_rowc : row;
+                const size_t o = ((size_t)brow * T + t) * H + u;
                 a.hs[o] = h;
                 a.cs[o] = c;
-                float* ar = a.act + ((size_t)row * T + t) * G4;
+                float* ar = a.act + ((size_t)brow * T + t) * G4;
                 ar[u] = ig;
                 ar[H + u] = fg;
                 ar[2 * H + u] = gg;
@@ -334,7 +367,7 @@
             }
         }
         if (tf_row) tokl[tid] = tf_next;
-        if (t + 1 == T && !SAMPLE) break;
+        if (t + 1 == steps && !SAMPLE) break;
         cl.signal();
         cl.wait();
         if constexpr (OVERLAP) {
@@ -402,6 +435,13 @@
             __syncthreads();
         }
     }
+    if constexpr (ORD) {
+        const int rl = tid >> 5, rl2 = tid >> 8;
+        for (int t = steps; t < T; ++t) {
+            if (row0 + rl < a.B) a.hs[((size_t)s_rowc * T + t) * H + u0 + (tid & 31)] = 0.f;
+            if (myrow0 + rl2 < a.B) a.ctx[((size_t)my_brow * T + t) * H + (tid & 255)] = 0.f;
+        }
+    }
     cl.finish();
 }
 
@@ -426,6 +466,30 @@
         tile -= tiles0;
         if (tile >= a1.tiles) return;
         attn_lstm_fwd_multi_body<OVERLAP, SAMPLE1>(a1, tile, part);
+    }
+}
+
+template <bool OVERLAP>
+__global__ __launch_bounds__(512) __attribute__((amdgpu_waves_per_eu(2, 2))) void attn_lstm_fwd_multi_ordered_kernel(const MFwdArgs a,
+                                                                                                                    const RowOrder ro) {
+    int tile, part;
+    pnmn::cluster_coords<MEMBERS>(tile, part);
+    if (tile >= a.tiles) return;
+    attn_lstm_fwd_multi_body<OVERLAP, false, false, false, true>(a, tile, part, pnmn::SamplingFilter{1.f, 0, 1.f}, nullptr, ro);
+}
+
+template <bool OVERLAP, bool SAMPLE0, bool SAMPLE1>
+__global__ __launch_bounds__(512) __attribute__((amdgpu_waves_per_eu(2, 2))) void attn_lstm_fwd_pair_ordered_kernel(
+    const MFwdArgs a0, const MFwdArgs a1, const int tiles0, const RowOrder ro0, const RowOrder ro1) {
+    int tile, part;
+    pnmn::cluster_coords<MEMBERS>(tile, part);
+    if (tile < tiles0) {
+        if (tile >= a0.tiles) return;
+        attn_lstm_fwd_multi_body<OVERLAP, SAMPLE0, false, false, !SAMPLE0>(a0, tile, part, pnmn::SamplingFilter{1.f, 0, 1.f}, nullptr, ro0);
+    } else {
+        tile -= tiles0;
+        if (tile >= a1.tiles) return;
+        attn_lstm_fwd_multi_body<OVERLAP, SAMPLE1, false, false, !SAMPLE1>(a1, tile, part, pnmn::SamplingFilter{1.f, 0, 1.f}, nullptr, ro1);
     }
 }
 
@@ -503,7 +567,9 @@
 constexpr int DLD = 4 * UW + 4;
 constexpr size_t BWD_FIXED_LDS = sizeof(float) * (ROWS * DLD + 2 * RW * H + 2 * RW * MAXS + RW * 4 * H + 64);
 
-__device__ __forceinline__ void attn_lstm_bwd_multi_body(const MBwdArgs& a, const int tile, const int part) {
+template <bool ORD = false>
+__device__ __forceinline__ void attn_lstm_bwd_multi_body(const MBwdArgs& a, const int tile, const int part,
+                                                         const RowOrder ro = RowOrder{nullptr, nullptr}) {
     extern __shared__ __attribute__((aligned(16))) char raw[];
     const int T = a.T, S = a.S;
     float* encl = reinterpret_cast<float*>(raw);
@@ -516,6 +582,13 @@
 
     const int tid = threadIdx.x, wave = tid >> 6, lane = tid & 63, li = lane & 15, g = lane >> 4;
     const int row0 = tile * ROWS, myrow0 = row0 + RW * part, u0 = UW * part;
+    const int steps = ORD ? tile_step_count(ro.tile_steps, tile, T) : T;
+    int erow[RW] = {0, 0}, my_brow = 0;
+    if constexpr (ORD) {
+#pragma unroll
+        for (int r = 0; r < RW; ++r) erow[r] = slot_row(ro.order, myrow0 + r, a.B);
+        my_brow = __builtin_amdgcn_readfirstlane((wave >> 2) ? erow[1] : erow[0]);
+    }
     pnmn::Cluster cl;
     cl.start(a.sync + tile * pnmn::CLUSTER_COUNTER_STRIDE, MEMBERS);
     float* x1t = a.x1 + (size_t)tile * 2 * MEMBERS * 2 * ROWS * H;
@@ -524,7 +597,8 @@
     for (int i = tid; i < RW * S * (H / 4); i += 512) {
         const int rl = i / (S * (H / 4)), rem = i - rl * S * (H / 4);
         f32x4 v = f32x4{0.f, 0.f, 0.f, 0.f};
-        if (myrow0 + rl < a.B) v = *reinterpret_cast<const f32x4*>(a.enc + (size_t)(myrow0 + rl) * S * H + 4 * rem);
+        if (myrow0 + rl < a.B)
+            v = *reinterpret_cast<const f32x4*>(a.enc + (size_t)(ORD ? (rl ? erow[1] : erow[0]) : myrow0 + rl) * S * H + 4 * rem);
         *reinterpret_cast<f32x4*>(encl + (size_t)rl * S * H + 4 * rem) = v;
     }
     constexpr int KB = 4 * UW / 16;
@@ -540,7 +614,7 @@
             wh[nt][kl] = *reinterpret_cast<const f32x4*>(a.w_hh_t + fo);
         }
     float dc_rec = 0.f;
-    const float row_mask = lane < S ? a.mask[(size_t)min(myrow0 + (wave >> 2), a.B - 1) * S + lane] : 0.f;
+    const float row_mask = lane < S ? a.mask[(size_t)(ORD ? my_brow : min(myrow0 + (wave >> 2), a.B - 1)) * S + lane] : 0.f;
     __syncthreads();
 
     struct Saved {
@@ -548,12 +622,13 @@
     };
     const int c_rl = tid >> 5, c_ul = tid & 31;
     const int c_row = row0 + c_rl, c_u = u0 + c_ul;
-    const int p_row = min(myrow0 + (wave >> 2), a.B - 1);
+    const int c_brow = ORD ? slot_row(ro.order, c_row, a.B) : c_row;
+    const int p_row = ORD ? my_brow : min(myrow0 + (wave >> 2), a.B - 1);
     auto load_saved = [&](int t) {
         Saved v{0.f, 0.f, 0.f, 0.f, 0.f, 0.f, 0.f, 0.f};
         if (c_row < a.B) {
-            const size_t o = ((size_t)c_row * T + t) * H + c_u;
-            const float* ar = a.act + ((size_t)c_row * T + t) * G4;
+            const size_t o = ((size_t)c_brow * T + t) * H + c_u;
+            const float* ar = a.act + ((size_t)c_brow * T + t) * G4;
             v.ig = ar[c_u], v.fg = ar[H + c_u], v.gg = ar[2 * H + c_u], v.og = ar[3 * H + c_u];
             v.c = a.cs[o];
             v.cp = t > 0 ? a.cs[o - H] : 0.f;
@@ -562,7 +637,7 @@
         if ((wave & 3) == 0 && lane < S) v.p = a.probs[((size_t)p_row * T + t) * S + lane];
         return v;
     };
-    Saved sv = load_saved(T - 1);
+    Saved sv = load_saved(steps - 1);
 
     auto dg_frag = [&](const int kl) { return *reinterpret_cast<const f32x4*>(&dgl[li][kl * 16 + 4 * g]); };
     auto mfma16 = [&](const f32x4 (&w)[2][KB], const int kl0, f32x4 (&acc)[2]) {
@@ -579,7 +654,7 @@
         }
     };
 
-    for (int t = T - 1; t >= 0; --t) {
+    for (int t = steps - 1; t >= 0; --t) {
         const Saved cur = sv;
         int zt = 0;
         asm volatile("" : "+v"(zt));
@@ -593,7 +668,7 @@
                 const float cp = cur.cp;
                 const float tc = tanhf(c);
                 float dhp = 0.f;
-                if (t < T - 1) {
+                if (t < steps - 1) {
                     const float* ph = x1t + (((size_t)((t + 1) & 1) * MEMBERS) * 2 + 1) * ROWS * H + (size_t)(rl + zt) * H + u;
                     float pv[MEMBERS];
 #pragma unroll
@@ -611,7 +686,7 @@
                 dg = dc * ig * (1.f - gg * gg);
                 dout = dh * tc * og * (1.f - og);
                 dcp = dc * fg;
-                float* dr = a.dgates + ((size_t)row * T + t) * G4;
+                float* dr = a.dgates + ((size_t)(ORD ? c_brow : row) * T + t) * G4;
                 dr[u] = di;
                 dr[H + u] = df;
                 dr[2 * H + u] = dg;
@@ -650,7 +725,7 @@
 #pragma unroll
             for (int s = 0; s < MEMBERS; ++s) sc += pv[s];
             dctxl[rl2][k] = sc;
-            if (myrow0 + rl2 < a.B) a.dctx[((size_t)(myrow0 + rl2 + zt) * T + t) * H + k] = sc;
+            if (myrow0 + rl2 < a.B) a.dctx[((size_t)(ORD ? my_brow : myrow0 + rl2 + zt) * T + t) * H + k] = sc;
         }
         __syncthreads();
         {
@@ -707,8 +782,8 @@
                 if (lane < S) {
                     dwl[rl][lane] = dscore;
                     if (row < a.B) {
-                        a.dscore[((size_t)row * T + t) * S + lane] = dscore;
-                        a.weights[((size_t)row * T + t) * S + lane] = qv / Z;
+                        a.dscore[((size_t)(ORD ? my_brow : row) * T + t) * S + lane] = dscore;
+                        a.weights[((size_t)(ORD ? my_brow : row) * T + t) * S + lane] = qv / Z;
                     }
                 }
             };
@@ -763,7 +838,20 @@
         float sh = 0.f;
 #pragma unroll
         for (int m = 0; m < MEMBERS; ++m) sh += pv[m];
-        if (myrow0 + rl2 < a.B) a.dh0[(size_t)(myrow0 + rl2) * H + k] = sh + att;
+        if (myrow0 + rl2 < a.B) a.dh0[(size_t)(ORD ? my_brow : myrow0 + rl2) * H + k] = sh + att;
+    }
+    if constexpr (ORD) {
+        const int rl2 = tid >> 8, k = tid & 255;
+        for (int t = steps; t < T; ++t) {
+            if (c_row < a.B) {
+                float* dr = a.dgates + ((size_t)c_brow * T + t) * G4 + c_u;
+                dr[0] = 0.f, dr[H] = 0.f, dr[2 * H] = 0.f, dr[3 * H] = 0.f;
+            }
+            if (myrow0 + rl2 < a.B) {
+                a.dctx[((size_t)my_brow * T + t) * H + k] = 0.f;
+                if (k < S) a.dscore[((size_t)my_brow * T + t) * S + k] = 0.f, a.weights[((size_t)my_brow * T + t) * S + k] = 0.f;
+            }
+        }
     }
     cl.finish();
 }
@@ -811,6 +899,47 @@
     }
 }
 
+__global__ __launch_bounds__(512) __attribute__((amdgpu_waves_per_eu(2, 2))) void attn_lstm_bwd_multi_ordered_kernel(const MBwdArgs a,
+                                                                                                                    const RowOrder ro) {
+    int tile, part;
+    pnmn::cluster_coords<MEMBERS>(tile, part);
+    if (tile >= a.tiles) return;
+    attn_lstm_bwd_multi_body<true>(a, tile, part, ro);
+}
+
+__global__ __launch_bounds__(512) __attribute__((amdgpu_waves_per_eu(2, 2))) void attn_lstm_bwd_pair_ordered_kernel(
+    const MBwdArgs a0, const MBwdArgs a1, const int tiles0, const RowOrder ro0, const RowOrder ro1) {
+    int tile, part;
+    pnmn::cluster_coords<MEMBERS>(tile, part);
+    if (tile < tiles0) {
+        if (tile >= a0.tiles) return;
+        attn_lstm_bwd_multi_body<true>(a0, tile, part, ro0);
+    } else {
+        tile -= tiles0;
+        if (tile >= a1.tiles) return;
+        attn_lstm_bwd_multi_body<true>(a1, tile, part, ro1);
+    }
+}
+
+__global__ __launch_bounds__(512) __attribute__((amdgpu_waves_per_eu(2, 2))) void attn_lstm_bwd_group3_ordered_kernel(
+    const MBwdArgs a0, const MBwdArgs a1, const MBwdArgs a2, const int tiles0, const int tiles01, const RowOrder ro0, const RowOrder ro1,
+    const RowOrder ro2) {
+    int tile, part;
+    pnmn::cluster_coords<MEMBERS>(tile, part);
+    if (tile < tiles0) {
+        if (tile >= a0.tiles) return;
+        attn_lstm_bwd_multi_body<true>(a0, tile, part, ro0);
+    } else if (tile < tiles01) {
+        tile -= tiles0;
+        if (tile >= a1.tiles) return;
+        attn_lstm_bwd_multi_body<true>(a1, tile, part, ro1);
+    } else {
+        tile -= tiles01;
+        if (tile >= a2.tiles) return;
+        attn_lstm_bwd_multi_body<true>(a2, tile, part, ro2);
+    }
+}
+
 const void* fwd_multi_variant(bool overlap, bool sample) {
     if (overlap) return sample ? reinterpret_cast<const void*>(attn_lstm_fwd_multi_kernel<true, true>)
                                : reinterpret_cast<const void*>(attn_lstm_fwd_multi_kernel<true, false>);
@@ -826,6 +955,20 @@
 }
 const void* fwd_pair_variant(bool overlap, bool s0, bool s1) {
     return overlap ? fwd_pair_variant_of<true>(s0, s1) : fwd_pair_variant_of<false>(s0, s1);
+}
+
+const void* fwd_multi_ordered_variant(bool overlap) {
+    return overlap ? reinterpret_cast<const void*>(attn_lstm_fwd_multi_ordered_kernel<true>)
+                   : reinterpret_cast<const void*>(attn_lstm_fwd_multi_ordered_kernel<false>);
+}
+template <bool OVERLAP>
+const void* fwd_pair_ordered_variant_of(bool s0, bool s1) {
+    if (s0) return reinterpret_cast<const void*>(attn_lstm_fwd_pair_ordered_kernel<OVERLAP, true, false>);
+    return s1 ? reinterpret_cast<const void*>(attn_lstm_fwd_pair_ordered_kernel<OVERLAP, false, true>)
+              : reinterpret_cast<const void*>(attn_lstm_fwd_pair_ordered_kernel<OVERLAP, false, false>);
+}
+const void* fwd_pair_ordered_variant(bool overlap, bool s0, bool s1) {
+    return overlap ? fwd_pair_ordered_variant_of<true>(s0, s1) : fwd_pair_ordered_variant_of<false>(s0, s1);
 }
 
 const void* fwd_multi_filtered_variant(bool overlap) {
@@ -959,17 +1102,24 @@
 int launch_fwd_constrained(const pnmn_decoder_fwd_job* j, const pnmn_sampling_filter* f, const pnmn::TokenAutomaton& au, int n,
                            int hidden, void* workspace, hipStream_t st);
 int launch_fwd(const pnmn_decoder_fwd_job* j, const pnmn_sampling_filter* f, int n, int hidden, void* workspace, hipStream_t st,
-               const pnmn::TokenAutomaton* au = nullptr) {
+               const pnmn::TokenAutomaton* au = nullptr, const int32_t* const* order = nullptr,
+               const int32_t* const* tile_steps = nullptr) {
     if (n > 1 && !jobs_fit(j, n)) {
-        const int rc = launch_fwd(j, f, n - 1, hidden, workspace, st, au);
-        return rc != 0 ? rc : launch_fwd(j + n - 1, f ? f + n - 1 : nullptr, 1, hidden, workspace, st, au);
+        const int rc = launch_fwd(j, f, n - 1, hidden, workspace, st, au, order, tile_steps);
+        return rc != 0 ? rc
+                       : launch_fwd(j + n - 1, f ? f + n - 1 : nullptr, 1, hidden, workspace, st, au, order ? order + n - 1 : nullptr,
+                                    tile_steps ? tile_steps + n - 1 : nullptr);
     }
     if (au && (j[0].sample != 0 || (n > 1 && j[1].sample != 0))) return launch_fwd_constrained(j, f, *au, n, hidden, workspace, st);
     if (j[0].B <= 0 || j[0].T <= 0) return 0;
     int smax, chunk, rows[MAX_JOBS], tile0[MAX_JOBS + 1];
     if (const int e = plan_group(j, n, hidden, smax, chunk, rows, tile0)) return e;
-    const bool overlap = FWD_FIXED_LDS + sizeof(float) * RW * smax * H + FWD_OVERLAP_LDS <= LDS_LIMIT;
-    const size_t lds = FWD_FIXED_LDS + sizeof(float) * RW * smax * H + (overlap ? FWD_OVERLAP_LDS : 0);
+    RowOrder ro[2] = {{nullptr, nullptr}, {nullptr, nullptr}};
+    for (int i = 0; i < n && order; ++i) ro[i] = RowOrder{order[i], tile_steps[i]};
+    const bool ordered = ro[0].order || ro[1].order;
+    const size_t order_lds = ordered ? ORDER_LDS : 0;
+    const bool overlap = FWD_FIXED_LDS + sizeof(float) * RW * smax * H + FWD_OVERLAP_LDS + order_lds <= LDS_LIMIT;
+    const size_t lds = FWD_FIXED_LDS + sizeof(float) * RW * smax * H + (overlap ? FWD_OVERLAP_LDS : 0) + order_lds;
     const bool s0 = j[0].sample != 0, s1 = n > 1 && j[1].sample != 0;
     int m[2] = {0, 0};
     pnmn::SamplingFilter ff[2] = {{1.f, 0, 1.f}, {1.f, 0, 1.f}};
@@ -978,11 +1128,15 @@
         if (m[i] == 2) ff[i] = pnmn::SamplingFilter{f[i].temperature, f[i].top_k, f[i].top_p};
     }
     const bool filtered = m[0] == 2 || m[1] == 2;
-    const void* kernel = filtered ? (n == 1 ? fwd_multi_filtered_variant(overlap) : fwd_pair_filtered_variant(overlap, m[0], m[1]))
-                                  : (n == 1 ? fwd_multi_variant(overlap, s0) : fwd_pair_variant(overlap, s0, s1));
+    if (ordered && filtered) return PNMN_EINVAL;
+    const void* kernel = ordered    ? (n == 1 ? fwd_multi_ordered_variant(overlap) : fwd_pair_ordered_variant(overlap, s0, s1))
+                         : filtered ? (n == 1 ? fwd_multi_filtered_variant(overlap) : fwd_pair_filtered_variant(overlap, m[0], m[1]))
+                                    : (n == 1 ? fwd_multi_variant(overlap, s0) : fwd_pair_variant(overlap, s0, s1));
     {
-        static std::atomic<uint64_t> cfg[2][8], cfg_filtered[2][2][9];
-        std::atomic<uint64_t>& c = filtered ? cfg_filtered[n - 1][overlap][3 * m[0] + m[1]] : cfg[n - 1][4 * overlap + 2 * s0 + s1];
+        static std::atomic<uint64_t> cfg[2][8], cfg_filtered[2][2][9], cfg_ordered[2][8];
+        std::atomic<uint64_t>& c = ordered    ? cfg_ordered[n - 1][4 * overlap + 2 * s0 + s1]
+                                   : filtered ? cfg_filtered[n - 1][overlap][3 * m[0] + m[1]]
+                                              : cfg[n - 1][4 * overlap + 2 * s0 + s1];
         if (const int e = pnmn::opt_in_lds(kernel, LDS_LIMIT, c)) return e;
     }
     int* sync = nullptr;
@@ -990,7 +1144,11 @@
         hipError_t e = pnmn::cluster_sync_block(workspace, st, &sync);
         if (e != hipSuccess) return (int)e;
         const MFwdArgs a0 = kernel_args(j[0], 0, rows[0], sync, 0), a1 = kernel_args(j[1], 0, rows[1], sync, tile0[1]);
-        if (filtered) {
+        if (ordered) {
+            const auto pair = reinterpret_cast<void (*)(const MFwdArgs, const MFwdArgs, const int, const RowOrder, const RowOrder)>(
+                const_cast<void*>(kernel));
+            hipLaunchKernelGGL(pair, dim3(MEMBERS * tile0[2]), dim3(512), lds, st, a0, a1, tile0[1], ro[0], ro[1]);
+        } else if (filtered) {
             const auto pair = reinterpret_cast<void (*)(const MFwdArgs, const MFwdArgs, const int, const pnmn::SamplingFilter,
                                                         const pnmn::SamplingFilter)>(const_cast<void*>(kernel));
             hipLaunchKernelGGL(pair, dim3(MEMBERS * tile0[2]), dim3(512), lds, st, a0, a1, tile0[1], ff[0], ff[1]);
@@ -1004,8 +1162,12 @@
         const int part = rows[0] - r0 < chunk ? rows[0] - r0 : chunk;
         hipError_t e = pnmn::cluster_sync_block(workspace, st, &sync);
         if (e != hipSuccess) return (int)e;
-        const MFwdArgs a = kernel_args(j[0], (size_t)r0, part, sync, 0);
-        if (filtered) {
+        const MFwdArgs a = kernel_args(j[0], ordered ? 0 : (size_t)r0, part, sync, 0);
+        if (ordered) {
+            const auto multi = reinterpret_cast<void (*)(const MFwdArgs, const RowOrder)>(const_cast<void*>(kernel));
+            hipLaunchKernelGGL(multi, dim3(MEMBERS * padded_tiles(part)), dim3(512), lds, st, a,
+                               RowOrder{ro[0].order + r0, ro[0].tile_steps + r0 / ROWS});
+        } else if (filtered) {
             const auto multi = reinterpret_cast<void (*)(const MFwdArgs, const pnmn::SamplingFilter)>(const_cast<void*>(kernel));
             hipLaunchKernelGGL(multi, dim3(MEMBERS * padded_tiles(part)), dim3(512), lds, st, a, ff[0]);
         } else {
@@ -1063,21 +1225,30 @@
     return 0;
 }
 
-int launch_bwd(const pnmn_decoder_bwd_job* j, int n, int hidden, void* workspace, hipStream_t st) {
+int launch_bwd(const pnmn_decoder_bwd_job* j, int n, int hidden, void* workspace, hipStream_t st,
+               const int32_t* const* order = nullptr, const int32_t* const* tile_steps = nullptr) {
     if (n > 1 && !jobs_fit(j, n)) {
-        const int rc = launch_bwd(j, n - 1, hidden, workspace, st);
-        return rc != 0 ? rc : launch_bwd(j + n - 1, 1, hidden, workspace, st);
+        const int rc = launch_bwd(j, n - 1, hidden, workspace, st, order, tile_steps);
+        return rc != 0 ? rc
+                       : launch_bwd(j + n - 1, 1, hidden, workspace, st, order ? order + n - 1 : nullptr,
+                                    tile_steps ? tile_steps + n - 1 : nullptr);
     }
     if (j[0].B <= 0 || j[0].T <= 0) return 0;
     int smax, chunk, rows[MAX_JOBS], tile0[MAX_JOBS + 1];
     if (const int e = plan_group(j, n, hidden, smax, chunk, rows, tile0)) return e;
     const size_t lds = BWD_FIXED_LDS + sizeof(float) * RW * smax * H;
+    RowOrder ro[MAX_JOBS] = {{nullptr, nullptr}, {nullptr, nullptr}, {nullptr, nullptr}};
+    for (int i = 0; i < n && order; ++i) ro[i] = RowOrder{order[i], tile_steps[i]};
+    const bool ordered = ro[0].order || ro[1].order || ro[2].order;
     {
-        const void* const kernels[MAX_JOBS] = {reinterpret_cast<const void*>(attn_lstm_bwd_multi_kernel),
-                                               reinterpret_cast<const void*>(attn_lstm_bwd_pair_kernel),
-                                               reinterpret_cast<const void*>(attn_lstm_bwd_group3_kernel)};
-        static std::atomic<uint64_t> cfg[MAX_JOBS];
-        if (const int e = pnmn::opt_in_lds(kernels[n - 1], LDS_LIMIT, cfg[n - 1])) return e;
+        const void* const kernels[2][MAX_JOBS] = {{reinterpret_cast<const void*>(attn_lstm_bwd_multi_kernel),
+                                                   reinterpret_cast<const void*>(attn_lstm_bwd_pair_kernel),
+                                                   reinterpret_cast<const void*>(attn_lstm_bwd_group3_kernel)},
+                                                  {reinterpret_cast<const void*>(attn_lstm_bwd_multi_ordered_kernel),
+                                                   reinterpret_cast<const void*>(attn_lstm_bwd_pair_ordered_kernel),
+                                                   reinterpret_cast<const void*>(attn_lstm_bwd_group3_ordered_kernel)}};
+        static std::atomic<uint64_t> cfg[2][MAX_JOBS];
+        if (const int e = pnmn::opt_in_lds(kernels[ordered][n - 1], LDS_LIMIT, cfg[ordered][n - 1])) return e;
     }
     float* x1 = reinterpret_cast<float*>(static_cast<char*>(workspace) + pnmn::CLUSTER_SYNC_BYTES);
     float* x2 = x1 + (size_t)exchange_tiles(rows, n, chunk) * 2 * MEMBERS * 2 * ROWS * H;
@@ -1088,7 +1259,11 @@
         MBwdArgs a[MAX_JOBS];
         for (int i = 0; i < n; ++i) a[i] = kernel_args(j[i], 0, rows[i], sync, tile0[i], x1, x2);
         const dim3 grid(MEMBERS * tile0[n]);
-        if (n == 2) hipLaunchKernelGGL(attn_lstm_bwd_pair_kernel, grid, dim3(512), lds, st, a[0], a[1], tile0[1]);
+        if (ordered) {
+            if (n == 2) hipLaunchKernelGGL(attn_lstm_bwd_pair_ordered_kernel, grid, dim3(512), lds, st, a[0], a[1], tile0[1], ro[0], ro[1]);
+            else hipLaunchKernelGGL(attn_lstm_bwd_group3_ordered_kernel, grid, dim3(512), lds, st, a[0], a[1], a[2], tile0[1], tile0[2],
+                                    ro[0], ro[1], ro[2]);
+        } else if (n == 2) hipLaunchKernelGGL(attn_lstm_bwd_pair_kernel, grid, dim3(512), lds, st, a[0], a[1], tile0[1]);
         else hipLaunchKernelGGL(attn_lstm_bwd_group3_kernel, grid, dim3(512), lds, st, a[0], a[1], a[2], tile0[1], tile0[2]);
         return (int)hipGetLastError();
     }
@@ -1096,8 +1271,12 @@
         const int part = rows[0] - r0 < chunk ? rows[0] - r0 : chunk;
         hipError_t e = pnmn::cluster_sync_block(workspace, st, &sync);
         if (e != hipSuccess) return (int)e;
-        const MBwdArgs a = kernel_args(j[0], (size_t)r0, part, sync, 0, x1, x2);
-        hipLaunchKernelGGL(attn_lstm_bwd_multi_kernel, dim3(MEMBERS * padded_tiles(part)), dim3(512), lds, st, a);
+        const MBwdArgs a = kernel_args(j[0], ordered ? 0 : (size_t)r0, part, sync, 0, x1, x2);
+        if (ordered)
+            hipLaunchKernelGGL(attn_lstm_bwd_multi_ordered_kernel, dim3(MEMBERS * padded_tiles(part)), dim3(512), lds, st, a,
+                               RowOrder{ro[0].order + r0, ro[0].tile_steps + r0 / ROWS});
+        else
+            hipLaunchKernelGGL(attn_lstm_bwd_multi_kernel, dim3(MEMBERS * padded_tiles(part)), dim3(512), lds, st, a);
         e = hipGetLastError();
         if (e != hipSuccess) return (int)e;
     }
@@ -1148,4 +1327,20 @@
     return launch_bwd(jobs, n, hidden, workspace, static_cast<hipStream_t>(stream));
 }
 
-}
+int pnmn_attn_lstm_fwd_group_ordered(const pnmn_decoder_fwd_job* jobs, const int32_t* const* order, const int32_t* const* tile_steps,
+                                     int n, int hidden, void* workspace, void* stream) {
+    if (!jobs || !order || !tile_steps || !workspace || n < 1 || n > 2) return PNMN_EINVAL;
+    for (int i = 0; i < n; ++i)
+        if (!order[i] != !tile_steps[i] || (order[i] && jobs[i].sample != 0)) return PNMN_EINVAL;
+    return launch_fwd(jobs, nullptr, n, hidden, workspace, static_cast<hipStream_t>(stream), nullptr, order, tile_steps);
+}
+
+int pnmn_attn_lstm_bwd_group_ordered(const pnmn_decoder_bwd_job* jobs, const int32_t* const* order, const int32_t* const* tile_steps,
+                                     int n, int hidden, void* workspace, void* stream) {
+    if (!jobs || !order || !tile_steps || !workspace || n < 1 || n > MAX_JOBS) return PNMN_EINVAL;
+    for (int i = 0; i < n; ++i)
+        if (!order[i] != !tile_steps[i]) return PNMN_EINVAL;
+    return launch_bwd(jobs, n, hidden, workspace, static_cast<hipStream_t>(stream), order, tile_steps);
+}
+
+}
diff --git a/probnmn-clevr_amd/csrc/seqglue.hip b/probnmn-clevr_amd/csrc/seqglue.hip
--- a/probnmn-clevr_amd/csrc/seqglue.hip
+++ b/probnmn-clevr_amd/csrc/seqglue.hip
@@ -131,6 +131,20 @@
     }
 }
 
+__global__ __launch_bounds__(256) void token_last_kernel(const int64_t* __restrict__ tokens, int64_t tstride, int B, int T, int pad,
+                                                         int extra, int32_t* __restrict__ last) {
+    const int b = blockIdx.x * 4 + (threadIdx.x >> 6);
+    const int lane = threadIdx.x & 63;
+    if (b >= B) return;
+    const int64_t* row = tokens + (size_t)b * tstride;
+    int end = -1;
+    for (int t = lane; t < T; t += 64)
+        if (row[t] != pad) end = t;
+#pragma unroll
+    for (int o = 32; o > 0; o >>= 1) end = max(end, __shfl_xor(end, o));
+    if (lane == 0) last[b] = end + extra;
+}
+
 __global__ __launch_bounds__(256) void mask_last_bwd_kernel(const float* __restrict__ denc, const float* __restrict__ dhlast,
                                                             const float* __restrict__ fmask, const int* __restrict__ last,
                                                             int T, int H, float* __restrict__ dhs) {
@@ -154,6 +168,8 @@
 }
 
 constexpr int EG_CHUNK = 64;
+constexpr int EG_SLICES = 8;
+constexpr int EG_COLS = 1024;
 
 __device__ __forceinline__ int eg_token(const int64_t* __restrict__ tokens, int64_t tok_bstride, int T, unsigned magic, int shift,
                                         int start, int skip, int V, int r) {
@@ -168,7 +184,8 @@
 __global__ __launch_bounds__(1024) void embedding_rows_kernel(const int64_t* __restrict__ tokens, int64_t tok_bstride, int B,
                                                               int T, unsigned magic, int V, int shift, int start, int skip, int C,
                                                               int* __restrict__ order, int* __restrict__ chunks, int max_per,
-                                                              int* __restrict__ count, float* __restrict__ dw, int keep) {
+                                                              int* __restrict__ count, int* __restrict__ done,
+                                                              int* __restrict__ tokch, float* __restrict__ dw, int keep) {
     __shared__ int whist[16][128], hist[128], rowbase[128], chbase[128];
     const int tid = threadIdx.x, wave = tid >> 6;
     const int per = (B * T + gridDim.x - 1) / gridDim.x;
@@ -176,6 +193,8 @@
     chunks += 3 * (size_t)blockIdx.x * max_per;
     count += blockIdx.x;
     for (int i = tid; i < 16 * 128; i += 1024) (&whist[0][0])[i] = 0;
+    if (tid < 128) done[128 + 128 * blockIdx.x + tid] = 0;
+    if (blockIdx.x == 0 && tid < 128) done[tid] = 0;
     __syncthreads();
     constexpr int UN = 8;
     for (int r0 = lo + tid; r0 < R; r0 += 1024 * UN) {
@@ -220,6 +239,7 @@
     }
     for (int v = tid; v < V; v += 1024) {
         const int n = hist[v];
+        tokch[256 * blockIdx.x + v] = chbase[v], tokch[256 * blockIdx.x + 128 + v] = (n + EG_CHUNK - 1) / EG_CHUNK;
         for (int j = 0; j * EG_CHUNK < n; ++j) {
             int* c = chunks + 3 * (chbase[v] + j);
             c[0] = v, c[1] = rowbase[v] + j * EG_CHUNK, c[2] = rowbase[v] + min(n, (j + 1) * EG_CHUNK);
@@ -227,30 +247,82 @@
     }
 }
 
+__device__ __forceinline__ float4 eg_sum_rows(const float* src, int n) {
+    constexpr int UN = 16;
+    float4 sum = float4{0.f, 0.f, 0.f, 0.f};
+    for (int i = 0; i < n; i += UN) {
+        float4 q[UN];
+#pragma unroll
+        for (int u = 0; u < UN; ++u) q[u] = *reinterpret_cast<const float4*>(src + (size_t)min(i + u, n - 1) * EG_COLS);
+#pragma unroll
+        for (int u = 0; u < UN; ++u)
+            if (i + u < n) sum.x += q[u].x, sum.y += q[u].y, sum.z += q[u].z, sum.w += q[u].w;
+    }
+    return sum;
+}
+
 __global__ __launch_bounds__(256) void embedding_sum_kernel(const float* __restrict__ dy, const int* __restrict__ order,
                                                             const int* __restrict__ chunks, int max_per,
-                                                            const int* __restrict__ count, int C, float* __restrict__ dw) {
+                                                            const int* __restrict__ count, int* done, const int* __restrict__ tokch,
+                                                            float* partial, float* slice_sums, int V, int C, int cols,
+                                                            float* __restrict__ dw) {
+    __shared__ int last_of_slice, last_of_token;
     const int slice = blockIdx.x / max_per, j = blockIdx.x % max_per;
     if (j >= count[slice]) return;
-    const int c = (blockIdx.y * 256 + threadIdx.x) * 4;
-    if (c >= C) return;
+    const int c = threadIdx.x * 4;
+    const bool active = c < cols;
     const int* ch = chunks + 3 * ((size_t)slice * max_per + j);
     const int v = ch[0], b = ch[1], e = ch[2];
     constexpr int UN = 8;
-    float4 acc = float4{0.f, 0.f, 0.f, 0.f};
-    for (int i = b; i < e; i += UN) {
-        float4 q[UN];
-#pragma unroll
-        for (int u = 0; u < UN; ++u) q[u] = *reinterpret_cast<const float4*>(dy + (size_t)order[min(i + u, e - 1)] * C + c);
-#pragma unroll
-        for (int u = 0; u < UN; ++u)
-            if (i + u < e) acc.x += q[u].x, acc.y += q[u].y, acc.z += q[u].z, acc.w += q[u].w;
-    }
-    float* dst = dw + (size_t)v * C + c;
-    unsafeAtomicAdd(dst, acc.x);
-    unsafeAtomicAdd(dst + 1, acc.y);
-    unsafeAtomicAdd(dst + 2, acc.z);
-    unsafeAtomicAdd(dst + 3, acc.w);
+    if (active) {
+        float4 acc = float4{0.f, 0.f, 0.f, 0.f};
+        for (int i = b; i < e; i += UN) {
+            float4 q[UN];
+#pragma unroll
+            for (int u = 0; u < UN; ++u) q[u] = *reinterpret_cast<const float4*>(dy + (size_t)order[min(i + u, e - 1)] * C + c);
+#pragma unroll
+            for (int u = 0; u < UN; ++u)
+                if (i + u < e) acc.x += q[u].x, acc.y += q[u].y, acc.z += q[u].z, acc.w += q[u].w;
+        }
+        *reinterpret_cast<float4*>(partial + (size_t)blockIdx.x * EG_COLS + c) = acc;
+    }
+    __threadfence();
+    __syncthreads();
+    const int n = tokch[256 * slice + 128 + v];
+    if (threadIdx.x == 0) {
+        const int last = atomicAdd(&done[128 + 128 * slice + v], 1) == n - 1;
+        if (last) done[128 + 128 * slice + v] = 0;
+        last_of_slice = last;
+    }
+    __syncthreads();
+    if (!last_of_slice) return;
+    __threadfence();
+    if (active) {
+        const float* src = partial + ((size_t)slice * max_per + tokch[256 * slice + v]) * EG_COLS + c;
+        *reinterpret_cast<float4*>(slice_sums + ((size_t)slice * V + v) * EG_COLS + c) = eg_sum_rows(src, n);
+    }
+    __threadfence();
+    __syncthreads();
+    if (threadIdx.x == 0) {
+        int total = 0;
+        for (int s = 0; s < EG_SLICES; ++s) total += tokch[256 * s + 128 + v] > 0;
+        const int last = atomicAdd(&done[v], 1) == total - 1;
+        if (last) done[v] = 0;
+        last_of_token = last;
+    }
+    __syncthreads();
+    if (!last_of_token || !active) return;
+    __threadfence();
+    float4 sum = float4{0.f, 0.f, 0.f, 0.f};
+#pragma unroll
+    for (int s = 0; s < EG_SLICES; ++s)
+        if (tokch[256 * s + 128 + v] > 0) {
+            const float4 q = *reinterpret_cast<const float4*>(slice_sums + ((size_t)s * V + v) * EG_COLS + c);
+            sum.x += q.x, sum.y += q.y, sum.z += q.z, sum.w += q.w;
+        }
+    float4* dst = reinterpret_cast<float4*>(dw + (size_t)v * C + c);
+    const float4 old = *dst;
+    *dst = float4{old.x + sum.x, old.y + sum.y, old.z + sum.z, old.w + sum.w};
 }
 
 __global__ __launch_bounds__(256) void derive_params_kernel(const pnmn_derive_job* __restrict__ jobs) {
@@ -392,6 +464,15 @@
     return (int)hipGetLastError();
 }
 
+extern "C" int pnmn_token_last(const int64_t* tokens, int64_t token_row_stride, int B, int T, int pad, int extra, int32_t* last,
+                               void* stream) {
+    if (B <= 0) return 0;
+    if (!tokens || !last || T < 0) return PNMN_EINVAL;
+    hipLaunchKernelGGL(token_last_kernel, dim3((B + 3) / 4), dim3(256), 0, static_cast<hipStream_t>(stream), tokens, token_row_stride, B,
+                       T, pad, extra, last);
+    return (int)hipGetLastError();
+}
+
 extern "C" int pnmn_token_rows(const pnmn_token_seg* segs, int n_segs, int64_t* dst, int W, int64_t pad, void* stream) {
     if (n_segs <= 0 || W <= 0) return 0;
     if (!segs || !dst || n_segs > PNMN_TOKEN_SEGS) return PNMN_EINVAL;
@@ -438,14 +519,14 @@
 }
 
 namespace {
-constexpr int EG_SLICES = 8;
 inline int eg_max_per(long rows, int V) { return (int)(((rows + EG_SLICES - 1) / EG_SLICES) / EG_CHUNK) + V; }
+inline long eg_ints(long rows, int V) { return (rows + (long)EG_SLICES * (3 * eg_max_per(rows, V) + 1 + 128 + 256) + 128 + 3) & ~3L; }
 }
 
 extern "C" int64_t pnmn_embedding_grad_workspace_bytes(int B, int T, int V) {
     if (B <= 0 || T <= 0 || V <= 0) return 0;
     const long rows = (long)B * T;
-    return (int64_t)sizeof(int) * (rows + (long)EG_SLICES * (3 * eg_max_per(rows, V) + 1));
+    return (int64_t)sizeof(int) * eg_ints(rows, V) + (int64_t)sizeof(float) * EG_SLICES * (eg_max_per(rows, V) + V) * EG_COLS;
 }
 
 extern "C" int pnmn_embedding_grad(const float* dy, const int64_t* tokens, int64_t token_row_stride, int B, int T, int C,
@@ -455,7 +536,7 @@
     if (!dw || (C & 3) || V > 128) return PNMN_EINVAL;
     hipStream_t s = static_cast<hipStream_t>(stream);
     if (B <= 0 || T <= 0) return accumulate ? 0 : (int)hipMemsetAsync(dw, 0, sizeof(float) * (size_t)V * C, s);
-    if (!dy || !tokens || !workspace) return PNMN_EINVAL;
+    if (!dy || !tokens || !workspace || (reinterpret_cast<uintptr_t>(workspace) & 15)) return PNMN_EINVAL;
     const long rows = (long)B * T;
     if (rows * T >= (1L << 32)) return PNMN_ESHAPE;
     const unsigned magic = T == 1 ? 0u : (unsigned)(((1ULL << 32) + T - 1) / T);
@@ -463,10 +544,15 @@
     int* order = static_cast<int*>(workspace);
     int* chunks = order + rows;
     int* count = chunks + 3 * (size_t)EG_SLICES * max_per;
+    int* done = count + EG_SLICES;
+    int* tokch = done + 128 * (1 + EG_SLICES);
+    float* partial = reinterpret_cast<float*>(order + eg_ints(rows, V));
+    float* slice_sums = partial + (size_t)EG_SLICES * max_per * EG_COLS;
     hipLaunchKernelGGL(embedding_rows_kernel, dim3(EG_SLICES), dim3(1024), 0, s, tokens, token_row_stride, B, T, magic, V, shift,
-                       start, skip, C, order, chunks, max_per, count, dw, accumulate);
-    hipLaunchKernelGGL(embedding_sum_kernel, dim3(EG_SLICES * max_per, (C + 1023) / 1024), dim3(256), 0, s, dy, order, chunks,
-                       max_per, count, C, dw);
+                       start, skip, C, order, chunks, max_per, count, done, tokch, dw, accumulate);
+    for (int c0 = 0; c0 < C; c0 += EG_COLS)
+        hipLaunchKernelGGL(embedding_sum_kernel, dim3(EG_SLICES * max_per), dim3(256), 0, s, dy + c0, order, chunks, max_per, count,
+                           done, tokch, partial, slice_sums, V, C, C - c0 < EG_COLS ? C - c0 : EG_COLS, dw + c0);
     return (int)hipGetLastError();
 }
 
diff --git a/probnmn-clevr_amd/probnmn/_hip.py b/probnmn-clevr_amd/probnmn/_hip.py
--- a/probnmn-clevr_amd/probnmn/_hip.py
+++ b/probnmn-clevr_amd/probnmn/_hip.py
@@ -205,6 +205,17 @@
 def decoder_workspace_bytes(rows, backward: bool) -> int:
     r = np.asarray(rows, np.int32)
     return int(lib().pnmn_attn_lstm_group_workspace_bytes(r.ctypes.data, len(r), 1 if backward else 0))
+
+
+DECODER_ORDER = np.dtype([("order", np.uint64, (3,)), ("tile_steps", np.uint64, (3,))])
+
+
+def decoder_order_record(pairs):
+    rec = np.zeros(1, DECODER_ORDER)
+    for i, pair in enumerate(pairs):
+        if pair is not None:
+            rec["order"][0, i], rec["tile_steps"][0, i] = pair[0].data_ptr(), pair[1].data_ptr()
+    return rec, rec.ctypes.data, rec.ctypes.data + DECODER_ORDER.fields["tile_steps"][1]
 
 
 def stream_ptr(device: torch.device) -> int:
diff --git a/probnmn-clevr_amd/probnmn/runtime/seq_plan.py b/probnmn-clevr_amd/probnmn/runtime/seq_plan.py
--- a/probnmn-clevr_amd/probnmn/runtime/seq_plan.py
+++ b/probnmn-clevr_amd/probnmn/runtime/seq_plan.py
@@ -130,6 +130,8 @@
     trimmed: Optional[torch.Tensor]
     v: Dict[str, torch.Tensor]
     loss: _Loss
+    order: Optional[torch.Tensor] = None
+    tile_steps: Optional[torch.Tensor] = None
 
 
 @dataclass
@@ -436,6 +438,23 @@
             j["w_p"], j["b_p"], j["tokens"], j["V"], j["sample"] = mm.proj.weight.data_ptr(), mm.proj.bias.data_ptr(), p.tokens.data_ptr(), mm.proj.weight.size(0), 1
             j["pad_index"], j["unk_index"] = mm.model._pad_index, mm.model._unk_index
 
+    def _decoder_order(self, calls: _Calls, p: _DecoderPass, tokens: torch.Tensor, extra: int) -> None:
+        if p.rows <= LENGTH_ORDER_ABOVE_ROWS or os.environ.get("PNMN_DECODER_LENGTH_ORDER", "1") == "0":
+            return
+        f = self.buf
+        last = f(p.tag + ".d_last", p.rows, dtype=torch.int32)
+        p.order, p.tile_steps = f(p.tag + ".d_order", p.rows, dtype=torch.int32), f(p.tag + ".d_tile_steps", (p.rows + 15) // 16, dtype=torch.int32)
+        calls.add("pnmn_token_last", tokens.data_ptr(), tokens.stride(0), p.rows, tokens.size(1), p.loss.pad, extra, last.data_ptr(), self.stream)
+        calls.add("pnmn_length_order", last.data_ptr(), p.rows, p.T, p.order.data_ptr(), p.tile_steps.data_ptr(), self.stream)
+
+    def _decoder_group(self, calls: _Calls, entry: str, jobs: np.ndarray, passes: List[_DecoderPass], ws: torch.Tensor) -> None:
+        if not any(p.order is not None for p in passes):
+            calls.add(entry, jobs.ctypes.data, len(jobs), 256, ws.data_ptr(), self.stream)
+            return
+        rec, order, tile_steps = _hip.decoder_order_record([None if p.order is None else (p.order, p.tile_steps) for p in passes])
+        self._keep.append(rec)
+        calls.add(entry + "_ordered", jobs.ctypes.data, order, tile_steps, len(jobs), 256, ws.data_ptr(), self.stream)
+
     def _decoder_forward(self, calls: _Calls, dec: _DecoderSet, source: torch.Tensor, tgt: torch.Tensor, ws_name: str) -> np.ndarray:
         model, rows = dec.mm.model, [p.rows for p in dec.passes]
         calls.add("pnmn_token_prep", source.data_ptr(), source.stride(0), source.size(0), source.size(1), model._pad_index, model._start_index,
@@ -444,8 +463,10 @@
         jobs = np.zeros(len(dec.passes), _hip.DECODER_FWD_JOB)
         for j, p in zip(jobs, dec.passes):
             self._decoder_fwd_job(j, dec, p)
+            if p.trimmed is None:
+                self._decoder_order(calls, p, source, 1)
         ws = self.bytes_buf(ws_name, _hip.decoder_workspace_bytes(rows, False))
-        calls.add("pnmn_attn_lstm_fwd_group", jobs.ctypes.data, len(jobs), 256, ws.data_ptr(), self.stream)
+        self._decoder_group(calls, "pnmn_attn_lstm_fwd_group", jobs, dec.passes, ws)
         return jobs
 
     def _decoder_losses(self, calls: _Calls, dec: _DecoderSet) -> None:
@@ -548,7 +569,10 @@
             j["B"], j["T"], j["S"] = p.rows, p.T, p.S
         self._keep.append(bj)
         gws = self.bytes_buf("group_ws", _hip.decoder_workspace_bytes([p.rows for _, p in passes], True))
-        c.add("pnmn_attn_lstm_bwd_group", bj.ctypes.data, len(bj), 256, gws.data_ptr(), st)
+        for _, p in passes:
+            if p.trimmed is not None:
+                self._decoder_order(c, p, p.trimmed, 0)
+        self._decoder_group(c, "pnmn_attn_lstm_bwd_group", bj, [p for _, p in passes], gws)
         for dec, p in passes:
             c.add("pnmn_attn_denc", p.v["weights"].data_ptr(), p.v["dscore"].data_ptr(), p.v["dctx"].data_ptr(), p.v["hs"].data_ptr(),
                   dec.enc["h"][p.enc_row0:].data_ptr(), dec.enc["denc"][p.enc_row0:].data_ptr(), p.rows, p.T, p.S, 256, st)
```

Result: slower. 36960 questions/s (-2.4%).
